# daviddmc/NeSVoR

Measured on AMD Instinct MI355X. Metric: INR train iters/sec (2^20 samples, L=16 hash, 64-wide MLP), higher is better.
Workload: dtype f32 (MLP products evaluated on 2-way fp16 splits of the power-of-two-scaled fp32 operands, fp32 accumulation: error against fp64 at or below the fp32 MFMA chain's; the all-fp32-MFMA rate of the same run is in strict_fp32_mfma)

## Files before the change

### include/nesvor_hip.h

```cpp
#ifndef NESVOR_HIP_H
#define NESVOR_HIP_H

#include <stdint.h>

#ifdef __cplusplus
extern "C" {
#endif

#define NESVOR_MAX_LEVELS 32
#define NESVOR_MAX_MLP_LAYERS 4

int nesvor_hip_abi_version(void);

int nesvor_axisangle2mat_forward(const float* ax, float* mat, int n, void* stream);
int nesvor_axisangle2mat_backward(const float* grad_mat, const float* ax, float* grad_ax, int n, void* stream);
int nesvor_mat2axisangle_forward(const float* mat, float* ax, int n, void* stream);
int nesvor_mat2axisangle_backward(const float* mat, const float* grad_ax, float* grad_mat, int n, void* stream);
int nesvor_axisangle2mat_forward_f64(const double* ax, double* mat, int n, void* stream);
int nesvor_axisangle2mat_backward_f64(const double* grad_mat, const double* ax, double* grad_ax, int n, void* stream);
int nesvor_mat2axisangle_forward_f64(const double* mat, double* ax, int n, void* stream);
int nesvor_mat2axisangle_backward_f64(const double* mat, const double* grad_ax, double* grad_mat, int n, void* stream);

int nesvor_trans_loss(const float* ax, const float* ax_init, float* loss_per_slice, float* grad_ax, int n, void* stream);

int nesvor_slice_acq_forward(const float* transforms, const float* vol, const uint8_t* vol_mask,
                             const uint8_t* slices_mask, const float* psf, float* slices, float* slices_weight,
                             int D, int H, int W, int d_p, int h_p, int w_p, int n, int h, int w,
                             float res_slice, int interp_psf, void* stream);

int nesvor_slice_acq_adjoint_forward(const float* transforms, const float* psf, const float* slices,
                                     const uint8_t* slices_mask, const uint8_t* vol_mask, float* vol, float* vol_weight,
                                     float* scratch, int D, int H, int W, int d_p, int h_p, int w_p, int n, int h, int w,
                                     float res_slice, int equalize, void* stream);
int nesvor_slice_acq_adjoint_backward(const float* transforms, float* grad_vol, const float* vol_weight,
                                      const uint8_t* vol_mask, const float* psf, const float* slices,
                                      const uint8_t* slices_mask, const float* vol, float* grad_slices,
                                      float* grad_transforms, int D, int H, int W, int d_p, int h_p, int w_p, int n, int h,
                                      int w, float res_slice, int equalize, void* stream);
int nesvor_slice_acq_backward(const float* transforms, const float* vol, const uint8_t* vol_mask, const float* psf,
                              const float* grad_slices, const uint8_t* slices_mask, float* grad_vol,
                              float* grad_transforms, float* scratch, int D, int H, int W, int d_p, int h_p, int w_p,
                              int n, int h, int w, float res_slice, void* stream);
int nesvor_slice_acq_adjoint_forward_interp(const float* transforms, const float* psf, const float* slices,
                                            const uint8_t* slices_mask, const uint8_t* vol_mask, float* vol, float* vol_weight,
                                            int D, int H, int W, int d_p, int h_p, int w_p, int n, int h, int w,
                                            float res_slice, int equalize, void* stream);
int nesvor_slice_acq_backward_interp(const float* transforms, const float* vol, const uint8_t* vol_mask, const float* psf,
                                     const float* grad_slices, const uint8_t* slices_mask, float* grad_vol,
                                     float* grad_transforms, int D, int H, int W, int d_p, int h_p, int w_p, int n, int h, int w,
                                     float res_slice, void* stream);
int nesvor_slice_acq_adjoint_backward_interp(const float* transforms, float* grad_vol, const float* vol_weight,
                                             const uint8_t* vol_mask, const float* psf, const float* slices,
                                             const uint8_t* slices_mask, const float* vol, float* grad_slices,
                                             float* grad_transforms, int D, int H, int W, int d_p, int h_p, int w_p, int n,
                                             int h, int w, float res_slice, int equalize, void* stream);
int nesvor_slice_acq_adjoint_forward_interp_f64(const double* transforms, const double* psf, const double* slices,
                                                const uint8_t* slices_mask, const uint8_t* vol_mask, double* vol,
                                                double* vol_weight, int D, int H, int W, int d_p, int h_p, int w_p, int n, int h,
                                                int w, double res_slice, int equalize, void* stream);
int nesvor_slice_acq_backward_interp_f64(const double* transforms, const double* vol, const uint8_t* vol_mask,
                                         const double* psf, const double* grad_slices, const uint8_t* slices_mask,
                                         double* grad_vol, double* grad_transforms, int D, int H, int W, int d_p, int h_p,
                                         int w_p, int n, int h, int w, double res_slice, void* stream);
int nesvor_slice_acq_adjoint_backward_interp_f64(const double* transforms, double* grad_vol, const double* vol_weight,
                                                 const uint8_t* vol_mask, const double* psf, const double* slices,
                                                 const uint8_t* slices_mask, const double* vol, double* grad_slices,
                                                 double* grad_transforms, int D, int H, int W, int d_p, int h_p, int w_p,
                                                 int n, int h, int w, double res_slice, int equalize, void* stream);
int nesvor_slice_acq_forward_f64(const double* transforms, const double* vol, const uint8_t* vol_mask,
                                 const uint8_t* slices_mask, const double* psf, double* slices, double* slices_weight,
                                 int D, int H, int W, int d_p, int h_p, int w_p, int n, int h, int w,
                                 double res_slice, int interp_psf, void* stream);
int nesvor_slice_acq_adjoint_forward_f64(const double* transforms, const double* psf, const double* slices,
                                         const uint8_t* slices_mask, const uint8_t* vol_mask, double* vol, double* vol_weight,
                                         double* scratch, int D, int H, int W, int d_p, int h_p, int w_p, int n, int h, int w,
                                         double res_slice, int equalize, void* stream);
int nesvor_slice_acq_backward_f64(const double* transforms, const double* vol, const uint8_t* vol_mask, const double* psf,
                                  const double* grad_slices, const uint8_t* slices_mask, double* grad_vol,
                                  double* grad_transforms, double* scratch, int D, int H, int W, int d_p, int h_p, int w_p,
                                  int n, int h, int w, double res_slice, void* stream);
int nesvor_slice_acq_adjoint_backward_f64(const double* transforms, double* grad_vol, const double* vol_weight,
                                          const uint8_t* vol_mask, const double* psf, const double* slices,
                                          const uint8_t* slices_mask, const double* vol, double* grad_slices,
                                          double* grad_transforms, int D, int H, int W, int d_p, int h_p, int w_p, int n, int h,
                                          int w, double res_slice, int equalize, void* stream);

typedef struct {
  int32_t n_levels;
  int32_t n_features;
  float scale[NESVOR_MAX_LEVELS];
  uint32_t res[NESVOR_MAX_LEVELS];
  uint32_t size[NESVOR_MAX_LEVELS];
  uint32_t offset[NESVOR_MAX_LEVELS];
  uint32_t hashed[NESVOR_MAX_LEVELS];
} nesvor_grid_t;

#define NESVOR_LAYOUT_ROW_MAJOR 0
#define NESVOR_LAYOUT_FEATURE_MAJOR 1
#define NESVOR_LAYOUT_CLUSTERED 4
#define NESVOR_LAYOUT_UNCLUSTERED 8
#define NESVOR_LAYOUT_DY_SCRATCH 16
#define NESVOR_LAYOUT_MASK 3

int nesvor_hashgrid_forward(const nesvor_grid_t* grid, const float* u, const float* table, float* pe,
                            int64_t N, int layout, void* stream);
int nesvor_hashgrid_forward_bounded(const nesvor_grid_t* grid, const float* u, const float* table, float* pe,
                                    int64_t N, int layout, float* pe_absmax, void* stream);
int64_t nesvor_hashgrid_forward_workspace_bytes(const nesvor_grid_t* grid, int64_t N, int layout);
int nesvor_hashgrid_forward_unclustered(const nesvor_grid_t* grid, const float* u, const float* table, float* pe, int64_t N,
                                        int layout, float* pe_absmax, void* workspace, int64_t workspace_bytes, void* stream);
int64_t nesvor_hashgrid_backward_workspace_bytes(const nesvor_grid_t* grid, int64_t N, const float* queue_scale);
int64_t nesvor_hashgrid_backward_workspace_bytes_ex(const nesvor_grid_t* grid, int64_t N, const float* queue_scale, int layout);
int64_t nesvor_hashgrid_backward_workspace_zero_bytes(void);
int64_t nesvor_hashgrid_backward_overflow_offset(void* workspace);
int nesvor_hashgrid_backward(const nesvor_grid_t* grid, const float* u, const float* table, const float* dpe,
                             float* grad_table, float* grad_u, int64_t N, int layout, void* workspace, int stages,
                             const float* queue_scale, void* stream);

int nesvor_hashgrid_backward_levels(const nesvor_grid_t* grid, const float* u, const float* table, const float* dpe,
                                    float* grad_table, float* grad_u, int64_t N, int layout, void* workspace, int stages,
                                    int level_begin, int level_end, const float* queue_scale, void* stream);
int nesvor_hashgrid_backward_bounded(const nesvor_grid_t* grid, const float* u, const float* table, const float* dpe,
                                     float* grad_table, float* grad_u, int64_t N, int layout, void* workspace, int stages,
                                     int level_begin, int level_end, const float* queue_scale, const float* dy_bound,
                                     void* stream);
int nesvor_hashgrid_backward_atomic(const nesvor_grid_t* grid, const float* u, const float* table, const float* dpe,
                                    float* grad_table, float* grad_u, int64_t N, int layout, void* stream);

int nesvor_psf_transform_forward(const float* mat, const int64_t* slice_idx, const float* xyz, const float* sigma,
                                 const float* noise, const float* bb, float* x, float* u, int B, int S, void* stream);
int nesvor_psf_transform_backward(const float* mat, const int64_t* slice_idx, const float* xyz, const float* sigma,
                                  const float* noise, const float* bb, const float* dx, const float* du, float* dmat,
                                  int B, int S, void* stream);
int nesvor_psf_transform_forward_rng(const float* mat, const int64_t* slice_idx, const float* xyz, const float* sigma,
                                     uint64_t seed, uint64_t offset, const float* bb, float* x, float* u, int B, int S,
                                     void* stream);
int nesvor_psf_transform_forward_rng_gather(const float* mat, const int64_t* slice_idx, const float* xyz, const float* sigma,
                                            uint64_t seed, uint64_t offset, const float* bb, float* x, float* u, int B, int S,
                                            const float* embedding, float* se, int ks, void* stream);
int nesvor_psf_transform_backward_rng(const float* mat, const int64_t* slice_idx, const float* xyz, const float* sigma,
                                      uint64_t seed, uint64_t offset, const float* bb, const float* dx, const float* du,
                                      float* dmat, int B, int S, void* stream);
int nesvor_psf_transform_backward_rng_slices(const float* mat, const int64_t* slice_idx, const float* xyz, const float* sigma,
                                             uint64_t seed, uint64_t offset, const float* bounding_box, const float* dx,
                                             const float* du, float* dpix, float* dmat_slice, int B, int S, void* stream);
int nesvor_psf_noise(uint64_t seed, uint64_t offset, float* out, int64_t n_samples, void* stream);

typedef struct {
  int32_t width;
  int32_t n_hidden;
  int32_t out_dim;
  int32_t k_a, k_b, b_row0;
  int32_t samples_per_pixel;
  int32_t dxa_group_sums;
  int32_t bf16_operands;
  int32_t compact_save;
  const float* weight[NESVOR_MAX_MLP_LAYERS];
  const float* bias[NESVOR_MAX_MLP_LAYERS];
  const float* prep;
  float* y_absmax;
  const void* weight_images;
} nesvor_mlp_t;
#define NESVOR_MLP_MODE_FP32 0
#define NESVOR_MLP_MODE_BF16 1
#define NESVOR_MLP_MODE_SPLIT 2
#define NESVOR_MLP_MODE_FP16 3
#define NESVOR_MLP_MODE_FP16_SCALED 4
#define NESVOR_ABSMAX_SLOTS 16
#define NESVOR_ABSMAX_STRIDE 64
#define NESVOR_ABSMAX_FLOATS (NESVOR_ABSMAX_SLOTS * NESVOR_ABSMAX_STRIDE)
#define NESVOR_MLP_PREP_XA 0
#define NESVOR_MLP_PREP_XB (1 * NESVOR_ABSMAX_FLOATS)
#define NESVOR_MLP_PREP_DY (2 * NESVOR_ABSMAX_FLOATS)
#define NESVOR_MLP_PREP_LAYER0 (3 * NESVOR_ABSMAX_FLOATS)
#define NESVOR_MLP_PREP_FLOATS (NESVOR_MLP_PREP_LAYER0 + 4 * NESVOR_MAX_MLP_LAYERS)
#define NESVOR_MLP_WHAT_INPUT 1
#define NESVOR_MLP_WHAT_DY 2
#define NESVOR_MLP_WHAT_WEIGHTS 4
int nesvor_mlp_prepare(const nesvor_mlp_t* net, const float* xa, const float* xb, const float* dy, int64_t N, float* prep,
                       int what, void* stream);
int nesvor_mlp_prepare_weights(const nesvor_mlp_t* const* nets, float* const* preps, int n_nets, const float* x, int64_t n_x,
                               float* x_slots, void* stream);

int nesvor_mlp_prepare_weights_images(const nesvor_mlp_t* const* nets, float* const* preps, void* const* images, int n_nets,
                                      const float* x, int64_t n_x, float* x_slots, void* stream);
int64_t nesvor_mlp_weight_images_bytes(const nesvor_mlp_t* net);

int nesvor_mlp_compact_save_ok(const nesvor_mlp_t* net, int64_t N);
int nesvor_mlp_bias_free_ok(const nesvor_mlp_t* net, int64_t N);

int nesvor_mlp_forward(const nesvor_mlp_t* net, const float* xa, const float* xb, float* y,
                       float* const* saved_hidden, int64_t N, void* stream);
int nesvor_mlp_backward_fused_ok(const nesvor_mlp_t* net, int64_t N);
int nesvor_mlp_backward(const nesvor_mlp_t* net, const float* xa, const float* xb, const float* dy,
                        float* const* saved_hidden, float* const* dpre_scratch, float* dxa, float* dxb,
                        float* dw_partial, int n_partial, int64_t N, void* stream);
int nesvor_mlp_backward_bounded(const nesvor_mlp_t* net, const float* xa, const float* xb, const float* dy,
                                float* const* saved_hidden, float* const* dpre_scratch, float* dxa, float* dxb,
                                float* dw_partial, int n_partial, int64_t N, float* dxb_absmax, void* stream);

#define NESVOR_MLP_WIDE_MAX_LAYERS 8
typedef struct {
  int32_t width;
  int32_t n_hidden;
  int32_t out_dim;
  int32_t k_a, k_b, b_row0;
  int32_t samples_per_pixel;
  int32_t reserved;
  const float* weight[NESVOR_MLP_WIDE_MAX_LAYERS];
  const float* bias[NESVOR_MLP_WIDE_MAX_LAYERS];
} nesvor_mlp_wide_t;
int64_t nesvor_mlp_wide_saved_floats(const nesvor_mlp_wide_t* net, int64_t N);
int nesvor_mlp_wide_param_count(const nesvor_mlp_wide_t* net);
int nesvor_mlp_wide_forward(const nesvor_mlp_wide_t* net, const float* xa, const float* xb, float* y, float* const* saved_hidden,
                            int64_t N, void* stream);
int nesvor_mlp_wide_backward(const nesvor_mlp_wide_t* net, const float* xa, const float* xb, const float* dy,
                             float* const* saved_hidden, float* const* dpre_scratch, float* dxa, float* dxb, float* dw_partial,
                             int n_partial, int64_t N, void* stream);
int nesvor_mlp_wide_backward_bounded(const nesvor_mlp_wide_t* net, const float* xa, const float* xb, const float* dy,
                                     float* const* saved_hidden, float* const* dpre_scratch, float* dxa, float* dxb,
                                     float* dw_partial, int n_partial, int64_t N, float* dxb_absmax, void* stream);

typedef struct {
  const float* z0; const float* log_var; const float* log_bias; const float* x; const float* v;
  const int64_t* slice_idx; const float* c; const float* log_var_slice; const float* log_bias_mean;
  const float* gw;
  float* loss_pix; float* dz0; float* dlog_var; float* dlog_bias; float* dx; float* dc_pix; float* dlvs_pix;
  int32_t B, S, reg_type;
  float delta;
  float* dz0_absmax; float* dlog_var_absmax; float* dlog_bias_absmax;
} nesvor_loss_t;

int nesvor_imaging_loss(const nesvor_loss_t* args, void* stream);

int nesvor_step_prologue(const float* logit_coef, float* c, const float* axisangle, float* mat, float* zero_buf,
                         int n_zero, int n, void* stream);
int nesvor_step_prologue_pose(const float* logit_coef, float* c, const float* axisangle, float* mat, float* zero_buf,
                              int n_zero, int n, const float* axisangle_init, float* trans_terms, float* g_trans, void* stream);
int nesvor_step_epilogue(const float* dc, const float* c, float* dlogit, const float* dmat, const float* axisangle,
                         const float* dtrans, float w_trans, float* daxisangle, const float* loss_pix,
                         const float* trans_terms, float* losses, int n, int B, float img_scale, float img_offset,
                         void* stream);
int nesvor_step_epilogue_scaled(const float* dc, const float* c, float* dlogit, const float* dmat, const float* axisangle,
                                const float* dtrans, float w_trans, const float* w_trans_scale, float* daxisangle,
                                const float* loss_pix, const float* trans_terms, float* losses, int n, int B, float img_scale,
                                float img_offset, void* stream);
int nesvor_slice_grads(const int64_t* slice_idx, const float* dc_pix, const float* dlvs_pix, const float* dxa,
                       const float* dpix, float* dc, float* dlvs, float* dse, float* dmat, int B, int S, int ks,
                       void* stream);
int nesvor_slice_grads_by_slice(const int64_t* slice_idx, const float* dc_pix, const float* dlvs_pix, const float* dxa,
                                const float* dpix, float* dc, float* dlvs, float* dse, float* dmat, int B, int S, int ks,
                                int n_slices, void* stream);

int nesvor_adamw_step(float* param, float* grad, float* exp_avg, float* exp_avg_sq, int64_t n,
                      float lr, float beta1, float beta2, float eps, float weight_decay,
                      float bias_correction1, float bias_correction2, float grad_scale, int zero_grad,
                      void* stream);

typedef struct {
  float lr, beta1, beta2, eps, weight_decay, bias_correction1, bias_correction2, grad_scale;
} nesvor_adamw_t;

typedef struct nesvor_loss_scaler_t {
  float scale, growth_factor, backoff_factor;
  int32_t growth_interval, growth_tracker, skipped, t;
  uint32_t found_inf;
} nesvor_loss_scaler_t;

int nesvor_grad_found_inf(const float* grad, int64_t n, nesvor_loss_scaler_t* s, void* stream);
int nesvor_adamw_step_scaled(float* param, float* grad, float* exp_avg, float* exp_avg_sq, int64_t n, float lr, double beta1,
                             double beta2, float eps, float weight_decay, int world_size, int zero_grad,
                             const nesvor_loss_scaler_t* s, void* stream);
int nesvor_loss_scaler_update(nesvor_loss_scaler_t* s, void* stream);
int nesvor_loss_scale_weights(const float* base, float* out, int n, const nesvor_loss_scaler_t* s, void* stream);

int nesvor_hashgrid_backward_adamw(const nesvor_grid_t* grid, const float* u, float* table, const float* dpe,
                                   float* grad_table, float* grad_u, int64_t N, int layout, void* workspace, int stages,
                                   const float* queue_scale, const float* dy_bound, float* exp_avg, float* exp_avg_sq,
// ... 66 lines not shown
```

### nesvor_amd/_lib.py

```python
import ctypes
import os
from ctypes import POINTER, Structure, c_double, c_float, c_int, c_int32, c_int64, c_uint32, c_uint64, c_void_p

import torch

_HERE = os.path.dirname(os.path.abspath(__file__))
LIB_PATH = os.environ.get("NESVOR_HIP_LIB") or os.path.join(_HERE, "lib", "libnesvor_hip.so")
MAX_LEVELS = 32
ABI_VERSION = 38

LAYOUT_ROW_MAJOR = 0
LAYOUT_FEATURE_MAJOR = 1
STEP_DEFER_JOIN = 8
STEP_BIAS_SUM_STOP = 16
STEP_BIAS_SUM_RESUME = 32
LAYOUT_CLUSTERED = 4
LAYOUT_UNCLUSTERED = 8
LAYOUT_DY_SCRATCH = 16


class GridT(Structure):

    _fields_ = [
        ("n_levels", c_int32),
        ("n_features", c_int32),
        ("scale", c_float * MAX_LEVELS),
        ("res", c_uint32 * MAX_LEVELS),
        ("size", c_uint32 * MAX_LEVELS),
        ("offset", c_uint32 * MAX_LEVELS),
        ("hashed", c_uint32 * MAX_LEVELS),
    ]


class MlpT(Structure):

    _fields_ = [
        ("width", c_int32), ("n_hidden", c_int32), ("out_dim", c_int32),
        ("k_a", c_int32), ("k_b", c_int32), ("b_row0", c_int32), ("samples_per_pixel", c_int32),
        ("dxa_group_sums", c_int32), ("bf16_operands", c_int32), ("compact_save", c_int32),
        ("weight", c_void_p * 4), ("bias", c_void_p * 4),
        ("prep", c_void_p), ("y_absmax", c_void_p), ("weight_images", c_void_p),
    ]


class MlpWideT(Structure):

    _fields_ = [
        ("width", c_int32), ("n_hidden", c_int32), ("out_dim", c_int32),
        ("k_a", c_int32), ("k_b", c_int32), ("b_row0", c_int32), ("samples_per_pixel", c_int32), ("reserved", c_int32),
        ("weight", c_void_p * 8), ("bias", c_void_p * 8),
    ]


class LossT(Structure):

    _fields_ = [(n, c_void_p) for n in (
        "z0", "log_var", "log_bias", "x", "v", "slice_idx", "c", "log_var_slice", "log_bias_mean", "gw",
        "loss_pix", "dz0", "dlog_var", "dlog_bias", "dx", "dc_pix", "dlvs_pix")] + [
        ("B", c_int32), ("S", c_int32), ("reg_type", c_int32), ("delta", c_float),
        ("dz0_absmax", c_void_p), ("dlog_var_absmax", c_void_p), ("dlog_bias_absmax", c_void_p)]


class StepT(Structure):

    _fields_ = (
        [("grid", GridT), ("density", MlpT), ("sigma", MlpT), ("bias_net", MlpT)]
        + [(n, c_int32) for n in ("B", "S", "n_slices", "opt_T", "has_lv", "has_c", "has_lvs", "has_b", "n_features_z", "ks", "kb_bias",
                                  "reg_type", "overlap_owner")]
        + [("delta", c_float), ("w_T", c_float)]
        + [(n, c_void_p) for n in ("axisangle", "axisangle_init", "psf_sigma", "bounding_box", "logit_coef", "log_var_slice",
                                   "slice_embedding", "table")]
        + [(n, c_void_p) for n in ("g_axisangle", "g_logit_coef", "g_log_var_slice", "g_slice_embedding", "g_table", "g_density", "g_sigma",
                                   "g_bias_net")]
        + [(n, c_int32) for n in ("n_density_params", "n_sigma_params", "n_bias_params")]
        + [("gw", c_void_p)]
        + [(n, c_void_p) for n in ("flat_param", "flat_grad", "flat_exp_avg", "flat_exp_avg_sq")]
        + [("flat_numel", c_int64)]
        + [(n, c_void_p) for n in ("small", "x", "u", "pe", "z", "log_var", "log_bias", "se", "dz", "dlv", "dlb", "dxl", "loss_pix", "pix",
                                   "dpe", "dpe_b", "du", "dpix", "dxa", "dxa_b", "trans_terms", "g_trans", "lb_mean", "mean_scratch",
                                   "partial")]
        + [("saved_d", c_void_p * 4), ("saved_s", c_void_p * 4), ("saved_b", c_void_p * 4), ("dpre_scratch", c_void_p * 4)]
        + [("hg_workspace", c_void_p), ("queue_scale", c_void_p), ("side_stream", c_void_p)]
    )


class AdamwT(Structure):

    _fields_ = [(n, c_float) for n in ("lr", "beta1", "beta2", "eps", "weight_decay", "bias_correction1", "bias_correction2", "grad_scale")]


class LossScalerT(Structure):

    _fields_ = [("scale", c_float), ("growth_factor", c_float), ("backoff_factor", c_float), ("growth_interval", c_int32),
                ("growth_tracker", c_int32), ("skipped", c_int32), ("t", c_int32), ("found_inf", c_uint32)]


_lib = None

_P = c_void_p
_SIGNATURES = {
    "nesvor_hip_abi_version": ([], c_int),
    "nesvor_axisangle2mat_forward": ([_P, _P, c_int, _P], c_int),
    "nesvor_axisangle2mat_backward": ([_P, _P, _P, c_int, _P], c_int),
    "nesvor_mat2axisangle_forward": ([_P, _P, c_int, _P], c_int),
    "nesvor_mat2axisangle_backward": ([_P, _P, _P, c_int, _P], c_int),
    "nesvor_axisangle2mat_forward_f64": ([_P, _P, c_int, _P], c_int),
    "nesvor_axisangle2mat_backward_f64": ([_P, _P, _P, c_int, _P], c_int),
    "nesvor_mat2axisangle_forward_f64": ([_P, _P, c_int, _P], c_int),
    "nesvor_mat2axisangle_backward_f64": ([_P, _P, _P, c_int, _P], c_int),
    "nesvor_trans_loss": ([_P, _P, _P, _P, c_int, _P], c_int),
    "nesvor_slice_acq_forward": (
        [_P, _P, _P, _P, _P, _P, _P] + [c_int] * 9 + [c_float, c_int, _P],
        c_int,
    ),
    "nesvor_slice_acq_adjoint_forward": ([_P] * 8 + [c_int] * 9 + [c_float, c_int, _P], c_int),
    "nesvor_slice_acq_backward": ([_P] * 9 + [c_int] * 9 + [c_float, _P], c_int),
    "nesvor_slice_acq_adjoint_backward": ([_P] * 10 + [c_int] * 9 + [c_float, c_int, _P], c_int),
    "nesvor_slice_acq_forward_f64": ([_P, _P, _P, _P, _P, _P, _P] + [c_int] * 9 + [c_double, c_int, _P], c_int),
    "nesvor_slice_acq_adjoint_forward_f64": ([_P] * 8 + [c_int] * 9 + [c_double, c_int, _P], c_int),
    "nesvor_slice_acq_backward_f64": ([_P] * 9 + [c_int] * 9 + [c_double, _P], c_int),
    "nesvor_slice_acq_adjoint_backward_f64": ([_P] * 10 + [c_int] * 9 + [c_double, c_int, _P], c_int),
    "nesvor_slice_acq_adjoint_forward_interp": ([_P] * 7 + [c_int] * 9 + [c_float, c_int, _P], c_int),
    "nesvor_slice_acq_backward_interp": ([_P] * 8 + [c_int] * 9 + [c_float, _P], c_int),
    "nesvor_slice_acq_adjoint_backward_interp": ([_P] * 10 + [c_int] * 9 + [c_float, c_int, _P], c_int),
    "nesvor_slice_acq_adjoint_forward_interp_f64": ([_P] * 7 + [c_int] * 9 + [c_double, c_int, _P], c_int),
    "nesvor_slice_acq_backward_interp_f64": ([_P] * 8 + [c_int] * 9 + [c_double, _P], c_int),
    "nesvor_slice_acq_adjoint_backward_interp_f64": ([_P] * 10 + [c_int] * 9 + [c_double, c_int, _P], c_int),
    "nesvor_hashgrid_forward": ([POINTER(GridT), _P, _P, _P, c_int64, c_int, _P], c_int),
    "nesvor_hashgrid_forward_bounded": ([POINTER(GridT), _P, _P, _P, c_int64, c_int, _P, _P], c_int),
    "nesvor_hashgrid_forward_workspace_bytes": ([POINTER(GridT), c_int64, c_int], c_int64),
    "nesvor_hashgrid_forward_unclustered": ([POINTER(GridT), _P, _P, _P, c_int64, c_int, _P, _P, c_int64, _P], c_int),
    "nesvor_hashgrid_backward_workspace_bytes": ([POINTER(GridT), c_int64, _P], c_int64),
    "nesvor_hashgrid_backward_workspace_bytes_ex": ([POINTER(GridT), c_int64, _P, c_int], c_int64),
    "nesvor_hashgrid_backward_workspace_zero_bytes": ([], c_int64),
    "nesvor_hashgrid_backward_overflow_offset": ([_P], c_int64),
    "nesvor_hashgrid_backward": ([POINTER(GridT), _P, _P, _P, _P, _P, c_int64, c_int, _P, c_int, _P, _P], c_int),
    "nesvor_hashgrid_backward_levels": ([POINTER(GridT), _P, _P, _P, _P, _P, c_int64, c_int, _P, c_int, c_int, c_int, _P, _P], c_int),
    "nesvor_hashgrid_backward_bounded": ([POINTER(GridT), _P, _P, _P, _P, _P, c_int64, c_int, _P, c_int, c_int, c_int, _P, _P, _P], c_int),
    "nesvor_hashgrid_backward_atomic": ([POINTER(GridT), _P, _P, _P, _P, _P, c_int64, c_int, _P], c_int),
    "nesvor_psf_transform_forward": ([_P] * 8 + [c_int, c_int, _P], c_int),
    "nesvor_psf_transform_backward": ([_P] * 9 + [c_int, c_int, _P], c_int),
    "nesvor_psf_transform_forward_rng_gather": ([_P] * 4 + [c_uint64, c_uint64] + [_P] * 3 + [c_int, c_int, _P, _P, c_int, _P], c_int),
    "nesvor_psf_transform_forward_rng": ([_P] * 4 + [c_uint64, c_uint64] + [_P] * 3 + [c_int, c_int, _P], c_int),
    "nesvor_psf_transform_backward_rng": ([_P] * 4 + [c_uint64, c_uint64] + [_P] * 4 + [c_int, c_int, _P], c_int),
    "nesvor_psf_transform_backward_rng_slices": ([_P] * 4 + [c_uint64, c_uint64] + [_P] * 5 + [c_int, c_int, _P], c_int),
    "nesvor_psf_noise": ([c_uint64, c_uint64, _P, c_int64, _P], c_int),
    "nesvor_mlp_compact_save_ok": ([POINTER(MlpT), c_int64], c_int),
    "nesvor_mlp_bias_free_ok": ([POINTER(MlpT), c_int64], c_int),
    "nesvor_mlp_backward_fused_ok": ([POINTER(MlpT), c_int64], c_int),
    "nesvor_mlp_prepare": ([POINTER(MlpT), _P, _P, _P, c_int64, _P, c_int, _P], c_int),
    "nesvor_mlp_prepare_weights": ([_P, _P, c_int, _P, c_int64, _P, _P], c_int),
    "nesvor_mlp_prepare_weights_images": ([_P, _P, _P, c_int, _P, c_int64, _P, _P], c_int),
    "nesvor_mlp_weight_images_bytes": ([POINTER(MlpT)], c_int64),
    "nesvor_mlp_forward": ([POINTER(MlpT), _P, _P, _P, POINTER(c_void_p), c_int64, _P], c_int),
    "nesvor_mlp_backward": (
        [POINTER(MlpT), _P, _P, _P, POINTER(c_void_p), POINTER(c_void_p), _P, _P, _P, c_int, c_int64, _P],
        c_int,
    ),
    "nesvor_mlp_backward_bounded": (
        [POINTER(MlpT), _P, _P, _P, POINTER(c_void_p), POINTER(c_void_p), _P, _P, _P, c_int, c_int64, _P, _P],
        c_int,
    ),
    "nesvor_mlp_wide_saved_floats": ([POINTER(MlpWideT), c_int64], c_int64),
    "nesvor_mlp_wide_param_count": ([POINTER(MlpWideT)], c_int),
    "nesvor_mlp_wide_forward": ([POINTER(MlpWideT), _P, _P, _P, POINTER(c_void_p), c_int64, _P], c_int),
    "nesvor_mlp_wide_backward": (
        [POINTER(MlpWideT), _P, _P, _P, POINTER(c_void_p), POINTER(c_void_p), _P, _P, _P, c_int, c_int64, _P],
        c_int,
    ),
    "nesvor_mlp_wide_backward_bounded": (
        [POINTER(MlpWideT), _P, _P, _P, POINTER(c_void_p), POINTER(c_void_p), _P, _P, _P, c_int, c_int64, _P, _P],
        c_int,
    ),
    "nesvor_imaging_loss": ([POINTER(LossT), _P], c_int),
    "nesvor_slice_grads_by_slice": ([_P] * 9 + [c_int, c_int, c_int, c_int, _P], c_int),
    "nesvor_slice_grads": ([_P] * 9 + [c_int, c_int, c_int, _P], c_int),
    "nesvor_step_prologue": ([_P] * 5 + [c_int, c_int, _P], c_int),
    "nesvor_step_prologue_pose": ([_P] * 5 + [c_int, c_int, _P, _P, _P, _P], c_int),
    "nesvor_step_epilogue": ([_P] * 6 + [c_float, _P, _P, _P, _P, c_int, c_int, c_float, c_float, _P], c_int),
    "nesvor_step_epilogue_scaled": ([_P] * 6 + [c_float, _P, _P, _P, _P, _P, c_int, c_int, c_float, c_float, _P], c_int),
    "nesvor_hashgrid_backward_adamw": ([POINTER(GridT), _P, _P, _P, _P, _P, c_int64, c_int, _P, c_int, _P, _P, _P, _P, POINTER(AdamwT), _P], c_int),
    "nesvor_adamw_step": (
        [_P, _P, _P, _P, c_int64] + [c_float] * 8 + [c_int, _P],
        c_int,
    ),
    "nesvor_grad_found_inf": ([_P, c_int64, _P, _P], c_int),
    "nesvor_adamw_step_scaled": ([_P, _P, _P, _P, c_int64, c_float, c_double, c_double, c_float, c_float, c_int, c_int, _P, _P], c_int),
    "nesvor_loss_scaler_update": ([_P, _P], c_int),
    "nesvor_loss_scale_weights": ([_P, _P, c_int, _P, _P], c_int),
    "nesvor_sum_rows_multi": ([_P, _P, _P, _P, c_int, c_int, _P], c_int),
    "nesvor_sum_rows": ([_P, _P, c_int, c_int, c_int, _P], c_int),
    "nesvor_step_create": ([POINTER(StepT)], c_void_p),
    "nesvor_step_update": ([_P, POINTER(StepT)], c_int),
    "nesvor_step_destroy": ([_P], None),
    "nesvor_step_join": ([_P, _P], c_int),
    "nesvor_step_set_bias_mean_ranks": ([_P, c_int], c_int),
    "nesvor_step_set_bias_mean_event": ([_P, _P], c_int),
    "nesvor_step_timing": ([_P, c_int], c_int),
    "nesvor_step_timing_read": ([_P, _P], c_int),
    "nesvor_step_run": ([_P, _P, _P, _P, c_uint64, c_uint64, _P, c_int, c_int, POINTER(AdamwT), _P], c_int),
    "nesvor_vvr_similarity": ([_P, c_int, c_int, c_int, _P, _P, _P, _P, c_int64, c_int, _P, _P, _P], c_int),
}


def exported_symbols():
    return list(_SIGNATURES)


def load():
    global _lib
    if _lib is not None:
        return _lib
    if not os.path.exists(LIB_PATH):
        raise RuntimeError(
            f"{LIB_PATH} not found: the HIP backend has not been built. "
            "Run `python -m nesvor_amd.csrc.build` (or __graft_entry__.build()). "
            "There is no CPU fallback for the native ops."
        )
    lib = ctypes.CDLL(LIB_PATH)
    for name, (argtypes, restype) in _SIGNATURES.items():
        fn = getattr(lib, name)
        fn.argtypes = argtypes
        fn.restype = restype
    v = lib.nesvor_hip_abi_version()
    if v != ABI_VERSION:
        raise RuntimeError(f"libnesvor_hip ABI {v} != expected {ABI_VERSION}; rebuild")
    _lib = lib
    return lib


def stream_ptr(device=None):
    return c_void_p(torch.cuda.current_stream(device).cuda_stream)


def ptr(t):
    if t is None:
        return c_void_p(0)
    return c_void_p(t.data_ptr())


def check(err, what):
    if err != 0:
        raise RuntimeError(f"{what}: HIP error {err}")


def require_device(*tensors, dtype=None, name="tensor"):
    for t in tensors:
        if t is None:
            continue
        if not t.is_cuda:
            raise RuntimeError(f"{name} must be a device (HIP) tensor — the native ops have no CPU path")
        if not t.is_contiguous():
            raise RuntimeError(f"{name} must be contiguous")
        if dtype is not None and t.dtype != dtype:
            raise RuntimeError(f"{name} must be {dtype}, got {t.dtype}")


class KernelTimer:

    def __init__(self):
        self.enabled = False
        self.records = {}

    def reset(self, enabled):
        self.enabled = enabled
        self.records = {}

    class _Span:
        def __init__(self, timer, name):
            self.timer, self.name = timer, name

        def __enter__(self):
            if self.timer.enabled:
                self.s = torch.cuda.Event(enable_timing=True)
                self.e = torch.cuda.Event(enable_timing=True)
                self.s.record()
            return self

        def __exit__(self, *exc):
            if self.timer.enabled:
                self.e.record()
                self.timer.records.setdefault(self.name, []).append((self.s, self.e))
            return False

    def span(self, name):
        return KernelTimer._Span(self, name)

    def summary(self):
        return {k: (len(v), sum(s.elapsed_time(e) for s, e in v) / len(v)) for k, v in self.records.items()}


kernel_timer = KernelTimer()
# ... 1 lines not shown
```

### nesvor_amd/csrc/hashgrid.hip

```cpp
#include <hip/hip_runtime.h>
#include <mutex>
#include <type_traits>
#include <unordered_map>
#include "common.h"
#include "adam.h"
#include "../../include/nesvor_hip.h"

#ifndef NESVOR_ABLATE
#define NESVOR_ABLATE 0
#endif
#define NESVOR_ABL(bit) ((NESVOR_ABLATE & (bit)) != 0)
#ifndef NESVOR_SORT_SPAN
#define NESVOR_SORT_SPAN 256
#endif

namespace {

constexpr uint32_t kPrimeY = 2654435761u;
constexpr uint32_t kPrimeZ = 805459861u;

struct LevelParams {
  float scale;
  uint32_t res, size, offset, hashed;
};

__device__ __forceinline__ LevelParams load_level(const nesvor_grid_t& g, int level) {
  LevelParams p;
  p.scale = g.scale[level];
  p.res = g.res[level];
  p.size = g.size[level];
  p.offset = g.offset[level];
  p.hashed = g.hashed[level];
  return p;
}

__device__ __forceinline__ uint32_t corner_index(const LevelParams& p, uint32_t x, uint32_t y, uint32_t z) {
  if (p.hashed) {
    const uint32_t h = x ^ (y * kPrimeY) ^ (z * kPrimeZ);
    return ((p.size & (p.size - 1)) == 0) ? (h & (p.size - 1)) : (h % p.size);
  }
  uint32_t idx = x + __umul24(y, p.res) + __umul24(z, p.res * p.res);
  if (idx >= p.size) idx %= p.size;
  return idx;
}

__device__ __forceinline__ uint32_t scan32_u32(uint32_t v, int lane) {
#define NESVOR_SCAN_STEP_(SHR)                                                                        \
  v += (uint32_t)__builtin_amdgcn_update_dpp(0, (int)v, 0x110 | (SHR), 0xf, 0xf, true);
  NESVOR_SCAN_STEP_(1) NESVOR_SCAN_STEP_(2) NESVOR_SCAN_STEP_(4) NESVOR_SCAN_STEP_(8)
#undef NESVOR_SCAN_STEP_
  const uint32_t row0 = (uint32_t)__builtin_amdgcn_readlane((int)v, 15);
  return v + ((lane >= 16 && lane < 32) ? row0 : 0u);
}

struct RoundSchedule {
  uint32_t slot_off, bkt_off, grp_end, rnd_slots, rnd_bkts;
  int box_end;
};
__device__ __forceinline__ RoundSchedule round_schedule(uint32_t vol, uint32_t nch, int first, int last, int lane, uint32_t max_slots,
                                                        uint32_t max_bkts, int max_group) {
  const unsigned long long no_box = __ballot(vol == 0u) | ~((1ull << last) - 1ull);
  const int e = __builtin_ctzll(no_box & ~((1ull << first) - 1ull));
  const bool in = lane >= first && lane < e;
  const uint32_t v_in = in ? vol : 0u, n_in = in ? nch : 0u;
  const uint32_t C = scan32_u32(v_in, lane), N = scan32_u32(n_in, lane);
  RoundSchedule r;
  r.slot_off = 0u; r.bkt_off = 0u; r.grp_end = 0u; r.rnd_slots = 0u; r.rnd_bkts = 0u; r.box_end = e;
  int g0 = first;
  while (g0 < e) {
    const uint32_t cb = (uint32_t)__builtin_amdgcn_readlane((int)(C - v_in), g0), nb = (uint32_t)__builtin_amdgcn_readlane((int)(N - n_in), g0);
    const bool ok = lane >= g0 && lane < e && C - cb <= max_slots && N - nb <= max_bkts && lane - g0 < max_group;
    int bnd = __builtin_ctzll((__ballot(!ok) & ~((1ull << g0) - 1ull)) | (1ull << 63));
    bnd = bnd > g0 ? bnd : g0 + 1;
    const bool mine = lane >= g0 && lane < bnd;
    r.slot_off = mine ? (C - v_in) - cb : r.slot_off;
    r.bkt_off = mine ? (N - n_in) - nb : r.bkt_off;
    r.grp_end = mine ? (uint32_t)bnd : r.grp_end;
    const uint32_t cs = (uint32_t)__builtin_amdgcn_readlane((int)C, bnd - 1) - cb, ns = (uint32_t)__builtin_amdgcn_readlane((int)N, bnd - 1) - nb;
    r.rnd_slots = lane == g0 ? cs : r.rnd_slots;
    r.rnd_bkts = lane == g0 ? ns : r.rnd_bkts;
    g0 = bnd;
  }
  return r;
}

struct CellPos {
  uint32_t gx, gy, gz;
  float wx, wy, wz;
};

__device__ __forceinline__ CellPos locate(const LevelParams& p, float ux, float uy, float uz) {
  CellPos c;
  const float px = fmaf(p.scale, ux, 0.5f), py = fmaf(p.scale, uy, 0.5f), pz = fmaf(p.scale, uz, 0.5f);
  const float fx = floorf(px), fy = floorf(py), fz = floorf(pz);
  c.gx = (uint32_t)(int)fx; c.gy = (uint32_t)(int)fy; c.gz = (uint32_t)(int)fz;
  c.wx = px - fx; c.wy = py - fy; c.wz = pz - fz;
  return c;
}

template <int F>
__device__ __forceinline__ void load_feat(const float* __restrict__ p, float (&v)[F]) {
  if constexpr (F == 1) {
    v[0] = p[0];
  } else if constexpr (F == 2) {
    const float2 t = *reinterpret_cast<const float2*>(p);
    v[0] = t.x; v[1] = t.y;
  } else {
#pragma unroll
    for (int k = 0; k < F; k += 4) {
      const float4 t = *reinterpret_cast<const float4*>(p + k);
      v[k] = t.x; v[k + 1] = t.y; v[k + 2] = t.z; v[k + 3] = t.w;
    }
  }
}

template <int F>
__device__ __forceinline__ void load_feat_pair(const float* __restrict__ tab, uint32_t i0, uint32_t i1, float (&v0)[F], float (&v1)[F]) {
  if constexpr (F <= 2) {
    const bool adj = (i1 == i0 + 1u) || (i0 == i1 + 1u);
    const uint32_t p = adj ? min(i0, i1) : (i0 & ~1u);
    float t[2 * F];
    if constexpr (F == 1) {
      struct __attribute__((packed, aligned(4))) P2 { float a, b; };
      const P2 w = *reinterpret_cast<const P2*>(tab + (size_t)p);
      t[0] = w.a; t[1] = w.b;
    } else {
      struct __attribute__((packed, aligned(8))) P4 { float a, b, c, d; };
      const P4 w = *reinterpret_cast<const P4*>(tab + (size_t)p * 2);
      t[0] = w.a; t[1] = w.b; t[2] = w.c; t[3] = w.d;
    }
    const bool second0 = i0 != p;
#pragma unroll
    for (int f = 0; f < F; ++f) { v0[f] = second0 ? t[F + f] : t[f]; v1[f] = second0 ? t[f] : t[F + f]; }
    if (!adj) load_feat<F>(tab + (size_t)i1 * F, v1);
  } else {
    load_feat<F>(tab + (size_t)i0 * F, v0);
    load_feat<F>(tab + (size_t)i1 * F, v1);
  }
}

template <int F, int LAYOUT>
__global__ __launch_bounds__(256) void hashgrid_fwd(const nesvor_grid_t g, const float* __restrict__ u,
                                                    const float* __restrict__ table, float* __restrict__ pe,
                                                    int64_t N, int box_cache, float* __restrict__ pe_absmax) {
  constexpr int kFwdSlots = F <= 2 ? 1024 : (F == 4 ? 512 : 256);
  __shared__ uint32_t wbox[4][6];
  __shared__ __attribute__((aligned(16))) float cache[kFwdSlots * F];
  const int level = blockIdx.y, tid = threadIdx.x, lane = tid & 63;
  const int64_t i = (int64_t)blockIdx.x * 256 + tid;
  const bool valid = i < N;
  const int64_t ii = valid ? i : N - 1;
  const LevelParams p = load_level(g, level);
  const float ux = u[3 * ii], uy = u[3 * ii + 1], uz = u[3 * ii + 2];
  const CellPos c = locate(p, ux, uy, uz);
  const float* tab = table + (size_t)p.offset * F;
  float v[8][F];
  bool cached = false;
  if (box_cache) {
    const uint32_t bx = c.gx + 1u, by = c.gy + 1u, bz = c.gz + 1u;
    const uint32_t lo0 = wave_min_u32_dpp(bx), lo1 = wave_min_u32_dpp(by), lo2 = wave_min_u32_dpp(bz);
    const uint32_t hi0 = wave_max_u32_dpp(bx), hi1 = wave_max_u32_dpp(by), hi2 = wave_max_u32_dpp(bz);
    if (lane == 0) {
      uint32_t* w = wbox[tid >> 6];
      w[0] = lo0; w[1] = lo1; w[2] = lo2; w[3] = hi0; w[4] = hi1; w[5] = hi2;
    }
    __syncthreads();
    uint32_t lo[3], hi[3];
#pragma unroll
    for (int d = 0; d < 3; ++d) {
      lo[d] = min(min(wbox[0][d], wbox[1][d]), min(wbox[2][d], wbox[3][d]));
      hi[d] = max(max(wbox[0][3 + d], wbox[1][3 + d]), max(wbox[2][3 + d], wbox[3][3 + d]));
      lo[d] = (uint32_t)__builtin_amdgcn_readfirstlane((int)lo[d]);
      hi[d] = (uint32_t)__builtin_amdgcn_readfirstlane((int)hi[d]);
    }
    const uint32_t ex = hi[0] - lo[0], ey = hi[1] - lo[1], ez = hi[2] - lo[2];
    const uint32_t nx = ex + 2u, ny = ey + 2u, nz = ez + 2u, nxy = nx * ny;
    cached = ex < (uint32_t)kFwdSlots && ey < (uint32_t)kFwdSlots && ez < (uint32_t)kFwdSlots &&
             (uint64_t)nxy * nz <= (uint64_t)kFwdSlots;
    if (cached) {
      const uint32_t vol = nxy * nz;
      const float inv_nxy = 1.f / (float)nxy, inv_nx = 1.f / (float)nx;
      for (uint32_t s = tid; s < vol; s += 256) {
        const uint32_t z = (uint32_t)(((float)s + 0.5f) * inv_nxy);
        const uint32_t r = s - __umul24(z, nxy);
        const uint32_t y = (uint32_t)(((float)r + 0.5f) * inv_nx);
        const uint32_t idx = corner_index(p, lo[0] - 1u + (r - __umul24(y, nx)), lo[1] - 1u + y, lo[2] - 1u + z);
        float t[F];
        load_feat<F>(tab + (size_t)idx * F, t);
#pragma unroll
        for (int f = 0; f < F; ++f) cache[s * F + f] = t[f];
      }
      __syncthreads();
      const uint32_t s0 = __umul24(__umul24(bz - lo[2], ny) + (by - lo[1]), nx) + (bx - lo[0]);
#pragma unroll
      for (int k = 0; k < 8; ++k) {
        const uint32_t s = s0 + (k & 1) + ((k >> 1) & 1) * nx + (k >> 2) * nxy;
#pragma unroll
        for (int f = 0; f < F; ++f) v[k][f] = cache[s * F + f];
      }
    }
  }
  if (!cached) {
#pragma unroll
    for (int k = 0; k < 8; k += 2) {
      const uint32_t i0 = corner_index(p, c.gx, c.gy + ((k >> 1) & 1), c.gz + (k >> 2));
      const uint32_t i1 = corner_index(p, c.gx + 1u, c.gy + ((k >> 1) & 1), c.gz + (k >> 2));
      load_feat_pair<F>(tab, i0, i1, v[k], v[k + 1]);
    }
  }
  float acc[F];
#pragma unroll
  for (int f = 0; f < F; ++f) acc[f] = 0.f;
  if (valid) {
#pragma unroll
    for (int k = 0; k < 8; ++k) {
      const float w = ((k & 1) ? c.wx : 1.f - c.wx) * (((k >> 1) & 1) ? c.wy : 1.f - c.wy) * ((k >> 2) ? c.wz : 1.f - c.wz);
#pragma unroll
      for (int f = 0; f < F; ++f) acc[f] = fmaf(w, v[k][f], acc[f]);
    }
    const int E = g.n_levels * F;
    if constexpr (LAYOUT == NESVOR_LAYOUT_ROW_MAJOR) {
      float* o = pe + (size_t)i * E + level * F;
#pragma unroll
      for (int f = 0; f < F; ++f) o[f] = acc[f];
    } else {
#pragma unroll
      for (int f = 0; f < F; ++f) pe[(size_t)(level * F + f) * N + i] = acc[f];
    }
  }
  if (pe_absmax != nullptr) {
    float m = 0.f;
#pragma unroll
    for (int f = 0; f < F; ++f) m = fmaxf(m, fabsf(acc[f]));
    publish_absmax_wg(pe_absmax, m);
  }
}

#ifndef NESVOR_FWD_PK
#define NESVOR_FWD_PK 1
#endif
#ifndef NESVOR_FWD_SSTORE
#define NESVOR_FWD_SSTORE 1
#endif
template <int F, int LAYOUT>
__global__ __launch_bounds__(256) void hashgrid_fwd_cloud(const nesvor_grid_t g, const float* __restrict__ u,
                                                          const float* __restrict__ table, float* __restrict__ pe, int64_t N,
                                                          float* __restrict__ pe_absmax,
                                                          const uint32_t* __restrict__ perm = nullptr, float* __restrict__ rows = nullptr,
                                                          int level_begin = 0, int level_stop = NESVOR_MAX_LEVELS) {
#ifndef NESVOR_FWD_CLOUD_SLOTS
#define NESVOR_FWD_CLOUD_SLOTS 512
#endif
  constexpr int kSlots = F <= 2 ? NESVOR_FWD_CLOUD_SLOTS : (F == 4 ? 512 : 256);
  constexpr int kMaxGroup = 8;
  constexpr int NRB = kSlots / 256;
  __shared__ __attribute__((aligned(16))) float tcache[2][kSlots * F];
  __shared__ float ubox[4][6];
  __shared__ uint32_t lbox[NESVOR_MAX_LEVELS + 1][8];
  __shared__ uint32_t lpar[NESVOR_MAX_LEVELS + 1][4];
  __shared__ uint32_t slot_off[NESVOR_MAX_LEVELS + 1], grp_end[NESVOR_MAX_LEVELS + 1], rnd_slots[NESVOR_MAX_LEVELS + 1];
  __shared__ int32_t box_end_s;
  const int tid = threadIdx.x, lane = tid & 63;
  const int64_t slot_i = (int64_t)blockIdx.x * 256 + tid;
  const bool valid = slot_i < N;
  const int64_t si = valid ? slot_i : N - 1;
  const int64_t i = perm != nullptr ? (int64_t)perm[si] : slot_i;
  const int64_t ii = perm != nullptr ? i : si;
  const int L = g.n_levels, E = L * F;
  const int lb = level_begin, le = min(level_stop, L);
  const float ux = u[3 * ii], uy = u[3 * ii + 1], uz = u[3 * ii + 2];
  {
    float lo[3] = {ux, uy, uz}, hi[3] = {ux, uy, uz};
#pragma unroll
    for (int d = 0; d < 3; ++d) { lo[d] = -wave_max_f32_dpp(-lo[d]); hi[d] = wave_max_f32_dpp(hi[d]); }
    if (lane == 0) {
#pragma unroll
      for (int d = 0; d < 3; ++d) { ubox[tid >> 6][d] = lo[d]; ubox[tid >> 6][3 + d] = hi[d]; }
    }
  }
  __syncthreads();
  if (tid < 64) {
    float ulo[3], uhi[3];
#pragma unroll
    for (int d = 0; d < 3; ++d) {
      ulo[d] = fminf(fminf(ubox[0][d], ubox[1][d]), fminf(ubox[2][d], ubox[3][d]));
      uhi[d] = fmaxf(fmaxf(ubox[0][3 + d], ubox[1][3 + d]), fmaxf(ubox[2][3 + d], ubox[3][3 + d]));
    }
    uint32_t b[8] = {0u, 0u, 0u, 0u, 0u, 0u, 0u, 0u};
    if (tid < L) {
      const LevelParams p = load_level(g, tid);
      const CellPos blo = locate(p, ulo[0], ulo[1], ulo[2]), bhi = locate(p, uhi[0], uhi[1], uhi[2]);
      const uint32_t ex = bhi.gx - blo.gx, ey = bhi.gy - blo.gy, ez = bhi.gz - blo.gz;
      const bool fits = ex < (uint32_t)kSlots && ey < (uint32_t)kSlots && ez < (uint32_t)kSlots &&
                        (uint64_t)(ex + 2u) * (ey + 2u) * (ez + 2u) <= (uint64_t)kSlots;
      const uint32_t nx = ex + 2u, nxy = nx * (ey + 2u), vol = fits ? nxy * (ez + 2u) : 0u;
      b[0] = blo.gx; b[1] = blo.gy; b[2] = blo.gz; b[3] = ex; b[4] = ey; b[5] = ez; b[6] = vol;
      b[7] = fits ? vol - 2u - nx - nxy : 0u;
      lpar[tid][0] = p.res; lpar[tid][1] = p.size; lpar[tid][2] = p.offset; lpar[tid][3] = p.hashed;
    }
    if (tid <= L) {
#pragma unroll
      for (int q = 0; q < 8; ++q) lbox[tid][q] = b[q];
    }
    const RoundSchedule rs = round_schedule(b[6], 0u, lb, le, tid, (uint32_t)kSlots, 0xFFFFFFFFu, kMaxGroup);
    if (tid == 0) box_end_s = rs.box_end;
    if (tid < NESVOR_MAX_LEVELS) { slot_off[tid] = rs.slot_off; grp_end[tid] = rs.grp_end; rnd_slots[tid] = rs.rnd_slots; }
  }
  __syncthreads();
  const int box_end = __builtin_amdgcn_readfirstlane(box_end_s);
  auto sgpr = [](uint32_t v) { return (uint32_t)__builtin_amdgcn_readfirstlane((int)v); };
  const bool off32 = NESVOR_FWD_SSTORE && N < ((int64_t)1 << 30);
  const uint32_t i4 = (uint32_t)i * 4u;
  float pe_mx = 0.f;
  auto store_pe = [&](int level, const float (&acc)[F]) __attribute__((always_inline)) {
    if (!valid) return;
#pragma unroll
    for (int f = 0; f < F; ++f) pe_mx = fmaxf(pe_mx, fabsf(acc[f]));
    if (rows != nullptr) {
      float* o = rows + (size_t)slot_i * E + level * F;
#pragma unroll
      for (int f = 0; f < F; ++f) o[f] = acc[f];
      return;
    }
    if constexpr (LAYOUT == NESVOR_LAYOUT_ROW_MAJOR) {
      float* o = pe + (size_t)i * E + level * F;
#pragma unroll
      for (int f = 0; f < F; ++f) o[f] = acc[f];
    } else {
      if (off32) {
#pragma unroll
        for (int f = 0; f < F; ++f) gstore_b32_sbase(pe + (size_t)(level * F + f) * N, i4, acc[f]);
      } else {
#pragma unroll
        for (int f = 0; f < F; ++f) pe[(size_t)(level * F + f) * N + i] = acc[f];
      }
    }
  };
  auto blend = [&](const CellPos& c, const float (&v)[8][F], float (&acc)[F]) __attribute__((always_inline)) {
    if constexpr (F == 2 && NESVOR_FWD_PK) {
      typedef float f32x2 __attribute__((ext_vector_type(2)));
      const f32x2 wx2 = {1.f - c.wx, c.wx};
      const float ay[2] = {1.f - c.wy, c.wy}, az[2] = {1.f - c.wz, c.wz};
      f32x2 a = {0.f, 0.f};
#pragma unroll
      for (int zy = 0; zy < 4; ++zy) {
        const f32x2 w2 = (wx2 * ay[zy & 1]) * az[zy >> 1];
        a = __builtin_elementwise_fma(f32x2{w2.x, w2.x}, f32x2{v[2 * zy][0], v[2 * zy][1]}, a);
        a = __builtin_elementwise_fma(f32x2{w2.y, w2.y}, f32x2{v[2 * zy + 1][0], v[2 * zy + 1][1]}, a);
      }
      acc[0] = a.x; acc[1] = a.y;
      return;
    }
#pragma unroll
    for (int f = 0; f < F; ++f) acc[f] = 0.f;
#pragma unroll
    for (int k = 0; k < 8; ++k) {
      const float w = ((k & 1) ? c.wx : 1.f - c.wx) * (((k >> 1) & 1) ? c.wy : 1.f - c.wy) * ((k >> 2) ? c.wz : 1.f - c.wz);
#pragma unroll
      for (int f = 0; f < F; ++f) acc[f] = fmaf(w, v[k][f], acc[f]);
    }
  };
  auto fetch_round = [&](int ra, int rb, float (&feat)[NRB][F]) __attribute__((always_inline)) {
    const uint32_t total = sgpr(rnd_slots[ra]);
#pragma unroll
    for (int j = 0; j < NRB; ++j) {
      const uint32_t slot = (uint32_t)j * 256u + (uint32_t)tid;
#pragma unroll
      for (int f = 0; f < F; ++f) feat[j][f] = 0.f;
      if (slot < total) {
        int lv = ra;
        for (int l = ra + 1; l < rb; ++l) lv = slot >= slot_off[l] ? l : lv;
        const uint32_t local = slot - slot_off[lv];
        const uint32_t nx = lbox[lv][3] + 2u, nxy = nx * (lbox[lv][4] + 2u);
        const uint32_t z = (uint32_t)(((float)local + 0.5f) * (1.f / (float)nxy));
        const uint32_t r = local - __umul24(z, nxy);
        const uint32_t y = (uint32_t)(((float)r + 0.5f) * (1.f / (float)nx));
        LevelParams pl;
        pl.scale = 0.f; pl.res = lpar[lv][0]; pl.size = lpar[lv][1]; pl.offset = lpar[lv][2]; pl.hashed = lpar[lv][3];
        const uint32_t key = corner_index(pl, lbox[lv][0] + (r - __umul24(y, nx)), lbox[lv][1] + y, lbox[lv][2] + z);
        load_feat<F>(table + ((size_t)pl.offset + key) * F, feat[j]);
      }
    }
  };
  auto stash_round = [&](int ra, int buf, const float (&feat)[NRB][F]) __attribute__((always_inline)) {
    const uint32_t total = sgpr(rnd_slots[ra]);
#pragma unroll
    for (int j = 0; j < NRB; ++j) {
      const uint32_t slot = (uint32_t)j * 256u + (uint32_t)tid;
      if (slot < total) {
#pragma unroll
        for (int f = 0; f < F; ++f) tcache[buf][slot * F + f] = feat[j][f];
      }
    }
  };
  if (box_end > lb) {
    int ra = lb, rb = (int)sgpr(grp_end[lb]), buf = 0;
    {
      float feat[NRB][F];
      fetch_round(ra, rb, feat);
      stash_round(ra, 0, feat);
    }
    __syncthreads();
    for (;;) {
      const int na = rb, nb = na < box_end ? (int)sgpr(grp_end[na]) : na;
      const bool more = na < box_end;
      float nfeat[NRB][F];
      if (more) fetch_round(na, nb, nfeat);
#pragma unroll 1
      for (int lv = ra; lv < rb; ++lv) {
        const LevelParams p = load_level(g, lv);
        const CellPos c = locate(p, ux, uy, uz);
        const uint32_t x0 = sgpr(lbox[lv][0]), y0 = sgpr(lbox[lv][1]), z0 = sgpr(lbox[lv][2]);
        const uint32_t ny = sgpr(lbox[lv][4]) + 2u, nx = sgpr(lbox[lv][3]) + 2u, nxy = nx * ny;
        const uint32_t s0 = min(__umul24(__umul24(c.gz - z0, ny) + (c.gy - y0), nx) + (c.gx - x0), sgpr(lbox[lv][7])) + sgpr(slot_off[lv]);
        float v[8][F], acc[F];
#pragma unroll
        for (int k = 0; k < 8; ++k) {
          const uint32_t sl = s0 + (k & 1) + ((k >> 1) & 1) * nx + (k >> 2) * nxy;
#pragma unroll
          for (int f = 0; f < F; ++f) v[k][f] = tcache[buf][sl * F + f];
        }
        blend(c, v, acc);
        store_pe(lv, acc);
      }
      if (!more) break;
      stash_round(na, buf ^ 1, nfeat);
      __syncthreads();
      buf ^= 1; ra = na; rb = nb;
    }
  }
#pragma unroll 1
  for (int lv = box_end; lv < le; lv += 2) {
    const bool two = lv + 1 < le;
    const LevelParams p0 = load_level(g, lv), p1 = load_level(g, two ? lv + 1 : lv);
    const CellPos c0 = locate(p0, ux, uy, uz), c1 = locate(p1, ux, uy, uz);
    const float* tab0 = table + (size_t)p0.offset * F;
    const float* tab1 = table + (size_t)p1.offset * F;
    float v0[8][F], v1[8][F], acc[F];
    {
#pragma unroll
    for (int k = 0; k < 8; ++k) load_feat<F>(tab0 + (size_t)corner_index(p0, c0.gx + (k & 1), c0.gy + ((k >> 1) & 1), c0.gz + (k >> 2)) * F, v0[k]);
    if (two) {
#pragma unroll
      for (int k = 0; k < 8; ++k) load_feat<F>(tab1 + (size_t)corner_index(p1, c1.gx + (k & 1), c1.gy + ((k >> 1) & 1), c1.gz + (k >> 2)) * F, v1[k]);
    }
    }
    blend(c0, v0, acc);
    store_pe(lv, acc);
    if (two) {
      blend(c1, v1, acc);
      store_pe(lv + 1, acc);
    }
  }
  if (pe_absmax != nullptr) publish_absmax_wg(pe_absmax, pe_mx);
}

template <int F, int LAYOUT, bool INPUT_GRAD, bool MERGE>
__global__ __launch_bounds__(256) void hashgrid_bwd(const nesvor_grid_t g, const float* __restrict__ u,
                                                    const float* __restrict__ table, const float* __restrict__ dpe,
                                                    float* __restrict__ grad_table, float* __restrict__ grad_u,
                                                    int64_t N) {
  const int level = blockIdx.y;
  const int64_t i = (int64_t)blockIdx.x * 256 + threadIdx.x;
  const bool valid = i < N;
  const LevelParams p = load_level(g, level);
  const int64_t ii = valid ? i : N - 1;
  const float ux = u[3 * ii], uy = u[3 * ii + 1], uz = u[3 * ii + 2];
  const CellPos c = locate(p, ux, uy, uz);
  const int E = g.n_levels * F;
  float dy[F];
  if constexpr (LAYOUT == NESVOR_LAYOUT_ROW_MAJOR) {
    const float* o = dpe + (size_t)ii * E + level * F;
#pragma unroll
    for (int f = 0; f < F; ++f) dy[f] = valid ? o[f] : 0.f;
  } else {
#pragma unroll
    for (int f = 0; f < F; ++f) dy[f] = valid ? dpe[(size_t)(level * F + f) * N + ii] : 0.f;
  }
  uint32_t idx[8];
#pragma unroll
  for (int k = 0; k < 8; ++k) idx[k] = corner_index(p, c.gx + (k & 1), c.gy + ((k >> 1) & 1), c.gz + (k >> 2));

  if constexpr (INPUT_GRAD) {
    const float* tab = table + (size_t)p.offset * F;
    float gx = 0.f, gy = 0.f, gz = 0.f;
    float v[8][F];
#pragma unroll
    for (int k = 0; k < 8; ++k) load_feat<F>(tab + (size_t)idx[k] * F, v[k]);
#pragma unroll
    for (int k = 0; k < 8; ++k) {
      float fd = 0.f;
#pragma unroll
      for (int f = 0; f < F; ++f) fd = fmaf(v[k][f], dy[f], fd);
      const float wxk = (k & 1) ? c.wx : 1.f - c.wx, wyk = ((k >> 1) & 1) ? c.wy : 1.f - c.wy, wzk = (k >> 2) ? c.wz : 1.f - c.wz;
      gx += ((k & 1) ? fd : -fd) * wyk * wzk;
      gy += (((k >> 1) & 1) ? fd : -fd) * wxk * wzk;
      gz += ((k >> 2) ? fd : -fd) * wxk * wyk;
    }
    if (valid) {
      atomicAdd(grad_u + 3 * i + 0, p.scale * gx);
      atomicAdd(grad_u + 3 * i + 1, p.scale * gy);
      atomicAdd(grad_u + 3 * i + 2, p.scale * gz);
    }
  }

  float* gt = grad_table + (size_t)p.offset * F;
  float val[8][F];
#pragma unroll
  for (int k = 0; k < 8; ++k) {
    const float w = ((k & 1) ? c.wx : 1.f - c.wx) * (((k >> 1) & 1) ? c.wy : 1.f - c.wy) * ((k >> 2) ? c.wz : 1.f - c.wz);
#pragma unroll
    for (int f = 0; f < F; ++f) val[k][f] = w * dy[f];
  }

  bool pending = valid;
  if constexpr (MERGE) {
    const int lane = threadIdx.x & 63;
    for (int round = 0; round < 4; ++round) {
      const unsigned long long rem = __ballot(pending);
      if (rem == 0) break;
      const int leader = __ffsll((long long)rem) - 1;
      const uint32_t lx = __shfl(c.gx, leader, 64), ly = __shfl(c.gy, leader, 64), lz = __shfl(c.gz, leader, 64);
      const bool mine = pending && c.gx == lx && c.gy == ly && c.gz == lz;
      const unsigned long long grp = __ballot(mine);
      if (__popcll(grp) < 8) break;
#pragma unroll
      for (int k = 0; k < 8; ++k)
#pragma unroll
        for (int f = 0; f < F; ++f) {
          const float s = wave_sum(mine ? val[k][f] : 0.f);
          if (lane == leader) atomicAdd(gt + (size_t)idx[k] * F + f, s);
        }
      pending = pending && !mine;
    }
  }
  if (pending) {
#pragma unroll
    for (int k = 0; k < 8; ++k)
#pragma unroll
      for (int f = 0; f < F; ++f) atomicAdd(gt + (size_t)idx[k] * F + f, val[k][f]);
  }
}

constexpr int kMaxChunks = 256;
constexpr int kSubQueues = 8;
constexpr uint32_t kTailStride = 4096;
constexpr uint32_t kOverflowBase = kTailStride - NESVOR_MAX_LEVELS;
constexpr int kOwnerLdsFloats = 8192;

struct BwdPlan {
  uint32_t shift[NESVOR_MAX_LEVELS];
  uint32_t n_buckets;
  uint32_t n_chunks[NESVOR_MAX_LEVELS];
  uint32_t bucket_base[NESVOR_MAX_LEVELS];
  uint32_t cap[NESVOR_MAX_LEVELS];
  uint32_t slice[NESVOR_MAX_LEVELS];
  uint64_t rec_off[NESVOR_MAX_LEVELS];
  uint32_t n_sub;
  uint32_t box_slots;
  int32_t level_begin, level_end;
  int32_t accumulate_u;
};

template <int K, int J>
__device__ __forceinline__ void bitonic_merge(uint32_t& sv, int tid, uint32_t* sortbuf) {
  uint32_t other;
  if constexpr (J < 64) {
    other = lane_xor_u32<J>(sv, tid & 63);
  } else {
    __syncthreads();
    sortbuf[tid] = sv;
    __syncthreads();
    other = sortbuf[tid ^ J];
  }
  const bool keep_min = ((tid & K) == 0) == ((tid & J) == 0);
  sv = keep_min ? min(sv, other) : max(sv, other);
  if constexpr (J > 1) bitonic_merge<K, J / 2>(sv, tid, sortbuf);
}
template <int K>
__device__ __forceinline__ void bitonic_sort(uint32_t& sv, int tid, uint32_t* sortbuf) {
  if constexpr (K > 2) bitonic_sort<K / 2>(sv, tid, sortbuf);
  bitonic_merge<K, K / 2>(sv, tid, sortbuf);
}

__device__ __forceinline__ uint32_t spread3(uint32_t x) {
  x &= 0xffu;
  x = (x ^ (x << 8)) & 0x0300f00fu;
  x = (x ^ (x << 4)) & 0x030c30c3u;
  x = (x ^ (x << 2)) & 0x09249249u;
  return x;
}

__device__ __forceinline__ unsigned long long to_fixed(float x) {
  const float t = rintf(x * 0x1p-32f);
  const int32_t lo = __float2int_rn(fmaf(-t, 0x1p32f, x));
  return ((unsigned long long)(uint32_t)((int32_t)t + (lo >> 31)) << 32) | (unsigned long long)(uint32_t)lo;
}
#ifndef NESVOR_HG_F64FIX
#define NESVOR_HG_F64FIX 0
#endif
__device__ __forceinline__ unsigned long long to_fixed51(float x, double scale) {
  return (unsigned long long)__double_as_longlong(fma((double)x, scale, 0x1.8p52));
}
__device__ __forceinline__ float from_fixed51(unsigned long long q) {
  const uint32_t lo = (uint32_t)q;
  const int32_t hi = ((int32_t)(uint32_t)(q >> 32) << 13) >> 13;
  return fmaf((float)(hi + (int32_t)(lo >> 31)), 0x1p32f, (float)(int32_t)lo);
}
__device__ __forceinline__ float from_fixed(unsigned long long q) {
  const uint32_t lo = (uint32_t)q;
  return fmaf((float)((int32_t)(q >> 32) + (int32_t)(lo >> 31)), 0x1p32f, (float)(int32_t)lo);
}


#ifndef NESVOR_FIXED32
#define NESVOR_FIXED32 0
#endif

#ifndef NESVOR_HG_SLOTS
#define NESVOR_HG_SLOTS 1024
#endif
#ifndef NESVOR_HG_MINBLOCKS
#define NESVOR_HG_MINBLOCKS 4
#endif
#ifndef NESVOR_HG_SPATIAL
#define NESVOR_HG_SPATIAL 1
#endif
#ifndef NESVOR_HG_TIMELINE
#define NESVOR_HG_TIMELINE 0
#endif
#if NESVOR_HG_TIMELINE
constexpr int kTlWgs = 64, kTlMarks = 96;
__device__ unsigned long long g_hg_timeline[kTlWgs][kTlMarks];
#define HG_TICK(site)                                                                                              \
  do {                                                                                                             \
    if (blockIdx.x < (unsigned)kTlWgs && threadIdx.x == 0 && tl_n < kTlMarks)                                      \
      g_hg_timeline[blockIdx.x][tl_n++] = ((unsigned long long)(site) << 56) | (__builtin_amdgcn_s_memtime() & 0x00FFFFFFFFFFFFFFull); \
  } while (0)
#else
#define HG_TICK(site) do { } while (0)
#endif
template <int F, int LAYOUT, bool INPUT_GRAD, bool MERGE, bool BOUND = false>
__global__ __launch_bounds__(256, F <= 2 ? NESVOR_HG_MINBLOCKS : (F == 4 ? 3 : 2)) void hashgrid_bwd_aggregate(const nesvor_grid_t g, const BwdPlan plan,
                                                              const float* __restrict__ u,
                                                              const float* __restrict__ table,
                                                              const float* __restrict__ dpe,
                                                              float* __restrict__ grad_table,
                                                              float* __restrict__ grad_u, uint32_t* __restrict__ tails,
                                                              uint32_t* __restrict__ tails_next,
                                                              uint32_t* __restrict__ records, int64_t N,
                                                              const float* __restrict__ dy_bound,
                                                              uint8_t* __restrict__ order,
                                                              int order_mode,
                                                              const uint32_t* __restrict__ perm,
                                                              int dy_by_slot) {
  for (uint32_t t = blockIdx.x * 256u + threadIdx.x; t < (uint32_t)kSubQueues * kTailStride; t += gridDim.x * 256u) tails_next[t] = 0u;
  constexpr bool kPack = (F == 2) && (NESVOR_FIXED32 != 0);
  constexpr bool kPerLevel = kPack && (NESVOR_FIXED32 >= 2);
  constexpr int kWords = kPack ? 1 : F;
  __shared__ uint32_t bcount[kMaxChunks];
  __shared__ __attribute__((aligned(16))) uint32_t bb_raw[4 * kMaxChunks];
  uint4* const bbase4 = reinterpret_cast<uint4*>(bb_raw);
  uint2(*const bbase)[kMaxChunks] = reinterpret_cast<uint2(*)[kMaxChunks]>(bb_raw);
  __shared__ uint32_t sortbuf[256];
  constexpr int kSlots = F <= 2 ? NESVOR_HG_SLOTS : (F == 4 ? 512 : 256);
  constexpr uint32_t kEmpty = 0xFFFFFFFFu;
  constexpr uint32_t kKeyMask = (1u << 27) - 1u;
  constexpr int kMaxGroup = 8;
  __shared__ __attribute__((aligned(16))) uint32_t tkeys[kSlots];
  __shared__ __attribute__((aligned(16))) unsigned long long tvals[kSlots * kWords];
  __shared__ __attribute__((aligned(16))) float tcache[INPUT_GRAD && MERGE ? kSlots * F : 1];
  __shared__ float gmax[4];
  __shared__ uint32_t lmax_bits[NESVOR_MAX_LEVELS + 1];
  __shared__ float lscale[NESVOR_MAX_LEVELS + 1][2];
  __shared__ uint32_t merge_stat[2];
  __shared__ uint32_t slots_log2;
  __shared__ uint32_t merge_off;
  __shared__ uint32_t prev_cnt;
  __shared__ float ubox[4][6];
  __shared__ uint32_t lbox[NESVOR_MAX_LEVELS + 1][8];
  __shared__ uint32_t lwin[NESVOR_MAX_LEVELS + 1];
  __shared__ uint32_t slot_off[NESVOR_MAX_LEVELS + 1], bkt_off[NESVOR_MAX_LEVELS + 1], grp_end[NESVOR_MAX_LEVELS + 1];
  __shared__ uint32_t rnd_slots[NESVOR_MAX_LEVELS + 1], rnd_bkts[NESVOR_MAX_LEVELS + 1];
  __shared__ uint32_t lpar[NESVOR_MAX_LEVELS + 1][8];
  __shared__ int32_t box_end_s;
  const int tid = threadIdx.x, lane = tid & 63;
  const int64_t base = (int64_t)blockIdx.x * 256;
  const int E = g.n_levels * F;
#if NESVOR_HG_TIMELINE
  int tl_n = 0;
  if (blockIdx.x < (unsigned)kTlWgs && tid == 0) for (int k = 0; k < kTlMarks; ++k) g_hg_timeline[blockIdx.x][k] = 0ull;
#endif
  HG_TICK(0);
  const int level_end = plan.level_end;
  const uint32_t sub = (uint32_t)__builtin_amdgcn_s_getreg((3 << 11) | (0 << 6) | 20) & (plan.n_sub - 1u);
  if (tid < kMaxChunks) bcount[tid] = 0;
  for (int t = tid; t < kSlots; t += 256) tkeys[t] = kEmpty;
  for (int t = tid; t < kSlots * kWords; t += 256) tvals[t] = 0ull;
  if (tid < 2) merge_stat[tid] = 0;
  if (tid == 0) { merge_off = MERGE ? 0u : 1u; slots_log2 = __builtin_ctz(kSlots); prev_cnt = 0u; }
  if constexpr (kPerLevel) {
    if (tid <= NESVOR_MAX_LEVELS) lmax_bits[tid] = 0u;
  }

  uint32_t sv;
  {
    const int64_t s0_ = base + tid;
    uint32_t code = 0x00ffffffu;
    if (s0_ < N) {
      const int64_t i0 = perm != nullptr ? (int64_t)perm[s0_] : s0_;
      const LevelParams pf = load_level(g, g.n_levels - 1);
      const CellPos c = locate(pf, u[3 * i0], u[3 * i0 + 1], u[3 * i0 + 2]);
      code = spread3(c.gx) | (spread3(c.gy) << 1) | (spread3(c.gz) << 2);
    }
    sv = (code << 8) | (uint32_t)tid;
    if (order_mode == 2) sv = (uint32_t)order[base + tid];
    else
#pragma unroll 1
    for (int rep = 0; rep < (NESVOR_ABL(1) ? 2 : 1); ++rep) {
      if (rep) sv ^= 0x80000000u;
      bitonic_sort<NESVOR_SORT_SPAN>(sv, tid, sortbuf);
      if (rep) sv ^= 0x80000000u;
    }
  }
  HG_TICK(1);
  if (order_mode == 1) order[base + tid] = (uint8_t)(sv & 255u);
  const int64_t slot_i = base + (sv & 255u);
  const bool valid = slot_i < N;
  const int64_t i = (valid && perm != nullptr) ? (int64_t)perm[slot_i] : slot_i;
  const int64_t ii = valid ? i : N - 1;
  const int64_t id = dy_by_slot ? (valid ? slot_i : N - 1) : ii;
  const float ux = u[3 * ii], uy = u[3 * ii + 1], uz = u[3 * ii + 2];
  float gux = 0.f, guy = 0.f, guz = 0.f;

  auto load_dy = [&](int level, float (&dy)[F]) __attribute__((always_inline)) {
    if constexpr (LAYOUT == NESVOR_LAYOUT_ROW_MAJOR) {
      const float* o = dpe + (size_t)id * E + level * F;
#pragma unroll
      for (int f = 0; f < F; ++f) dy[f] = valid ? o[f] : 0.f;
    } else {
#pragma unroll
      for (int f = 0; f < F; ++f) dy[f] = valid ? dpe[(size_t)(level * F + f) * N + id] : 0.f;
    }
  };

  if constexpr (MERGE) {
    float lo[3] = {ux, uy, uz}, hi[3] = {ux, uy, uz};
#pragma unroll
    for (int d = 0; d < 3; ++d) {
      lo[d] = -wave_max_f32_dpp(-lo[d]);
      hi[d] = wave_max_f32_dpp(hi[d]);
    }
    float m = 0.f;
    if constexpr (kPerLevel) __syncthreads();
    if constexpr (BOUND) {
      m = *dy_bound;
      if constexpr (kPerLevel) {
        if (tid < NESVOR_MAX_LEVELS) lmax_bits[tid] = __float_as_uint(m);
      }
    } else
    for (int l0 = plan.level_begin; l0 < level_end; l0 += 8) {
      float d[8][F];
#pragma unroll
      for (int q = 0; q < 8; ++q) {
        if (l0 + q < level_end) load_dy(l0 + q, d[q]);
        else {
#pragma unroll
          for (int f = 0; f < F; ++f) d[q][f] = 0.f;
        }
      }
#pragma unroll
      for (int q = 0; q < 8; ++q) {
        float ml = 0.f;
#pragma unroll
        for (int f = 0; f < F; ++f) ml = fmaxf(ml, fabsf(d[q][f]));
        m = fmaxf(m, ml);
        if constexpr (kPerLevel) {
          ml = wave_max_f32_dpp(ml);
          if (lane == 0 && l0 + q < level_end) atomicMax(&lmax_bits[l0 + q], __float_as_uint(ml));
        }
      }
    }
    m = wave_max_f32_dpp(m);
    if (lane == 0) {
#pragma unroll
      for (int d = 0; d < 3; ++d) { ubox[tid >> 6][d] = lo[d]; ubox[tid >> 6][3 + d] = hi[d]; }
      gmax[tid >> 6] = m;
    }
  }
  __syncthreads();
  HG_TICK(2);
  float ulo[3] = {0.f, 0.f, 0.f}, uhi[3] = {0.f, 0.f, 0.f};
  float fscale = 1.f, finv = 1.f;
  if constexpr (MERGE) {
#pragma unroll
    for (int d = 0; d < 3; ++d) {
      ulo[d] = fminf(fminf(ubox[0][d], ubox[1][d]), fminf(ubox[2][d], ubox[3][d]));
      uhi[d] = fmaxf(fmaxf(ubox[0][3 + d], ubox[1][3 + d]), fmaxf(ubox[2][3 + d], ubox[3][3 + d]));
      ulo[d] = __builtin_bit_cast(float, __builtin_amdgcn_readfirstlane(__builtin_bit_cast(int, ulo[d])));
      uhi[d] = __builtin_bit_cast(float, __builtin_amdgcn_readfirstlane(__builtin_bit_cast(int, uhi[d])));
    }
    {
      float mx = 256.f * fmaxf(fmaxf(gmax[0], gmax[1]), fmaxf(gmax[2], gmax[3]));
      mx = __builtin_bit_cast(float, __builtin_amdgcn_readfirstlane(__builtin_bit_cast(int, mx)));
      int sexp = (kPack ? 29 : (NESVOR_HG_F64FIX ? 48 : 60)) - ((int)((__float_as_uint(mx) >> 23) & 0xFFu) - 127);
      sexp = sexp > 100 ? 100 : (sexp < -100 ? -100 : sexp);
      fscale = __uint_as_float((uint32_t)(sexp + 127) << 23);
      finv = __uint_as_float((uint32_t)(127 - sexp) << 23);
    }
    HG_TICK(6);
    if (tid < 64) {
      uint32_t b[8] = {0u, 0u, 0u, 0u, 0u, 0u, 0u, 0u};
      uint32_t nch = 0u;
      const LevelParams p = load_level(g, tid < g.n_levels ? tid : 0);
      const int tl_ = tid < g.n_levels ? tid : 0;
      const uint32_t pl_nch = plan.n_chunks[tl_], pl_cap = plan.cap[tl_], pl_base = plan.bucket_base[tl_], pl_rec = (uint32_t)plan.rec_off[tl_],
                     pl_shift = plan.shift[tl_];
      if (tid < g.n_levels) {
        const CellPos blo = locate(p, ulo[0], ulo[1], ulo[2]), bhi = locate(p, uhi[0], uhi[1], uhi[2]);
        const uint32_t ex = bhi.gx - blo.gx, ey = bhi.gy - blo.gy, ez = bhi.gz - blo.gz;
        const bool fits = plan.box_slots != 0u && ex < (uint32_t)kSlots && ey < (uint32_t)kSlots && ez < (uint32_t)kSlots &&
                          (uint64_t)(ex + 2u) * (ey + 2u) * (ez + 2u) <= (uint64_t)kSlots;
        const uint32_t nx = ex + 2u, nxy = nx * (ey + 2u), vol = fits ? nxy * (ez + 2u) : 0u;
        b[0] = blo.gx; b[1] = blo.gy; b[2] = blo.gz; b[3] = ex; b[4] = ey; b[5] = ez; b[6] = vol;
        b[7] = fits ? vol - 2u - nx - nxy : 0u;
        {
          const uint32_t vx = min(ex, 1023u) + 2u, vy = min(ey, 1023u) + 2u, vz = min(ez, 1023u) + 2u;
          uint32_t ba = 0, bb = 0, bc = 0;
          for (int n = 0; n < __builtin_ctz(kSlots); ++n) {
            const uint32_t rx = (vx << 12) >> ba, ry = (vy << 12) >> bb, rz = (vz << 12) >> bc;
            if (rz >= rx && rz >= ry) ++bc;
            else if (ry >= rx) ++bb;
            else ++ba;
          }
          lwin[tid] = ba | (bb << 8) | (bc << 16);
        }
        nch = pl_nch;
        lpar[tid][0] = p.res; lpar[tid][1] = p.size; lpar[tid][2] = p.offset; lpar[tid][3] = p.hashed;
        lpar[tid][4] = pl_cap; lpar[tid][5] = pl_base; lpar[tid][6] = pl_rec;
        lpar[tid][7] = pl_shift;
        if constexpr (kPerLevel) {
          const float mxl = 256.f * __uint_as_float(lmax_bits[tid]);
          int se = 29 - ((int)((__float_as_uint(mxl) >> 23) & 0xFFu) - 127);
          se = se > 100 ? 100 : (se < -100 ? -100 : se);
          lscale[tid][0] = __uint_as_float((uint32_t)(se + 127) << 23);
          lscale[tid][1] = __uint_as_float((uint32_t)(127 - se) << 23);
        }
      }
      HG_TICK(7);
      if (tid <= g.n_levels) {
#pragma unroll
        for (int q = 0; q < 8; ++q) lbox[tid][q] = b[q];
      }
      const RoundSchedule rs = round_schedule(b[6], nch, plan.level_begin, level_end, tid, (uint32_t)kSlots, (uint32_t)kMaxChunks, kMaxGroup);
      if (tid == 0) box_end_s = rs.box_end;
      if (tid < NESVOR_MAX_LEVELS) {
        slot_off[tid] = rs.slot_off; bkt_off[tid] = rs.bkt_off; grp_end[tid] = rs.grp_end;
        rnd_slots[tid] = rs.rnd_slots; rnd_bkts[tid] = rs.rnd_bkts;
      }
      HG_TICK(8);
    }
    __syncthreads();
    HG_TICK(3);
  }
  const int box_end = MERGE ? __builtin_amdgcn_readfirstlane(box_end_s) : plan.level_begin;
  auto sgpr = [](uint32_t v) { return (uint32_t)__builtin_amdgcn_readfirstlane((int)v); };

  auto prepare = [&](auto box_c, int level, const float (&dy)[F], uint32_t (&idx)[8], uint32_t& s0, uint32_t& nx, uint32_t& nxy,
                     float (&val)[8][F], bool& tail) __attribute__((always_inline)) {
    constexpr bool BOX = decltype(box_c)::value;
    level = __builtin_amdgcn_readfirstlane(level);
    const LevelParams p = load_level(g, level);
    const CellPos c = locate(p, ux, uy, uz);
    if constexpr (BOX) {
      const uint32_t x0 = sgpr(lbox[level][0]), y0 = sgpr(lbox[level][1]), z0 = sgpr(lbox[level][2]);
      const uint32_t ny = sgpr(lbox[level][4]) + 2u;
      nx = sgpr(lbox[level][3]) + 2u; nxy = nx * ny;
      s0 = min(__umul24(__umul24(c.gz - z0, ny) + (c.gy - y0), nx) + (c.gx - x0), sgpr(lbox[level][7])) + sgpr(slot_off[level]);
    } else {
#pragma unroll
      for (int k = 0; k < 8; ++k) idx[k] = corner_index(p, c.gx + (k & 1), c.gy + ((k >> 1) & 1), c.gz + (k >> 2));
      s0 = (c.gx & 1023u) | ((c.gy & 1023u) << 10) | ((c.gz & 1023u) << 20);
    }
    if constexpr (INPUT_GRAD) {
      float v[8][F];
      if constexpr (BOX) {
#pragma unroll
        for (int k = 0; k < 8; ++k) {
          const uint32_t s = s0 + (k & 1) + ((k >> 1) & 1) * nx + (k >> 2) * nxy;
#pragma unroll
          for (int f = 0; f < F; ++f) v[k][f] = tcache[s * F + f];
        }
      } else {
        const float* tab = table + (size_t)p.offset * F;
#pragma unroll
        for (int k = 0; k < 8; ++k) load_feat<F>(tab + (size_t)idx[k] * F, v[k]);
      }
      float q[8];
#pragma unroll
      for (int k = 0; k < 8; ++k) {
        q[k] = v[k][0] * dy[0];
#pragma unroll
        for (int f = 1; f < F; ++f) q[k] = fmaf(v[k][f], dy[f], q[k]);
      }
      float dxl[4], lx[4];
#pragma unroll
      for (int e = 0; e < 4; ++e) { dxl[e] = q[2 * e + 1] - q[2 * e]; lx[e] = fmaf(c.wx, dxl[e], q[2 * e]); }
      const float sx0 = fmaf(c.wy, dxl[1] - dxl[0], dxl[0]), sx1 = fmaf(c.wy, dxl[3] - dxl[2], dxl[2]);
      const float sx = fmaf(c.wz, sx1 - sx0, sx0);
      const float dy0 = lx[1] - lx[0], dy1 = lx[3] - lx[2];
      const float sy = fmaf(c.wz, dy1 - dy0, dy0);
      const float sz = fmaf(c.wy, dy1, lx[2]) - fmaf(c.wy, dy0, lx[0]);
      gux = fmaf(p.scale, sx, gux); guy = fmaf(p.scale, sy, guy); guz = fmaf(p.scale, sz, guz);
    }
    {
      const float ax[2] = {1.f - c.wx, c.wx}, ay[2] = {1.f - c.wy, c.wy}, az[2] = {1.f - c.wz, c.wz};
#pragma unroll
      for (int k = 0; k < 8; ++k) {
        const float w = ax[k & 1] * ay[(k >> 1) & 1] * az[k >> 2];
#pragma unroll
        for (int f = 0; f < F; ++f) val[k][f] = w * dy[f];
      }
    }
    const int rl = lane & 15;
    const uint32_t px_ = (uint32_t)__builtin_amdgcn_update_dpp(0, (int)c.gx, 0x111, 0xf, 0xf, true);
    const uint32_t py_ = (uint32_t)__builtin_amdgcn_update_dpp(0, (int)c.gy, 0x111, 0xf, 0xf, true);
    const uint32_t pz_ = (uint32_t)__builtin_amdgcn_update_dpp(0, (int)c.gz, 0x111, 0xf, 0xf, true);
    const bool vprev = __builtin_amdgcn_update_dpp(0, (int)valid, 0x111, 0xf, 0xf, true) != 0;
    const bool head = rl == 0 || !valid || !vprev || c.gx != px_ || c.gy != py_ || c.gz != pz_;
    const bool next_head = __builtin_amdgcn_update_dpp(1, (int)head, 0x101, 0xf, 0xf, false) != 0;
    tail = valid && (rl == 15 || next_head);
    int flag = head ? 1 : 0;
#define NESVOR_SCAN_STEP(SHR, CTRL)                                                                        \
    {                                                                                                      \
      const float m = flag ? 0.f : 1.f;                                                                    \
      _Pragma("unroll") for (int k = 0; k < 8; ++k) _Pragma("unroll") for (int f = 0; f < F; ++f)          \
        asm volatile("v_fmac_f32_dpp %0, %0, %1 row_shr:" #SHR " row_mask:0xf bank_mask:0xf bound_ctrl:1"  \
                     : "+v"(val[k][f]) : "v"(m));                                                          \
      flag |= __builtin_amdgcn_update_dpp(0, flag, CTRL, 0xf, 0xf, true);                                  \
    }
    if constexpr (!NESVOR_ABL(2)) {
#define NESVOR_FENCE8(f) asm volatile("s_nop 1" : "+v"(val[0][f]), "+v"(val[1][f]), "+v"(val[2][f]), "+v"(val[3][f]), "+v"(val[4][f]), "+v"(val[5][f]), "+v"(val[6][f]), "+v"(val[7][f]))
      NESVOR_FENCE8(0);
      if constexpr (F >= 2) NESVOR_FENCE8(1);
      if constexpr (F >= 4) { NESVOR_FENCE8(2); NESVOR_FENCE8(3); }
      if constexpr (F >= 8) { NESVOR_FENCE8(4); NESVOR_FENCE8(5); NESVOR_FENCE8(6); NESVOR_FENCE8(7); }
#undef NESVOR_FENCE8
      NESVOR_SCAN_STEP(1, 0x111)
      if (__ballot(flag == 0)) {
        NESVOR_SCAN_STEP(2, 0x112)
        if (__ballot(flag == 0)) {
          NESVOR_SCAN_STEP(4, 0x114)
          if (__ballot(flag == 0)) NESVOR_SCAN_STEP(8, 0x118)
        }
      }
    }
#undef NESVOR_SCAN_STEP
  };

  auto scale_of = [&](uint32_t lv) __attribute__((always_inline)) { return kPerLevel ? lscale[lv][0] : fscale; };
  auto inv_of = [&](uint32_t lv) __attribute__((always_inline)) { return kPerLevel ? lscale[lv][1] : finv; };
  auto slot_add = [&](uint32_t slot, const float (&v)[F], float fscale) __attribute__((always_inline)) {
    if constexpr (kPack) {
      const int32_t q0 = __float2int_rn(v[0] * fscale), q1 = __float2int_rn(v[1] * fscale);
      atomicAdd(&tvals[slot], ((unsigned long long)(uint32_t)(q1 + (q0 >> 31)) << 32) | (unsigned long long)(uint32_t)q0);
    } else {
#pragma unroll
      for (int f = 0; f < F; ++f) {
        if constexpr (NESVOR_HG_F64FIX != 0) atomicAdd(&tvals[f * kSlots + slot], to_fixed51(v[f], (double)fscale));
        else atomicAdd(&tvals[f * kSlots + slot], to_fixed(v[f] * fscale));
      }
    }
  };
  auto slot_take = [&](uint32_t slot, float (&v)[F], float finv) __attribute__((always_inline)) -> bool {
    bool any = false;
    if constexpr (kPack) {
      const unsigned long long w = tvals[slot];
      any = w != 0ull;
      if (any) {
        const int32_t lo = (int32_t)(uint32_t)w;
        const int32_t hi = (int32_t)(uint32_t)(w >> 32) - (lo >> 31);
        v[0] = (float)lo * finv; v[1] = (float)hi * finv;
        tvals[slot] = 0ull;
      }
    } else {
      unsigned long long w[F];
#pragma unroll
      for (int f = 0; f < F; ++f) { w[f] = tvals[f * kSlots + slot]; any = any || w[f] != 0ull; }
      if (any) {
#pragma unroll
        for (int f = 0; f < F; ++f) {
          v[f] = (NESVOR_HG_F64FIX != 0 ? from_fixed51(w[f]) : from_fixed(w[f])) * finv;
          tvals[f * kSlots + slot] = 0ull;
        }
      }
    }
    return any;
  };

  float dy_a[F], dy_b[F];
// ... 751 lines not shown
  s.where[i] = ((unsigned long long)c << 32) | k;
}
__global__ __launch_bounds__(1024) void sort_scan_kernel(SortPlan p, SortBufs s) {
  constexpr int kTile = 32768, kPer = kTile / 1024;
  extern __shared__ uint32_t cnt[];
  __shared__ uint32_t wsum[16];
  __shared__ uint32_t carry_s;
  const int tid = threadIdx.x;
  if (tid == 0) carry_s = 0;
  __syncthreads();
  const uint32_t total = p.n_cells + 1;
  for (uint32_t t0 = 0; t0 < total; t0 += kTile) {
    {
      uint32_t v[kPer];
#pragma unroll
      for (int k = 0; k < kPer; ++k) {
        const uint32_t c = t0 + (uint32_t)(k * 1024 + tid);
        v[k] = c < total ? s.count[c] : 0u;
      }
#pragma unroll
      for (int k = 0; k < kPer; ++k) {
        const uint32_t c = t0 + (uint32_t)(k * 1024 + tid);
        const int j = k * 1024 + tid;
        cnt[j + (j >> 5)] = c < p.n_cells ? min(v[k], p.cap) : v[k];
      }
    }
    __syncthreads();
    uint32_t sum = 0;
#pragma unroll
    for (int k = 0; k < kPer; ++k) sum += cnt[tid * kPer + k + tid];
    uint32_t incl = sum;
#pragma unroll
    for (int d = 1; d < 64; d <<= 1) {
      const uint32_t o = (uint32_t)__shfl_up((int)incl, d);
      if ((tid & 63) >= d) incl += o;
    }
    if ((tid & 63) == 63) wsum[tid >> 6] = incl;
    __syncthreads();
    uint32_t before = carry_s + incl - sum;
    for (int w = 0; w < (tid >> 6); ++w) before += wsum[w];
#pragma unroll
    for (int k = 0; k < kPer; ++k) {
      const int j = tid * kPer + k;
      const uint32_t v = cnt[j + tid];
      cnt[j + tid] = before;
      before += v;
    }
    __syncthreads();
    if (tid == 1023) carry_s = before;
    for (int k = 0; k < kPer; ++k) {
      const uint32_t c = t0 + (uint32_t)(k * 1024 + tid);
      const int j = k * 1024 + tid;
      if (c < total) s.first[c] = cnt[j + (j >> 5)];
    }
    __syncthreads();
  }
  if (tid == 0) s.first[total] = carry_s;
}
__global__ __launch_bounds__(256) void sort_compact_kernel(SortPlan p, SortBufs s) {
  const uint64_t t = (uint64_t)blockIdx.x * 256 + threadIdx.x;
  const uint64_t n_strip = (uint64_t)p.n_cells * p.cap;
  if (t < n_strip) {
    const uint32_t c = (uint32_t)(t / p.cap), k = (uint32_t)(t - (uint64_t)c * p.cap);
    if (k < min(s.count[c], p.cap)) s.perm[s.first[c] + k] = s.strips[t];
  } else {
    const uint64_t k = t - n_strip;
    if (k < (uint64_t)s.count[p.n_cells]) s.perm[s.first[p.n_cells] + (uint32_t)k] = s.spill[k];
  }
}
constexpr int kGatherPts = 256;
__global__ __launch_bounds__(256) void gather_dy_rows_kernel(const float* __restrict__ dpe, SortBufs s, float* __restrict__ rows, int64_t N, int E) {
  extern __shared__ float tile[];
  __shared__ uint32_t rank[kGatherPts];
  const int tid = threadIdx.x;
  const int64_t i0 = (int64_t)blockIdx.x * kGatherPts;
  const bool ok = i0 + tid < N;
  if (ok) {
    const unsigned long long w = s.where[i0 + tid];
    rank[tid] = s.first[(uint32_t)(w >> 32)] + (uint32_t)w;
  }
  for (int e0 = 0; e0 < E; e0 += 8) {
    float v[8];
#pragma unroll
    for (int q = 0; q < 8; ++q) v[q] = (ok && e0 + q < E) ? dpe[(size_t)(e0 + q) * N + i0 + tid] : 0.f;
#pragma unroll
    for (int q = 0; q < 8; ++q)
      if (e0 + q < E) tile[tid * (E + 1) + e0 + q] = v[q];
  }
  __syncthreads();
  if ((E & 3) == 0) {
    const int E4 = E >> 2;
    for (int idx = tid; idx < kGatherPts * E4; idx += 256) {
      const int q = idx / E4, e = (idx - q * E4) * 4;
      const float* t = tile + q * (E + 1) + e;
      if (i0 + q < N) *reinterpret_cast<float4*>(rows + (size_t)rank[q] * E + e) = make_float4(t[0], t[1], t[2], t[3]);
    }
  } else {
    for (int idx = tid; idx < kGatherPts * E; idx += 256) {
      const int q = idx / E, e = idx - q * E;
      if (i0 + q < N) rows[(size_t)rank[q] * E + e] = tile[q * (E + 1) + e];
    }
  }
}
__global__ __launch_bounds__(256) void scatter_pe_rows_kernel(const float* __restrict__ rows, SortBufs s, float* __restrict__ pe, int64_t N, int E) {
  extern __shared__ float tile[];
  __shared__ uint32_t rank[kGatherPts];
  const int tid = threadIdx.x;
  const int64_t i0 = (int64_t)blockIdx.x * kGatherPts;
  const bool ok = i0 + tid < N;
  if (ok) {
    const unsigned long long w = s.where[i0 + tid];
    rank[tid] = s.first[(uint32_t)(w >> 32)] + (uint32_t)w;
  }
  __syncthreads();
  if ((E & 3) == 0) {
    const int E4 = E >> 2;
    for (int idx = tid; idx < kGatherPts * E4; idx += 256) {
      const int q = idx / E4, e = (idx - q * E4) * 4;
      if (i0 + q < N) {
        const float4 v = *reinterpret_cast<const float4*>(rows + (size_t)rank[q] * E + e);
        float* t = tile + q * (E + 1) + e;
        t[0] = v.x; t[1] = v.y; t[2] = v.z; t[3] = v.w;
      }
    }
  } else {
    for (int idx = tid; idx < kGatherPts * E; idx += 256) {
      const int q = idx / E, e = idx - q * E;
      if (i0 + q < N) tile[q * (E + 1) + e] = rows[(size_t)rank[q] * E + e];
    }
  }
  __syncthreads();
  if (ok) {
    for (int e = 0; e < E; ++e) pe[(size_t)e * N + i0 + tid] = tile[tid * (E + 1) + e];
  }
}
inline int sort_points(const float* u, int64_t N, uint32_t* base, hipStream_t st) {
  const SortPlan p = sort_plan(N);
  const SortBufs s = sort_bufs(base, N, p);
  hipError_t e = hipMemsetAsync(s.count, 0, sizeof(uint32_t) * (p.n_cells + 1), st);
  if (e != hipSuccess) return (int)e;
  hipLaunchKernelGGL(sort_place_kernel, dim3((unsigned)((N + 255) / 256)), dim3(256), 0, st, u, N, p, s);
  static std::once_flag raised;
  constexpr size_t kScanLds = sizeof(uint32_t) * (32768 + 32768 / 32);
  std::call_once(raised, []() { (void)hipFuncSetAttribute(reinterpret_cast<const void*>(sort_scan_kernel), hipFuncAttributeMaxDynamicSharedMemorySize, (int)kScanLds); });
  hipLaunchKernelGGL(sort_scan_kernel, dim3(1), dim3(1024), kScanLds, st, p, s);
  const uint64_t n_threads = (uint64_t)p.n_cells * p.cap + (uint64_t)((N + 255) / 256) * 256;
  hipLaunchKernelGGL(sort_compact_kernel, dim3((unsigned)((n_threads + 255) / 256)), dim3(256), 0, st, p, s);
  return (int)hipGetLastError();
}

template <int F, int LAYOUT>
int launch_bwd_owner(const nesvor_grid_t* g, const float* u, const float* table, const float* dpe, float* gt,
                     float* gu, int64_t N, void* workspace, int stages, int level_begin, int level_end, const float* queue_scale,
                     const float* dy_bound, const OwnerAdam* adam, hipStream_t st, int hints = 0) {
  const bool unclustered = (hints & NESVOR_LAYOUT_UNCLUSTERED) != 0;
  if constexpr (LAYOUT == NESVOR_LAYOUT_FEATURE_MAJOR) {
    if (unclustered && (hints & NESVOR_LAYOUT_DY_SCRATCH) && (stages & 1))
      return launch_bwd_owner<F, NESVOR_LAYOUT_ROW_MAJOR>(g, u, table, dpe, gt, gu, N, workspace, stages, level_begin, level_end, queue_scale,
                                                          dy_bound, adam, st, hints | 0x10000);
  }
  BwdPlan plan;
  uint64_t n_rec;
  if (!make_plan(g, N, &plan, &n_rec, queue_scale)) return (int)hipErrorInvalidValue;
  plan.level_begin = level_begin; plan.level_end = level_end;
  plan.accumulate_u = (stages & 8) ? 1 : 0;
  const int par = tails_parity(workspace, (stages & 1) && !(stages & 4));
  uint32_t* tails = reinterpret_cast<uint32_t*>(reinterpret_cast<char*>(workspace) + (par ? kTailBytes : 0));
  uint32_t* tails_next = reinterpret_cast<uint32_t*>(reinterpret_cast<char*>(workspace) + (par ? 0 : kTailBytes));
  uint32_t* records = reinterpret_cast<uint32_t*>(reinterpret_cast<char*>(workspace) + kHeadBytes);
  uint8_t* order = reinterpret_cast<uint8_t*>(records) + n_rec * (1 + F) * sizeof(uint32_t);
  const int order_mode = (stages & 4) ? 2 : 1;
  uint32_t* const perm_buf = reinterpret_cast<uint32_t*>((reinterpret_cast<uintptr_t>(order) + (uintptr_t)((N + 255) / 256) * 256 + 255) & ~(uintptr_t)255);
  const uint32_t* const perm = unclustered ? perm_buf : nullptr;
  dim3 grid((unsigned)((N + 255) / 256)), block(256);
  hipError_t e;
  int dy_by_slot = 0;
  if (!(stages & 1)) goto owner_stage;
  if (unclustered && order_mode == 1) {
    const int se = sort_points(u, N, perm_buf, st);
    if (se) return se;
  }
  if (hints & 0x10000) {
    const int E = g->n_levels * F;
    float* rows = reinterpret_cast<float*>(reinterpret_cast<char*>(perm_buf) + ((sort_bytes(N) + 255) & ~(uint64_t)255));
    if (order_mode == 1) {
      const size_t lds = sizeof(float) * kGatherPts * (E + 1);
      if (lds > 48 * 1024) {
        static std::mutex mu;
        static size_t raised = 0;
        std::lock_guard<std::mutex> lock(mu);
        if (lds > raised) {
          e = hipFuncSetAttribute(reinterpret_cast<const void*>(gather_dy_rows_kernel), hipFuncAttributeMaxDynamicSharedMemorySize, (int)lds);
          if (e != hipSuccess) return (int)e;
          raised = lds;
        }
      }
      hipLaunchKernelGGL(gather_dy_rows_kernel, dim3((unsigned)((N + kGatherPts - 1) / kGatherPts)), dim3(256), lds, st, dpe,
                         sort_bufs(perm_buf, N, sort_plan(N)), rows, N, E);
    }
    dpe = rows;
    dy_by_slot = 1;
  }
  {
    static const bool merge = []() { const char* e = getenv("NESVOR_HASHGRID_MERGE"); return e == nullptr || atoi(e) != 0; }();
#define NESVOR_LAUNCH_AGG(IG, MG, BD)                                                                                     \
    hipLaunchKernelGGL((hashgrid_bwd_aggregate<F, LAYOUT, IG, MG, BD>), grid, block, 0, st, *g, plan, u, table, dpe, gt, gu, \
                       tails, tails_next, records, N, dy_bound, order, order_mode, perm, dy_by_slot)
    const bool bounded = dy_bound != nullptr && merge;
    if (gu != nullptr) { if (bounded) NESVOR_LAUNCH_AGG(true, true, true); else if (merge) NESVOR_LAUNCH_AGG(true, true, false); else NESVOR_LAUNCH_AGG(true, false, false); }
    else { if (bounded) NESVOR_LAUNCH_AGG(false, true, true); else if (merge) NESVOR_LAUNCH_AGG(false, true, false); else NESVOR_LAUNCH_AGG(false, false, false); }
#undef NESVOR_LAUNCH_AGG
  }
  e = hipGetLastError();
  if (e != hipSuccess) return (int)e;
owner_stage:
  if (stages & 2) {
    static const int coalesced = []() { const char* e = getenv("NESVOR_OWNER_COALESCED"); return e == nullptr ? 1 : atoi(e); }();
    OwnerAdam oa{};
    static const uint32_t want = []() { const char* e = getenv("NESVOR_OWNER_STRIDE"); return e ? (uint32_t)atoi(e) : 1u; }();
    const uint32_t wg_base = NESVOR_OWNER_FINE_FIRST ? 0u : owner_grid(g, plan, 0, plan.level_begin);
    const uint32_t og = NESVOR_OWNER_FINE_FIRST ? owner_grid(g, plan) : owner_grid(g, plan, plan.level_begin, plan.level_end);
    if (og == 0u) return (int)hipGetLastError();
    uint32_t id_stride = want < 1u ? 1u : want;
    auto gcd = [](uint32_t a, uint32_t b) { while (b) { const uint32_t t = a % b; a = b; b = t; } return a; };
    while (id_stride > 1u && gcd(id_stride, og) != 1u) ++id_stride;
    if (adam != nullptr) {
      oa = *adam;
      oa.done = reinterpret_cast<uint32_t*>(reinterpret_cast<char*>(workspace) + 2 * kTailBytes);
      hipLaunchKernelGGL((hashgrid_bwd_owner<F, true, true>), dim3(og), dim3(kOwnerThreads), 0, st, *g, plan, tails, records, gt, oa, id_stride, wg_base);
    } else if (coalesced)
      hipLaunchKernelGGL((hashgrid_bwd_owner<F, true>), dim3(og), dim3(kOwnerThreads), 0, st, *g, plan, tails, records, gt, oa, id_stride, wg_base);
    else
      hipLaunchKernelGGL((hashgrid_bwd_owner<F, false>), dim3(og), dim3(kOwnerThreads), 0, st, *g, plan, tails, records, gt, oa, id_stride, wg_base);
  }
  return (int)hipGetLastError();
}

inline uint64_t fwd_ws_bytes(const nesvor_grid_t* g, int64_t N, int layout) {
  const uint64_t n_pad = (uint64_t)((N + 255) / 256) * 256;
  uint64_t b = 256 + ((sort_bytes(N) + 255) & ~(uint64_t)255);
  if ((layout & NESVOR_LAYOUT_MASK) == NESVOR_LAYOUT_FEATURE_MAJOR) b += n_pad * (uint64_t)(g->n_levels * g->n_features) * sizeof(float);
  return b;
}
template <int F, int LAYOUT>
int launch_fwd_unclustered(const nesvor_grid_t* g, const float* u, const float* table, float* pe, int64_t N, float* pe_absmax,
                           void* workspace, hipStream_t st) {
  uint32_t* const perm_buf = reinterpret_cast<uint32_t*>((reinterpret_cast<uintptr_t>(workspace) + 255) & ~(uintptr_t)255);
  const int se = sort_points(u, N, perm_buf, st);
  if (se) return se;
  float* rows = nullptr;
  const int E = g->n_levels * F;
  if constexpr (LAYOUT == NESVOR_LAYOUT_FEATURE_MAJOR)
    rows = reinterpret_cast<float*>(reinterpret_cast<char*>(perm_buf) + ((sort_bytes(N) + 255) & ~(uint64_t)255));
  hipLaunchKernelGGL((hashgrid_fwd_cloud<F, LAYOUT>), dim3((unsigned)((N + 255) / 256)), dim3(256), 0, st, *g, u, table, pe, N, pe_absmax,
                     (const uint32_t*)perm_buf, rows);
  if constexpr (LAYOUT == NESVOR_LAYOUT_FEATURE_MAJOR) {
    const size_t lds = sizeof(float) * kGatherPts * (E + 1);
    if (lds > 48 * 1024) {
      static std::mutex mu;
      static size_t raised = 0;
      std::lock_guard<std::mutex> lock(mu);
      if (lds > raised) {
        const hipError_t e = hipFuncSetAttribute(reinterpret_cast<const void*>(scatter_pe_rows_kernel), hipFuncAttributeMaxDynamicSharedMemorySize, (int)lds);
        if (e != hipSuccess) return (int)e;
        raised = lds;
      }
    }
    hipLaunchKernelGGL(scatter_pe_rows_kernel, dim3((unsigned)((N + kGatherPts - 1) / kGatherPts)), dim3(256), lds, st, rows,
                       sort_bufs(perm_buf, N, sort_plan(N)), pe, N, E);
  }
  return (int)hipGetLastError();
}

template <int F, int LAYOUT>
int launch_fwd(const nesvor_grid_t* g, const float* u, const float* table, float* pe, int64_t N, int clustered, float* pe_absmax, hipStream_t st) {
  static const int forced = []() {
    const char* e = getenv("NESVOR_HASHGRID_FWD");
    if (e == nullptr) return -1;
    return e[0] == 'c' ? 0 : (e[0] == 'g' ? 2 : 1);
  }();
  const int mode = forced >= 0 ? forced : (clustered ? 0 : 1);
  if (mode == 0) {
    hipLaunchKernelGGL((hashgrid_fwd_cloud<F, LAYOUT>), dim3((unsigned)((N + 255) / 256)), dim3(256), 0, st, *g, u, table, pe, N, pe_absmax);
    return (int)hipGetLastError();
  }
  dim3 grid((unsigned)((N + 255) / 256), g->n_levels), block(256);
  hipLaunchKernelGGL((hashgrid_fwd<F, LAYOUT>), grid, block, 0, st, *g, u, table, pe, N, mode == 1 ? 1 : 0, pe_absmax);
  return (int)hipGetLastError();
}

template <int F, int LAYOUT>
int launch_bwd(const nesvor_grid_t* g, const float* u, const float* table, const float* dpe, float* gt, float* gu,
               int64_t N, hipStream_t st) {
  dim3 grid((unsigned)((N + 255) / 256), g->n_levels), block(256);
  if (gu != nullptr) {
    hipError_t e = hipMemsetAsync(gu, 0, sizeof(float) * 3 * N, st);
    if (e != hipSuccess) return (int)e;
    hipLaunchKernelGGL((hashgrid_bwd<F, LAYOUT, true, true>), grid, block, 0, st, *g, u, table, dpe, gt, gu, N);
  } else {
    hipLaunchKernelGGL((hashgrid_bwd<F, LAYOUT, false, true>), grid, block, 0, st, *g, u, table, dpe, gt, gu, N);
  }
  return (int)hipGetLastError();
}

}

#define DISPATCH_F_LAYOUT(FN, ...)                                                              \
  do {                                                                                          \
    const int F_ = grid->n_features;                                                            \
    if (layout == NESVOR_LAYOUT_ROW_MAJOR) {                                                    \
      if (F_ == 1) return FN<1, NESVOR_LAYOUT_ROW_MAJOR>(__VA_ARGS__);                          \
      if (F_ == 2) return FN<2, NESVOR_LAYOUT_ROW_MAJOR>(__VA_ARGS__);                          \
      if (F_ == 4) return FN<4, NESVOR_LAYOUT_ROW_MAJOR>(__VA_ARGS__);                          \
      if (F_ == 8) return FN<8, NESVOR_LAYOUT_ROW_MAJOR>(__VA_ARGS__);                          \
    } else if (layout == NESVOR_LAYOUT_FEATURE_MAJOR) {                                         \
      if (F_ == 1) return FN<1, NESVOR_LAYOUT_FEATURE_MAJOR>(__VA_ARGS__);                      \
      if (F_ == 2) return FN<2, NESVOR_LAYOUT_FEATURE_MAJOR>(__VA_ARGS__);                      \
      if (F_ == 4) return FN<4, NESVOR_LAYOUT_FEATURE_MAJOR>(__VA_ARGS__);                      \
      if (F_ == 8) return FN<8, NESVOR_LAYOUT_FEATURE_MAJOR>(__VA_ARGS__);                      \
    }                                                                                           \
    return (int)hipErrorInvalidValue;                                                           \
  } while (0)

extern "C" int nesvor_hashgrid_forward_bounded(const nesvor_grid_t* grid, const float* u, const float* table, float* pe,
                                               int64_t N, int layout, float* pe_absmax, void* stream) {
  if (N <= 0) return 0;
  if (grid->n_levels <= 0 || grid->n_levels > NESVOR_MAX_LEVELS) return (int)hipErrorInvalidValue;
  const int clustered = (layout & NESVOR_LAYOUT_CLUSTERED) ? 1 : 0;
  layout &= NESVOR_LAYOUT_MASK;
  DISPATCH_F_LAYOUT(launch_fwd, grid, u, table, pe, N, clustered, pe_absmax, (hipStream_t)stream);
}

extern "C" int nesvor_hashgrid_forward(const nesvor_grid_t* grid, const float* u, const float* table, float* pe,
                                       int64_t N, int layout, void* stream) {
  return nesvor_hashgrid_forward_bounded(grid, u, table, pe, N, layout, nullptr, stream);
}

extern "C" int64_t nesvor_hashgrid_forward_workspace_bytes(const nesvor_grid_t* grid, int64_t N, int layout) {
  if (grid == nullptr || N <= 0) return 0;
  if (!(layout & NESVOR_LAYOUT_UNCLUSTERED)) return 0;
  return (int64_t)fwd_ws_bytes(grid, N, layout);
}

extern "C" int nesvor_hashgrid_forward_unclustered(const nesvor_grid_t* grid, const float* u, const float* table, float* pe,
                                                   int64_t N, int layout, float* pe_absmax, void* workspace, int64_t workspace_bytes,
                                                   void* stream) {
  if (N <= 0) return 0;
  if (grid->n_levels <= 0 || grid->n_levels > NESVOR_MAX_LEVELS) return (int)hipErrorInvalidValue;
  if (N >= ((int64_t)1 << 32)) return (int)hipErrorInvalidValue;
  if (workspace == nullptr || workspace_bytes < (int64_t)fwd_ws_bytes(grid, N, layout)) return (int)hipErrorInvalidValue;
  layout &= NESVOR_LAYOUT_MASK;
  DISPATCH_F_LAYOUT(launch_fwd_unclustered, grid, u, table, pe, N, pe_absmax, workspace, (hipStream_t)stream);
}

extern "C" int nesvor_hashgrid_backward_atomic(const nesvor_grid_t* grid, const float* u, const float* table,
                                               const float* dpe, float* grad_table, float* grad_u, int64_t N,
                                               int layout, void* stream) {
  if (N <= 0) return 0;
  if (grid->n_levels <= 0 || grid->n_levels > NESVOR_MAX_LEVELS) return (int)hipErrorInvalidValue;
  layout &= NESVOR_LAYOUT_MASK;
  DISPATCH_F_LAYOUT(launch_bwd, grid, u, table, dpe, grad_table, grad_u, N, (hipStream_t)stream);
}

extern "C" int64_t nesvor_hashgrid_backward_workspace_bytes_ex(const nesvor_grid_t* grid, int64_t N, const float* queue_scale, int layout) {
  int64_t base = nesvor_hashgrid_backward_workspace_bytes(grid, N, queue_scale);
  if (base <= 0) return base;
  if (!(layout & NESVOR_LAYOUT_UNCLUSTERED)) base -= (int64_t)((sort_bytes(N) + 255) & ~(uint64_t)255);
  if ((layout & NESVOR_LAYOUT_MASK) == NESVOR_LAYOUT_FEATURE_MAJOR && (layout & NESVOR_LAYOUT_UNCLUSTERED) && (layout & NESVOR_LAYOUT_DY_SCRATCH))
    return base + 256 + (int64_t)((N + 255) / 256) * 256 * grid->n_levels * grid->n_features * (int64_t)sizeof(float);
  return base;
}

extern "C" int64_t nesvor_hashgrid_backward_workspace_bytes(const nesvor_grid_t* grid, int64_t N, const float* queue_scale) {
  if (N <= 0) return 0;
  BwdPlan plan;
  uint64_t n_rec;
  if (grid->n_levels <= 0 || grid->n_levels > NESVOR_MAX_LEVELS) return -1;
  if (!make_plan(grid, N, &plan, &n_rec, queue_scale)) return -1;
  if (plan.n_buckets > kOverflowBase) return -1;
  return (int64_t)(kHeadBytes + n_rec * (1 + grid->n_features) * sizeof(uint32_t) + (uint64_t)((N + 255) / 256) * 256 + 256 + ((sort_bytes(N) + 255) & ~(uint64_t)255));
}

extern "C" int64_t nesvor_hashgrid_backward_workspace_zero_bytes(void) { return (int64_t)kHeadBytes; }

#if NESVOR_HG_TIMELINE
extern "C" int nesvor_debug_hg_timeline(unsigned long long* dst_host) {
  return (int)hipMemcpyFromSymbol(dst_host, HIP_SYMBOL(g_hg_timeline), sizeof(unsigned long long) * kTlWgs * kTlMarks);
}
#endif

extern "C" int64_t nesvor_hashgrid_backward_overflow_offset(void* workspace) {
  return (int64_t)(tails_parity(workspace, false) ? kTailBytes : 0) + (int64_t)kOverflowBase * (int64_t)sizeof(uint32_t);
}

extern "C" int nesvor_hashgrid_backward(const nesvor_grid_t* grid, const float* u, const float* table,
                                        const float* dpe, float* grad_table, float* grad_u, int64_t N, int layout,
                                        void* workspace, int stages, const float* queue_scale, void* stream) {
  if (N <= 0) return 0;
  if (grid->n_levels <= 0 || grid->n_levels > NESVOR_MAX_LEVELS) return (int)hipErrorInvalidValue;
  if (workspace == nullptr || (stages & 3) == 0) return (int)hipErrorInvalidValue;
  const int hints = layout & (NESVOR_LAYOUT_UNCLUSTERED | NESVOR_LAYOUT_DY_SCRATCH);
  layout &= NESVOR_LAYOUT_MASK;
  DISPATCH_F_LAYOUT(launch_bwd_owner, grid, u, table, dpe, grad_table, grad_u, N, workspace, stages & 3, 0, grid->n_levels,
                    queue_scale, nullptr, nullptr, (hipStream_t)stream, hints);
}

extern "C" int nesvor_hashgrid_backward_levels(const nesvor_grid_t* grid, const float* u, const float* table,
                                               const float* dpe, float* grad_table, float* grad_u, int64_t N, int layout,
                                               void* workspace, int stages, int level_begin, int level_end,
                                               const float* queue_scale, void* stream) {
  if (N <= 0) return 0;
  if (grid->n_levels <= 0 || grid->n_levels > NESVOR_MAX_LEVELS) return (int)hipErrorInvalidValue;
  if (workspace == nullptr || (stages & 3) == 0) return (int)hipErrorInvalidValue;
  if (level_begin < 0 || level_end > grid->n_levels || level_begin >= level_end) return (int)hipErrorInvalidValue;
  const int hints = layout & (NESVOR_LAYOUT_UNCLUSTERED | NESVOR_LAYOUT_DY_SCRATCH);
  layout &= NESVOR_LAYOUT_MASK;
  DISPATCH_F_LAYOUT(launch_bwd_owner, grid, u, table, dpe, grad_table, grad_u, N, workspace, stages, level_begin, level_end,
                    queue_scale, nullptr, nullptr, (hipStream_t)stream, hints);
}

extern "C" int nesvor_hashgrid_backward_bounded(const nesvor_grid_t* grid, const float* u, const float* table,
                                                const float* dpe, float* grad_table, float* grad_u, int64_t N, int layout,
                                                void* workspace, int stages, int level_begin, int level_end,
                                                const float* queue_scale, const float* dy_bound, void* stream) {
  if (N <= 0) return 0;
  if (grid->n_levels <= 0 || grid->n_levels > NESVOR_MAX_LEVELS) return (int)hipErrorInvalidValue;
  if (workspace == nullptr || (stages & 3) == 0) return (int)hipErrorInvalidValue;
  if (level_begin < 0 || level_end > grid->n_levels || level_begin >= level_end) return (int)hipErrorInvalidValue;
  const int hints = layout & (NESVOR_LAYOUT_UNCLUSTERED | NESVOR_LAYOUT_DY_SCRATCH);
  layout &= NESVOR_LAYOUT_MASK;
  DISPATCH_F_LAYOUT(launch_bwd_owner, grid, u, table, dpe, grad_table, grad_u, N, workspace, stages, level_begin, level_end,
                    queue_scale, dy_bound, nullptr, (hipStream_t)stream, hints);
}

extern "C" int nesvor_hashgrid_backward_adamw(const nesvor_grid_t* grid, const float* u, float* table, const float* dpe,
                                              float* grad_table, float* grad_u, int64_t N, int layout, void* workspace,
                                              int stages, const float* queue_scale, const float* dy_bound, float* exp_avg,
                                              float* exp_avg_sq, const nesvor_adamw_t* adam, void* stream) {
  if (grid->n_levels <= 0 || grid->n_levels > NESVOR_MAX_LEVELS) return (int)hipErrorInvalidValue;
  if (N <= 0 || workspace == nullptr || (stages & ~3) != 0 || (stages & 3) == 0) return (int)hipErrorInvalidValue;
  if (table == nullptr || grad_table == nullptr || exp_avg == nullptr || exp_avg_sq == nullptr || adam == nullptr) return (int)hipErrorInvalidValue;
  OwnerAdam oa;
  oa.param = table; oa.exp_avg = exp_avg; oa.exp_avg_sq = exp_avg_sq; oa.done = nullptr;
  oa.a = make_adam_args(adam->lr, adam->beta1, adam->beta2, adam->eps, adam->weight_decay, adam->bias_correction1,
                        adam->bias_correction2, adam->grad_scale);
  const int hints = layout & (NESVOR_LAYOUT_UNCLUSTERED | NESVOR_LAYOUT_DY_SCRATCH);
  layout &= NESVOR_LAYOUT_MASK;
  DISPATCH_F_LAYOUT(launch_bwd_owner, grid, u, table, dpe, grad_table, grad_u, N, workspace, stages, 0, grid->n_levels, queue_scale,
                    dy_bound, &oa, (hipStream_t)stream, hints);
}
```

### nesvor_amd/csrc/step.hip

```cpp
#include <hip/hip_runtime.h>
#include <cstdlib>
#include <cstring>
#include <new>
#include "../../include/nesvor_hip.h"

namespace {

struct StepCtx {
  nesvor_step_t d;
  hipEvent_t ev_agg, ev_owner, ev_sg0, ev_sg1;
  void* wimg = nullptr;
  size_t wimg_stride = 0;
  bool pending_join = false;
  int bias_mean_ranks = 1;
  hipEvent_t bias_mean_event = nullptr;
  unsigned* mean_ticket = nullptr;
  bool timing = false, timed_run = false;
  hipEvent_t t0[NESVOR_STEP_TIMED_SPANS], t1[NESVOR_STEP_TIMED_SPANS];
  bool span_used[NESVOR_STEP_TIMED_SPANS];
};
struct Span {
  StepCtx* c; int k; hipStream_t st;
  Span(StepCtx* c_, int k_, hipStream_t st_) : c(c_->timing ? c_ : nullptr), k(k_), st(st_) {
    if (c != nullptr) { (void)hipEventRecord(c->t0[k], st); c->span_used[k] = true; }
  }
  ~Span() { if (c != nullptr) (void)hipEventRecord(c->t1[k], st); }
};

__global__ __launch_bounds__(256) void mean_partial_kernel(const float* __restrict__ x, int64_t n, float* __restrict__ partial) {
  __shared__ float red[256];
  float s = 0.f;
  for (int64_t i = (int64_t)blockIdx.x * 256 + threadIdx.x; i < n; i += (int64_t)gridDim.x * 256) s += x[i];
  red[threadIdx.x] = s;
  __syncthreads();
  for (int w = 128; w > 0; w >>= 1) {
    if ((int)threadIdx.x < w) red[threadIdx.x] += red[threadIdx.x + w];
    __syncthreads();
  }
  if (threadIdx.x == 0) partial[blockIdx.x] = red[0];
}
__global__ __launch_bounds__(256) void mean_final_kernel(const float* __restrict__ partial, int n_partial, float scale, float* __restrict__ out) {
  __shared__ float red[256];
  red[threadIdx.x] = (int)threadIdx.x < n_partial ? partial[threadIdx.x] : 0.f;
  __syncthreads();
  for (int w = 128; w > 0; w >>= 1) {
    if ((int)threadIdx.x < w) red[threadIdx.x] += red[threadIdx.x + w];
    __syncthreads();
  }
  if (threadIdx.x == 0) out[0] = red[0] * scale;
}

__global__ __launch_bounds__(256) void mean_share_kernel(const float* __restrict__ x, int64_t n, int64_t n4, float scale, float* partial,
                                                         unsigned* ticket, float* __restrict__ out) {
  __shared__ float red[256];
  __shared__ unsigned arrived;
  const int t = (int)threadIdx.x;
  const int64_t stride = (int64_t)gridDim.x * 256;
  float s = 0.f;
  const float4* x4 = reinterpret_cast<const float4*>(x);
  for (int64_t i = (int64_t)blockIdx.x * 256 + t; i < n4; i += stride) {
    const float4 q = x4[i];
    s += (q.x + q.y) + (q.z + q.w);
  }
  for (int64_t i = 4 * n4 + (int64_t)blockIdx.x * 256 + t; i < n; i += stride) s += x[i];
  red[t] = s;
  __syncthreads();
  for (int w = 128; w > 0; w >>= 1) {
    if (t < w) red[t] += red[t + w];
    __syncthreads();
  }
  if (t == 0) {
    __hip_atomic_store(&partial[blockIdx.x], red[0], __ATOMIC_RELAXED, __HIP_MEMORY_SCOPE_AGENT);
    arrived = __hip_atomic_fetch_add(ticket, 1u, __ATOMIC_ACQ_REL, __HIP_MEMORY_SCOPE_AGENT);
  }
  __syncthreads();
  if (arrived != gridDim.x - 1) return;
  __atomic_thread_fence(__ATOMIC_ACQUIRE);
  red[t] = t < (int)gridDim.x ? __hip_atomic_load(&partial[t], __ATOMIC_RELAXED, __HIP_MEMORY_SCOPE_AGENT) : 0.f;
  __syncthreads();
  for (int w = 128; w > 0; w >>= 1) {
    if (t < w) red[t] += red[t + w];
    __syncthreads();
  }
  if (t == 0) {
    out[0] = red[0] * scale;
    __hip_atomic_store(ticket, 0u, __ATOMIC_RELAXED, __HIP_MEMORY_SCOPE_AGENT);
  }
}

__global__ __launch_bounds__(256) void add_inplace_kernel(float* __restrict__ dst, const float* __restrict__ src, int64_t n) {
  const int64_t i = ((int64_t)blockIdx.x * 256 + threadIdx.x) * 4;
  if (i + 3 < n) {
    float4 a = *reinterpret_cast<float4*>(dst + i);
    const float4 b = *reinterpret_cast<const float4*>(src + i);
    a.x += b.x; a.y += b.y; a.z += b.z; a.w += b.w;
    *reinterpret_cast<float4*>(dst + i) = a;
  } else {
    for (int64_t k = i; k < n; ++k) dst[k] += src[k];
  }
}

__global__ void square_kernel(const float* __restrict__ m, float* __restrict__ out) { out[0] = m[0] * m[0]; }

#define NESVOR_TRY(expr)            \
  do {                              \
    const int e_ = (int)(expr);     \
    if (e_ != 0) return e_;         \
  } while (0)

int mlp_backward_into(const nesvor_mlp_t& net, int group_sums, const float* xa, const float* xb, const float* dy,
                      float* const* saved, float* dxa, float* dxb, float* partial, int64_t N, hipStream_t st, float* const* dpre_scratch, float* dxb_absmax = nullptr) {
  nesvor_mlp_t d = net;
  d.dxa_group_sums = group_sums;
  float* no_scratch[NESVOR_MAX_MLP_LAYERS] = {nullptr, nullptr, nullptr, nullptr};
  if (!nesvor_mlp_backward_fused_ok(&d, N)) {
    for (int l = 0; l < d.n_hidden; ++l) {
      if (dpre_scratch == nullptr || dpre_scratch[l] == nullptr) return (int)hipErrorInvalidValue;
      no_scratch[l] = dpre_scratch[l];
    }
  }
  return nesvor_mlp_backward_bounded(&d, xa, xb, dy, saved, no_scratch, dxa, dxb, partial, NESVOR_STEP_MLP_PARTIALS, N, dxb_absmax, st);
}

bool bias_free_refused(const nesvor_mlp_t& n) {
  bool any_null = false;
  for (int l = 0; l <= n.n_hidden && l < NESVOR_MAX_MLP_LAYERS; ++l) any_null = any_null || n.bias[l] == nullptr;
  return any_null && n.bf16_operands != NESVOR_MLP_MODE_FP16_SCALED;
}
bool bias_free_refused(const nesvor_step_t& d) {
  return bias_free_refused(d.density) || (d.has_lv && bias_free_refused(d.sigma)) || (d.has_b && bias_free_refused(d.bias_net));
}

}

extern "C" void* nesvor_step_create(const nesvor_step_t* desc) {
  if (desc == nullptr) return nullptr;
  if (bias_free_refused(*desc)) return nullptr;
  StepCtx* c = new (std::nothrow) StepCtx;
  if (c == nullptr) return nullptr;
  c->d = *desc;
  hipEvent_t* evs[4] = {&c->ev_agg, &c->ev_owner, &c->ev_sg0, &c->ev_sg1};
  for (hipEvent_t* e : evs) {
    if (hipEventCreateWithFlags(e, hipEventDisableTiming) != hipSuccess) { delete c; return nullptr; }
  }
  for (int k = 0; k < NESVOR_STEP_TIMED_SPANS; ++k) { c->t0[k] = nullptr; c->t1[k] = nullptr; c->span_used[k] = false; }
  {
    int64_t need = nesvor_mlp_weight_images_bytes(&desc->density);
    if (desc->has_lv && nesvor_mlp_weight_images_bytes(&desc->sigma) > need) need = nesvor_mlp_weight_images_bytes(&desc->sigma);
    if (desc->has_b && nesvor_mlp_weight_images_bytes(&desc->bias_net) > need) need = nesvor_mlp_weight_images_bytes(&desc->bias_net);
    c->wimg_stride = ((size_t)need + 255) / 256 * 256;
    if (need > 0 && hipMalloc(&c->wimg, 3 * c->wimg_stride) != hipSuccess) { c->wimg = nullptr; (void)hipGetLastError(); }
  }
  if (desc->has_b) {
    if (hipMalloc(reinterpret_cast<void**>(&c->mean_ticket), sizeof(unsigned)) != hipSuccess) { c->mean_ticket = nullptr; (void)hipGetLastError(); }
    else if (hipMemset(c->mean_ticket, 0, sizeof(unsigned)) != hipSuccess) { (void)hipFree(c->mean_ticket); c->mean_ticket = nullptr; (void)hipGetLastError(); }
  }
  return c;
}

extern "C" int nesvor_step_timing(void* handle, int on) {
  if (handle == nullptr) return (int)hipErrorInvalidValue;
  StepCtx* c = static_cast<StepCtx*>(handle);
  if (on && c->t0[0] == nullptr) {
    for (int k = 0; k < NESVOR_STEP_TIMED_SPANS; ++k)
      if (hipEventCreate(&c->t0[k]) != hipSuccess || hipEventCreate(&c->t1[k]) != hipSuccess) return (int)hipGetLastError();
  }
  c->timing = on != 0;
  c->timed_run = false;
  return 0;
}
extern "C" int nesvor_step_timing_read(void* handle, float* ms) {
  if (handle == nullptr || ms == nullptr) return (int)hipErrorInvalidValue;
  StepCtx* c = static_cast<StepCtx*>(handle);
  for (int k = 0; k < NESVOR_STEP_TIMED_SPANS; ++k) ms[k] = -1.f;
  if (!c->timed_run) return 0;
  for (int k = 0; k < NESVOR_STEP_TIMED_SPANS; ++k) {
    if (!c->span_used[k]) continue;
    if (hipEventSynchronize(c->t1[k]) != hipSuccess || hipEventElapsedTime(&ms[k], c->t0[k], c->t1[k]) != hipSuccess) return (int)hipGetLastError();
  }
  return 0;
}

extern "C" int nesvor_step_update(void* handle, const nesvor_step_t* desc) {
  if (handle == nullptr || desc == nullptr) return (int)hipErrorInvalidValue;
  if (bias_free_refused(*desc)) return (int)hipErrorInvalidValue;
  static_cast<StepCtx*>(handle)->d = *desc;
  return 0;
}

extern "C" int nesvor_step_set_bias_mean_ranks(void* handle, int ranks) {
  if (handle == nullptr) return (int)hipErrorInvalidValue;
  static_cast<StepCtx*>(handle)->bias_mean_ranks = ranks > 0 ? ranks : 1;
  return 0;
}
extern "C" int nesvor_step_set_bias_mean_event(void* handle, void* event) {
  if (handle == nullptr) return (int)hipErrorInvalidValue;
  static_cast<StepCtx*>(handle)->bias_mean_event = (hipEvent_t)event;
  return 0;
}

extern "C" void nesvor_step_destroy(void* handle) {
  if (handle == nullptr) return;
  StepCtx* c = static_cast<StepCtx*>(handle);
  (void)hipEventDestroy(c->ev_agg); (void)hipEventDestroy(c->ev_owner); (void)hipEventDestroy(c->ev_sg0); (void)hipEventDestroy(c->ev_sg1);
  if (c->wimg != nullptr) (void)hipFree(c->wimg);
  if (c->mean_ticket != nullptr) (void)hipFree(c->mean_ticket);
  for (int k = 0; k < NESVOR_STEP_TIMED_SPANS; ++k) {
    if (c->t0[k] != nullptr) (void)hipEventDestroy(c->t0[k]);
    if (c->t1[k] != nullptr) (void)hipEventDestroy(c->t1[k]);
  }
  delete c;
}

extern "C" int nesvor_step_run(void* handle, const float* xyz, const float* v, const int64_t* slice_idx, uint64_t seed,
                               uint64_t offset, float* losses, int phase, int split_level, const nesvor_adamw_t* adam,
                               void* stream) {
  if (handle == nullptr || xyz == nullptr || v == nullptr || slice_idx == nullptr || losses == nullptr) return (int)hipErrorInvalidValue;
  StepCtx* ctx = static_cast<StepCtx*>(handle);
  const nesvor_step_t& d = ctx->d;
  hipStream_t main = (hipStream_t)stream, side = (hipStream_t)d.side_stream;
  const int B = d.B, S = d.S, n = d.n_slices, L = d.grid.n_levels;
  const int64_t N = (int64_t)B * S;
  const bool defer_join = (phase & NESVOR_STEP_DEFER_JOIN) != 0;
  const bool bias_stop = (phase & NESVOR_STEP_BIAS_SUM_STOP) != 0, bias_resume = (phase & NESVOR_STEP_BIAS_SUM_RESUME) != 0;
  phase &= ~(NESVOR_STEP_DEFER_JOIN | NESVOR_STEP_BIAS_SUM_STOP | NESVOR_STEP_BIAS_SUM_RESUME);
  if (phase < 0 || phase > 2 || (phase != 0) != (split_level > 0 && split_level < L)) return (int)hipErrorInvalidValue;
  if ((bias_stop || bias_resume) && (!d.has_b || phase == 2 || (bias_stop && bias_resume) || ctx->mean_ticket == nullptr))
    return (int)hipErrorInvalidValue;
  float* c = d.has_c ? d.small : nullptr;
  float* mat = d.small + n;
  float* acc = d.small + 13 * n;
  float* dc = acc;
  float* dmat = acc + n;
  float* dpe_bound = d.has_b ? nullptr : d.small + 26 * n;
  float* prep_d = d.small + 26 * n + 1;
  float* prep_s = prep_d + NESVOR_MLP_PREP_FLOATS;
  float* prep_b = prep_s + NESVOR_MLP_PREP_FLOATS;
  nesvor_mlp_t net_d = d.density, net_s = d.sigma, net_b = d.bias_net;
  net_d.prep = prep_d; net_s.prep = prep_s; net_b.prep = prep_b;
  net_d.y_absmax = d.has_lv ? prep_s + NESVOR_MLP_PREP_XB : nullptr;
  void* wimg_d = ctx->wimg;
  void* wimg_s = ctx->wimg != nullptr ? static_cast<char*>(ctx->wimg) + ctx->wimg_stride : nullptr;
  void* wimg_b = ctx->wimg != nullptr ? static_cast<char*>(ctx->wimg) + 2 * ctx->wimg_stride : nullptr;
  net_d.weight_images = nesvor_mlp_weight_images_bytes(&net_d) > 0 ? wimg_d : nullptr;
  net_s.weight_images = (d.has_lv && nesvor_mlp_weight_images_bytes(&net_s) > 0) ? wimg_s : nullptr;
  net_b.weight_images = (d.has_b && nesvor_mlp_weight_images_bytes(&net_b) > 0) ? wimg_b : nullptr;
  auto scaled = [](const nesvor_mlp_t& n_) { return n_.bf16_operands == NESVOR_MLP_MODE_SPLIT || n_.bf16_operands == NESVOR_MLP_MODE_FP16_SCALED; };
  const bool split_d = scaled(net_d), split_s = d.has_lv && scaled(net_s), split_b = d.has_b && scaled(net_b);
  const int layout = NESVOR_LAYOUT_FEATURE_MAJOR;
  const bool overlap_owner = (d.overlap_owner & 1) != 0;
  const int64_t table_off = d.table - d.flat_param;
  const bool fuse_adamw = adam != nullptr && phase == 0 && (d.overlap_owner & 2) != 0 && d.table != nullptr && d.flat_param != nullptr &&
                          d.g_table == d.flat_grad + table_off && table_off >= 0 && table_off < d.flat_numel;

  const int group_sums_s = (d.has_lv && nesvor_mlp_backward_fused_ok(&net_s, N)) ? 1 : 0;
  const int group_sums_b = (d.has_b && nesvor_mlp_backward_fused_ok(&net_b, N)) ? 1 : 0;
  const int rows_pp_s = group_sums_s ? S / 16 : S, rows_pp_b = group_sums_b ? S / 16 : S;
  const bool first_is_sigma = d.has_lv && d.ks;
  const float* dxa_first = first_is_sigma ? d.dxa : ((d.has_b && d.ks) ? d.dxa_b : nullptr);
  const int rows_pp_first = first_is_sigma ? rows_pp_s : rows_pp_b;
  auto slice_grads = [&](const float* dc_pix, const float* dlvs_pix, const float* dxa, int rows_per_pixel, const float* dpix, float* dc_,
                         float* dlvs_, float* dse_, float* dmat_, hipStream_t st_) -> int {
    static const bool by_slice = []() { const char* e = getenv("NESVOR_SLICE_GRADS"); return e != nullptr && strcmp(e, "by_slice") == 0; }();
    if (by_slice) {
      const int e = nesvor_slice_grads_by_slice(slice_idx, dc_pix, dlvs_pix, dxa, dpix, dc_, dlvs_, dse_, dmat_, B, rows_per_pixel, d.ks, n, st_);
      if (e != (int)hipErrorInvalidValue) return e;
    }
    return nesvor_slice_grads(slice_idx, dc_pix, dlvs_pix, dxa, dpix, dc_, dlvs_, dse_, dmat_, B, rows_per_pixel, d.ks, st_);
  };
  const bool early_sg = overlap_owner && !d.has_b;
  if (ctx->timing && !bias_resume) { for (int k = 0; k < NESVOR_STEP_TIMED_SPANS; ++k) ctx->span_used[k] = false; ctx->timed_run = true; }
  auto bias_forward = [&](bool share) -> int {
    if (split_b) NESVOR_TRY(nesvor_mlp_prepare(&net_b, d.se, d.pe, nullptr, N, prep_b, NESVOR_MLP_WHAT_INPUT, main));
    NESVOR_TRY(nesvor_mlp_forward(&net_b, d.se, d.pe, d.log_bias, d.saved_b, N, main));
    if (share) {
      const int64_t n4 = (reinterpret_cast<uintptr_t>(d.log_bias) % 16 == 0) ? N / 4 : 0;
      const int64_t blocks = (N + 1023) / 1024;
      hipLaunchKernelGGL(mean_share_kernel, dim3((unsigned)(blocks < 1 ? 1 : (blocks > 256 ? 256 : blocks))), dim3(256), 0, main, d.log_bias, N, n4,
                         1.f / ((float)N * (float)ctx->bias_mean_ranks), d.mean_scratch, ctx->mean_ticket, d.lb_mean);
    } else {
      hipLaunchKernelGGL(mean_partial_kernel, dim3(256), dim3(256), 0, main, d.log_bias, N, d.mean_scratch);
      hipLaunchKernelGGL(mean_final_kernel, dim3(1), dim3(256), 0, main, d.mean_scratch, 256, 1.f / (float)N, d.lb_mean);
    }
    return 0;
  };
  if (phase != 2) {
   if (!bias_resume) {
    NESVOR_TRY(nesvor_step_prologue_pose(d.has_c ? d.logit_coef : nullptr, c, d.axisangle, mat, acc, 13 * n + 1 + 3 * NESVOR_MLP_PREP_FLOATS, n,
                                         d.opt_T ? d.axisangle_init : nullptr, d.opt_T ? d.trans_terms : nullptr,
                                         d.opt_T ? d.g_trans : nullptr, main));
    const bool any_split = split_d || split_s || split_b;
    if (any_split) {
      const nesvor_mlp_t* nets[3]; float* preps[3]; void* imgs[3]; int nn = 0;
      if (split_d) { nets[nn] = &net_d; imgs[nn] = const_cast<void*>(net_d.weight_images); preps[nn++] = prep_d; }
      if (split_s) { nets[nn] = &net_s; imgs[nn] = const_cast<void*>(net_s.weight_images); preps[nn++] = prep_s; }
      if (split_b) { nets[nn] = &net_b; imgs[nn] = const_cast<void*>(net_b.weight_images); preps[nn++] = prep_b; }
      const bool se_bound = split_s && d.ks > 0;
      NESVOR_TRY(nesvor_mlp_prepare_weights_images(nets, preps, imgs, nn, se_bound ? d.slice_embedding : nullptr, (int64_t)n * d.ks,
                                                   se_bound ? prep_s + NESVOR_MLP_PREP_XA : nullptr, main));
    }
    {
      Span t(ctx, NESVOR_STEP_SPAN_PSF_FWD, main);
      NESVOR_TRY(nesvor_psf_transform_forward_rng_gather(mat, slice_idx, xyz, d.psf_sigma, seed, offset, d.bounding_box, d.x, d.u, B, S,
                                                         d.ks > 0 ? d.slice_embedding : nullptr, d.ks > 0 ? d.se : nullptr, d.ks, main));
    }
    if (ctx->pending_join) {
      if (hipStreamWaitEvent(main, ctx->ev_owner, 0) != hipSuccess) return (int)hipGetLastError();
      ctx->pending_join = false;
    }
    {
      Span t(ctx, NESVOR_STEP_SPAN_HASHGRID_FWD, main);
      NESVOR_TRY(nesvor_hashgrid_forward_bounded(&d.grid, d.u, d.table, d.pe, N, layout | (S >= 128 ? NESVOR_LAYOUT_CLUSTERED : 0),
                                                 split_d ? prep_d + NESVOR_MLP_PREP_XB : nullptr, main));
    }
   }
    if (bias_stop) {
      NESVOR_TRY(bias_forward(true));
      return (int)hipGetLastError();
    }
    {
      Span t(ctx, NESVOR_STEP_SPAN_MLP_FWD_DENSITY, main);
      NESVOR_TRY(nesvor_mlp_forward(&net_d, nullptr, d.pe, d.z, d.saved_d, N, main));
    }
    if (d.has_b && !bias_resume) NESVOR_TRY(bias_forward(false));
    if (d.has_lv) {
      Span t(ctx, NESVOR_STEP_SPAN_MLP_FWD_SIGMA, main);
      NESVOR_TRY(nesvor_mlp_forward(&net_s, d.se, d.z, d.log_var, d.saved_s, N, main));
    }
    if (bias_resume) {
      hipEvent_t exchanged = ctx->bias_mean_event;
      ctx->bias_mean_event = nullptr;
      if (exchanged != nullptr && hipStreamWaitEvent(main, exchanged, 0) != hipSuccess) return (int)hipGetLastError();
    }
    const int z_rows = 1 + d.n_features_z, written = 1 + (d.has_lv ? d.n_features_z : 0);
    if (written < z_rows) {
      if (hipMemsetAsync(d.dz + (size_t)written * N, 0, sizeof(float) * (size_t)(z_rows - written) * N, main) != hipSuccess) return (int)hipGetLastError();
    }
    nesvor_loss_t la;
    std::memset(&la, 0, sizeof(la));
    la.z0 = d.z; la.log_var = d.has_lv ? d.log_var : nullptr; la.log_bias = d.has_b ? d.log_bias : nullptr;
    la.x = d.x; la.v = v; la.slice_idx = slice_idx; la.c = c; la.log_var_slice = d.has_lvs ? d.log_var_slice : nullptr;
    la.log_bias_mean = d.has_b ? d.lb_mean : nullptr;
    la.gw = d.gw; la.loss_pix = d.loss_pix; la.dz0 = d.dz; la.dlog_var = d.has_lv ? d.dlv : nullptr;
    la.dlog_bias = d.has_b ? d.dlb : nullptr; la.dx = d.opt_T ? d.dxl : nullptr;
    la.dc_pix = d.has_c ? d.pix : nullptr; la.dlvs_pix = d.has_lvs ? d.pix + B : nullptr;
    la.B = B; la.S = S; la.reg_type = d.reg_type; la.delta = d.delta;
    la.dz0_absmax = prep_d + NESVOR_MLP_PREP_DY; la.dlog_var_absmax = prep_s + NESVOR_MLP_PREP_DY; la.dlog_bias_absmax = prep_b + NESVOR_MLP_PREP_DY;
    {
      Span t(ctx, NESVOR_STEP_SPAN_LOSS, main);
      NESVOR_TRY(nesvor_imaging_loss(&la, main));
    }
    int widest = d.n_density_params;
    if (d.has_lv && d.n_sigma_params > widest) widest = d.n_sigma_params;
    if (d.has_b && d.n_bias_params > widest) widest = d.n_bias_params;
    float* part_d = d.partial;
    float* part_s = d.partial + (size_t)NESVOR_STEP_MLP_PARTIALS * widest;
    float* part_b = d.partial + 2 * (size_t)NESVOR_STEP_MLP_PARTIALS * widest;
    if (d.has_lv) {
      Span t(ctx, NESVOR_STEP_SPAN_MLP_BWD_SIGMA, main);
      NESVOR_TRY(mlp_backward_into(net_s, group_sums_s, d.se, d.z, d.dlv, d.saved_s, d.ks ? d.dxa : nullptr, d.dz + N, part_s, N, main,
                                   d.dpre_scratch, prep_d + NESVOR_MLP_PREP_DY));
    }
    if (early_sg) {
      if (hipEventRecord(ctx->ev_sg0, main) != hipSuccess || hipStreamWaitEvent(side, ctx->ev_sg0, 0) != hipSuccess) return (int)hipGetLastError();
      NESVOR_TRY(slice_grads(d.has_c ? d.pix : nullptr, d.has_lvs ? d.pix + B : nullptr, (d.has_lv && d.ks) ? d.dxa : nullptr, rows_pp_s, nullptr, dc,
                             d.has_lvs ? d.g_log_var_slice : nullptr, d.ks ? d.g_slice_embedding : nullptr, nullptr, side));
      if (hipEventRecord(ctx->ev_sg1, side) != hipSuccess) return (int)hipGetLastError();
    }
    {
      Span t(ctx, NESVOR_STEP_SPAN_MLP_BWD_DENSITY, main);
      NESVOR_TRY(mlp_backward_into(net_d, 0, nullptr, d.pe, d.dz, d.saved_d, nullptr, d.dpe, part_d, N, main, d.dpre_scratch, dpe_bound));
    }
    if (d.has_b) {
      NESVOR_TRY(mlp_backward_into(net_b, group_sums_b, d.se, d.pe, d.dlb, d.saved_b, d.ks ? d.dxa_b : nullptr, d.dpe_b, part_b, N, main,
                                   d.dpre_scratch));
      const int64_t nb = (int64_t)d.kb_bias * N;
      hipLaunchKernelGGL(add_inplace_kernel, dim3((unsigned)((nb / 4 + 255) / 256 + 1)), dim3(256), 0, main, d.dpe, d.dpe_b, nb);
    }
    {
      const float* in[3]; float* out[3]; int cols[3], n_jobs = 0;
      in[n_jobs] = part_d; out[n_jobs] = d.g_density; cols[n_jobs++] = d.n_density_params;
      if (d.has_lv) { in[n_jobs] = part_s; out[n_jobs] = d.g_sigma; cols[n_jobs++] = d.n_sigma_params; }
      if (d.has_b) { in[n_jobs] = part_b; out[n_jobs] = d.g_bias_net; cols[n_jobs++] = d.n_bias_params; }
      NESVOR_TRY(nesvor_sum_rows_multi(in, out, cols, cols, n_jobs, NESVOR_STEP_MLP_PARTIALS, main));
    }
  }
  float* du = d.opt_T ? d.du : nullptr;
  if (phase == 0) {
    {
      Span t(ctx, NESVOR_STEP_SPAN_HASHGRID_BWD_AGGREGATE, main);
      NESVOR_TRY(nesvor_hashgrid_backward_bounded(&d.grid, d.u, d.table, d.dpe, d.g_table, du, N, layout, d.hg_workspace, 1, 0, L,
                                                  d.queue_scale, dpe_bound, main));
    }
    hipStream_t owner_stream = main;
    if (overlap_owner) {
      if (hipEventRecord(ctx->ev_agg, main) != hipSuccess || hipStreamWaitEvent(side, ctx->ev_agg, 0) != hipSuccess) return (int)hipGetLastError();
      owner_stream = side;
    }
    {
      Span t(ctx, NESVOR_STEP_SPAN_HASHGRID_BWD_OWNER, owner_stream);
      if (fuse_adamw)
        NESVOR_TRY(nesvor_hashgrid_backward_adamw(&d.grid, d.u, d.flat_param + table_off, d.dpe, d.g_table, du, N, layout, d.hg_workspace, 2,
                                                  d.queue_scale, dpe_bound, d.flat_exp_avg + table_off, d.flat_exp_avg_sq + table_off, adam,
                                                  owner_stream));
      else
        NESVOR_TRY(nesvor_hashgrid_backward_levels(&d.grid, d.u, d.table, d.dpe, d.g_table, du, N, layout, d.hg_workspace, 2, 0, L,
                                                   d.queue_scale, owner_stream));
    }
    if (overlap_owner && hipEventRecord(ctx->ev_owner, side) != hipSuccess) return (int)hipGetLastError();
  } else if (phase == 1) {
    return nesvor_hashgrid_backward_bounded(&d.grid, d.u, d.table, d.dpe, d.g_table, du, N, layout, d.hg_workspace, 3, split_level, L,
                                            d.queue_scale, dpe_bound, main);
  } else {
    NESVOR_TRY(nesvor_hashgrid_backward_bounded(&d.grid, d.u, d.table, d.dpe, d.g_table, du, N, layout, d.hg_workspace, 1 | 4 | 8, 0,
                                                split_level, d.queue_scale, dpe_bound, main));
    hipStream_t owner_stream = main;
    if (overlap_owner) {
      if (hipEventRecord(ctx->ev_agg, main) != hipSuccess || hipStreamWaitEvent(side, ctx->ev_agg, 0) != hipSuccess) return (int)hipGetLastError();
      owner_stream = side;
    }
    NESVOR_TRY(nesvor_hashgrid_backward_bounded(&d.grid, d.u, d.table, d.dpe, d.g_table, du, N, layout, d.hg_workspace, 2 | 4 | 8, 0,
                                                split_level, d.queue_scale, dpe_bound, owner_stream));
    if (overlap_owner && hipEventRecord(ctx->ev_owner, side) != hipSuccess) return (int)hipGetLastError();
  }
  if (d.opt_T) {
    Span t(ctx, NESVOR_STEP_SPAN_PSF_BWD, main);
    if (early_sg)
      NESVOR_TRY(nesvor_psf_transform_backward_rng_slices(mat, slice_idx, xyz, d.psf_sigma, seed, offset, d.bounding_box, d.dxl, du, nullptr, dmat, B, S, main));
    else
      NESVOR_TRY(nesvor_psf_transform_backward_rng(mat, slice_idx, xyz, d.psf_sigma, seed, offset, d.bounding_box, d.dxl, du, d.dpix, B, S, main));
  }
  if (early_sg) {
    if (hipStreamWaitEvent(main, ctx->ev_sg1, 0) != hipSuccess) return (int)hipGetLastError();
  } else {
    NESVOR_TRY(slice_grads(d.has_c ? d.pix : nullptr, d.has_lvs ? d.pix + B : nullptr, dxa_first, rows_pp_first, d.opt_T ? d.dpix : nullptr, dc,
                           d.has_lvs ? d.g_log_var_slice : nullptr, d.ks ? d.g_slice_embedding : nullptr, dmat, main));
    if (d.has_lv && d.has_b && d.ks)
      NESVOR_TRY(slice_grads(nullptr, nullptr, d.dxa_b, rows_pp_b, nullptr, nullptr, nullptr, d.g_slice_embedding, nullptr, main));
  }
  const float img_scale = (d.reg_type == 0 ? d.delta : 1.f) / (float)N, img_off = d.reg_type == 0 ? -d.delta : 0.f;
  NESVOR_TRY(nesvor_step_epilogue(d.has_c ? dc : nullptr, c, d.has_c ? d.g_logit_coef : nullptr, d.opt_T ? dmat : nullptr, d.axisangle,
                                  d.opt_T ? d.g_trans : nullptr, d.w_T, d.opt_T ? d.g_axisangle : nullptr, d.loss_pix,
                                  d.opt_T ? d.trans_terms : nullptr, losses, n, B, img_scale, img_off, main));
  if (d.has_b) hipLaunchKernelGGL(square_kernel, dim3(1), dim3(1), 0, main, d.lb_mean, losses + 5);
  if (adam != nullptr) {
    if (fuse_adamw) {
      NESVOR_TRY(nesvor_adamw_step(d.flat_param, d.flat_grad, d.flat_exp_avg, d.flat_exp_avg_sq, table_off, adam->lr, adam->beta1, adam->beta2,
                                   adam->eps, adam->weight_decay, adam->bias_correction1, adam->bias_correction2, adam->grad_scale, 1, main));
      const int64_t table_end = (table_off + (int64_t)(d.grid.offset[L - 1] + d.grid.size[L - 1]) * d.grid.n_features + 3) / 4 * 4;
      if (table_end < d.flat_numel)
        NESVOR_TRY(nesvor_adamw_step(d.flat_param + table_end, d.flat_grad + table_end, d.flat_exp_avg + table_end, d.flat_exp_avg_sq + table_end,
                                     d.flat_numel - table_end, adam->lr, adam->beta1, adam->beta2, adam->eps, adam->weight_decay,
                                     adam->bias_correction1, adam->bias_correction2, adam->grad_scale, 1, main));
      if (overlap_owner) {
        if (defer_join) ctx->pending_join = true;
        else if (hipStreamWaitEvent(main, ctx->ev_owner, 0) != hipSuccess) return (int)hipGetLastError();
      }
    } else {
      if (phase != 1 && overlap_owner && hipStreamWaitEvent(main, ctx->ev_owner, 0) != hipSuccess) return (int)hipGetLastError();
      NESVOR_TRY(nesvor_adamw_step(d.flat_param, d.flat_grad, d.flat_exp_avg, d.flat_exp_avg_sq, d.flat_numel, adam->lr, adam->beta1, adam->beta2,
                                   adam->eps, adam->weight_decay, adam->bias_correction1, adam->bias_correction2, adam->grad_scale, 1, main));
    }
  }
  return (int)hipGetLastError();
}

extern "C" int nesvor_step_join(void* handle, void* stream) {
  if (handle == nullptr) return (int)hipErrorInvalidValue;
  StepCtx* ctx = static_cast<StepCtx*>(handle);
  if (ctx->pending_join) {
    if (hipStreamWaitEvent((hipStream_t)stream, ctx->ev_owner, 0) != hipSuccess) return (int)hipGetLastError();
    ctx->pending_join = false;
  }
  return 0;
}
```

### nesvor_amd/encoding.py

```python
import ctypes

import torch
from torch.autograd import Function

from . import _lib
from .grid import HashGridSpec


_FWD_WS = {}
UNCLUSTERED_FWD_MIN_POINTS = 1 << 15
_FWD_MODE = __import__("os").environ.get("NESVOR_HASHGRID_FWD", "")


def hashgrid_forward(spec: HashGridSpec, u: torch.Tensor, table: torch.Tensor, layout=_lib.LAYOUT_ROW_MAJOR, clustered=False):
    _lib.require_device(u, table, dtype=torch.float32, name="hashgrid input/table")
    N = u.shape[0]
    E = spec.n_output_dims
    shape = (N, E) if layout == _lib.LAYOUT_ROW_MAJOR else (E, N)
    pe = torch.empty(shape, dtype=torch.float32, device=u.device)
    lib = _lib.load()
    ordered = ((not clustered and layout == _lib.LAYOUT_ROW_MAJOR and N >= UNCLUSTERED_FWD_MIN_POINTS and _FWD_MODE == "")
               or (_FWD_MODE == "sorted" and N > 0))
    with torch.cuda.device(u.device), _lib.kernel_timer.span("hashgrid_fwd"):
        if ordered:
            lay = layout | _lib.LAYOUT_UNCLUSTERED
            nbytes = lib.nesvor_hashgrid_forward_workspace_bytes(ctypes.byref(spec.c_struct), N, lay)
            ws = _FWD_WS.get(u.device)
            if ws is None or ws.numel() < nbytes:
                ws = _FWD_WS[u.device] = torch.empty(nbytes, dtype=torch.uint8, device=u.device)
            err = lib.nesvor_hashgrid_forward_unclustered(ctypes.byref(spec.c_struct), _lib.ptr(u), _lib.ptr(table), _lib.ptr(pe), N, lay,
                                                          None, _lib.ptr(ws), ws.numel(), _lib.stream_ptr())
        else:
            err = lib.nesvor_hashgrid_forward(
                ctypes.byref(spec.c_struct), _lib.ptr(u), _lib.ptr(table), _lib.ptr(pe), N,
                layout | (_lib.LAYOUT_CLUSTERED if clustered else 0), _lib.stream_ptr()
            )
    _lib.check(err, "hashgrid forward")
    return pe


def points_are_ordered(u: torch.Tensor, box_fraction: float = 1.0 / 16) -> bool:
    n = min(int(u.shape[0]), 4096)
    if n < 2:
        return False
    step = (u[1:n] - u[: n - 1]).abs().amax(-1)
    return bool(step.median() < box_fraction)


_WORKSPACES = {}


class QueueSizer:

    START = 1.0 / 16
    policy = __import__("os").environ.get("NESVOR_HASHGRID_QUEUE", "adaptive")

    def __init__(self, n_levels: int, key=None) -> None:
        start = 1.0 if QueueSizer.policy == "worst" else QueueSizer.START
        self.scale = (ctypes.c_float * _lib.MAX_LEVELS)(*([start] * _lib.MAX_LEVELS))
        if QueueSizer.policy.startswith("load:") and key is not None:
            import json, os

            path = QueueSizer.policy[5:]
            saved = json.load(open(path)).get(_key_name(key)) if os.path.exists(path) else None
            if saved is not None:
                for l, v in enumerate(saved[: _lib.MAX_LEVELS]):
                    self.scale[l] = min(1.0, max(QueueSizer.START, float(v)))
        self.n_levels = n_levels
        self.calls = 0
        self.pending = None
        self.host = None

    def poll(self) -> bool:
        if self.pending is None or not self.pending.query():
            return False
        counts = self.host.tolist()
        self.pending = None
        grown = False
        for l in range(self.n_levels):
            if counts[l] > 0 and self.scale[l] < 1.0:
                self.scale[l] = min(1.0, self.scale[l] * 4)
                grown = True
        return grown

    def snapshot(self, ws: torch.Tensor) -> None:
        self.calls += 1
        if QueueSizer.policy == "worst" or self.pending is not None or not (self.calls <= 64 or self.calls % 4 == 0):
            return
        if all(self.scale[l] >= 1.0 for l in range(self.n_levels)):
            return
        off = _lib.load().nesvor_hashgrid_backward_overflow_offset(_lib.ptr(ws))
        if self.host is None:
            self.host = torch.empty(_lib.MAX_LEVELS, dtype=torch.int32, pin_memory=True)
            self.stream = torch.cuda.Stream(device=ws.device)
        self.stream.wait_stream(torch.cuda.current_stream(ws.device))
        with torch.cuda.stream(self.stream):
            self.host.copy_(ws[off : off + 4 * _lib.MAX_LEVELS].view(torch.int32), non_blocking=True)
            self.pending = torch.cuda.Event()
            self.pending.record()


_SIZERS = {}


def _key_name(key) -> str:
    return "/".join(str(k) for k in key[1:])


def save_queue_scales(path: str) -> None:
    import json

    with open(path, "w") as f:
        json.dump({_key_name(k): [float(v) for v in sz.scale] for k, sz in _SIZERS.items()}, f)


def queue_sizer(spec, N, device, clustered=True) -> QueueSizer:
    key = (device, N, spec.n_levels, spec.n_features, spec.log2_hashmap_size, spec.base_resolution, spec.per_level_scale, bool(clustered))
    sz = _SIZERS.get(key)
    if sz is None:
        sz = _SIZERS[key] = QueueSizer(spec.n_levels, key)
    return sz


def _workspace(spec, N, device, sizer=None, layout=0):
    sizer = sizer or queue_sizer(spec, N, device)
    nbytes = _lib.load().nesvor_hashgrid_backward_workspace_bytes_ex(ctypes.byref(spec.c_struct), N, sizer.scale, layout)
    if nbytes < 0:
        return None
    key = (device, nbytes)
    ws = _WORKSPACES.get(key)
    if ws is None:
        stale = [k for k in _WORKSPACES if k[0] == device]
        if stale:
            torch.cuda.synchronize(device)
        for k in stale:
            del _WORKSPACES[k]
        ws = torch.empty(nbytes, dtype=torch.uint8, device=device)
        ws[: _lib.load().nesvor_hashgrid_backward_workspace_zero_bytes()].zero_()
        _WORKSPACES[key] = ws
    return ws


def hashgrid_backward(spec, u, table, dpe, grad_table=None, need_input_grad=True, layout=_lib.LAYOUT_ROW_MAJOR,
                      method="owner", levels=None, grad_u=None, first=True, owner_stream=None, dy_bound=None, clustered=True):
    _lib.require_device(u, table, dpe, dtype=torch.float32, name="hashgrid backward input")
    if not clustered:
        layout = layout | _lib.LAYOUT_UNCLUSTERED | _lib.LAYOUT_DY_SCRATCH
    N = u.shape[0]
    if grad_table is None:
        grad_table = torch.zeros_like(table)
    if grad_u is None:
        if not first and need_input_grad:
            raise RuntimeError("a later part of a split backward needs the first part's grad_u")
        grad_u = torch.empty_like(u) if need_input_grad else None
    lib = _lib.load()
    sizer = queue_sizer(spec, N, u.device, clustered) if method == "owner" else None
    if sizer is not None and first:
        sizer.poll()
    ws = _workspace(spec, N, u.device, sizer, layout) if method == "owner" else None
    if levels is not None and ws is None:
        raise RuntimeError("level ranges exist for the owner method only")
    with torch.cuda.device(u.device):
        if ws is not None:
            args = (ctypes.byref(spec.c_struct), _lib.ptr(u), _lib.ptr(table), _lib.ptr(dpe), _lib.ptr(grad_table),
                    _lib.ptr(grad_u), N, layout, _lib.ptr(ws))
            l0, l1 = (0, spec.n_levels) if levels is None else levels
            extra = 0 if first else (4 | 8)
            call = lambda stage: lib.nesvor_hashgrid_backward_bounded(*args, stage | extra, l0, l1, sizer.scale, _lib.ptr(dy_bound),
                                                                      _lib.stream_ptr())
            if _lib.kernel_timer.enabled:
                with _lib.kernel_timer.span("hashgrid_bwd_aggregate"):
                    err = call(1)
                if err == 0:
                    with _lib.kernel_timer.span("hashgrid_bwd_owner"):
                        err = call(2)
            elif owner_stream is not None:
                err = call(1)
                if err == 0:
                    owner_stream.wait_stream(torch.cuda.current_stream(u.device))
                    err = lib.nesvor_hashgrid_backward_bounded(*args, 2 | extra, l0, l1, sizer.scale, _lib.ptr(dy_bound),
                                                               ctypes.c_void_p(owner_stream.cuda_stream))
            else:
                err = call(3)
        else:
            err = lib.nesvor_hashgrid_backward_atomic(
                ctypes.byref(spec.c_struct), _lib.ptr(u), _lib.ptr(table), _lib.ptr(dpe), _lib.ptr(grad_table),
                _lib.ptr(grad_u), N, layout, _lib.stream_ptr(),
            )
    _lib.check(err, "hashgrid backward")
    if sizer is not None and ws is not None:
        sizer.snapshot(ws)
    return grad_table, grad_u


def hashgrid_backward_adamw(spec, u, table, dpe, grad_table, exp_avg, exp_avg_sq, adam, need_input_grad=True,
                            layout=_lib.LAYOUT_ROW_MAJOR, dy_bound=None):
    _lib.require_device(u, table, dpe, grad_table, exp_avg, exp_avg_sq, dtype=torch.float32, name="hashgrid backward + AdamW input")
    N = u.shape[0]
    grad_u = torch.empty_like(u) if need_input_grad else None
    lib = _lib.load()
    sizer = queue_sizer(spec, N, u.device)
    sizer.poll()
    ws = _workspace(spec, N, u.device, sizer)
    if ws is None:
        raise RuntimeError("the grid does not fit the owner method's plan")
    with torch.cuda.device(u.device):
        err = lib.nesvor_hashgrid_backward_adamw(ctypes.byref(spec.c_struct), _lib.ptr(u), _lib.ptr(table), _lib.ptr(dpe), _lib.ptr(grad_table),
                                                 _lib.ptr(grad_u), N, layout, _lib.ptr(ws), 3, sizer.scale, _lib.ptr(dy_bound),
                                                 _lib.ptr(exp_avg), _lib.ptr(exp_avg_sq), ctypes.byref(adam), _lib.stream_ptr())
    _lib.check(err, "hashgrid backward + AdamW")
    sizer.snapshot(ws)
    return grad_u


def hashgrid_encode(u, table, spec, layout=_lib.LAYOUT_ROW_MAJOR, grad_accum=None):
    cfg = (spec.n_levels, spec.n_features, spec.log2_hashmap_size, spec.base_resolution, spec.per_level_scale, layout)
    if grad_accum is None:
        return torch.ops.nesvor.hashgrid_encode(u.contiguous(), table, *cfg)
    return _AccumulatingEncode.apply(u.contiguous(), table, cfg, grad_accum)


class _AccumulatingEncode(Function):

    @staticmethod
    def forward(ctx, u, table, cfg, grad_accum):
        ctx.save_for_backward(u, table)
        ctx.cfg, ctx.grad_accum = cfg, grad_accum
        with torch.no_grad():
            return torch.ops.nesvor.hashgrid_encode(u, table, *cfg)

    @staticmethod
    def backward(ctx, dpe):
        u, table = ctx.saved_tensors
        gu = torch.ops.nesvor.hashgrid_encode_backward_(u, table, dpe.contiguous(), ctx.grad_accum, *ctx.cfg, ctx.needs_input_grad[0])
        return (gu if ctx.needs_input_grad[0] else None), None, None, None
```

Measured before the change: 1063.

## Hand the forward pass's point sort and cloud plan to the hashgrid backward

The hashgrid forward now computes the Morton-key bitonic sort order and per-block lattice box and round schedule records, and writes them to device buffers. The backward aggregate kernel reads these instead of recomputing the sort, the bounding box reductions and the schedule. This removes duplicated sorting and planning work in the backward pass. In exchange the forward does extra work and writes extra memory, and the handover depends on the points being unchanged between forward and backward.

After: 1076 (median of 6 runs). 1.01x the previous value.

```diff
diff --git a/include/nesvor_hip.h b/include/nesvor_hip.h
--- a/include/nesvor_hip.h
+++ b/include/nesvor_hip.h
@@ -124,6 +124,15 @@
                                      float* grad_table, float* grad_u, int64_t N, int layout, void* workspace, int stages,
                                      int level_begin, int level_end, const float* queue_scale, const float* dy_bound,
                                      void* stream);
+int64_t nesvor_hashgrid_cloud_order_bytes(int64_t N);
+int64_t nesvor_hashgrid_cloud_plan_bytes(const nesvor_grid_t* grid, int64_t N);
+int64_t nesvor_hashgrid_backward_order_offset(const nesvor_grid_t* grid, int64_t N, const float* queue_scale);
+int nesvor_hashgrid_forward_plan(const nesvor_grid_t* grid, const float* u, const float* table, float* pe, int64_t N, int layout,
+                                 float* pe_absmax, void* order, void* cloud_plan, const float* queue_scale, void* stream);
+int nesvor_hashgrid_backward_plan(const nesvor_grid_t* grid, const float* u, const float* table, const float* dpe,
+                                  float* grad_table, float* grad_u, int64_t N, int layout, void* workspace, int stages,
+                                  int level_begin, int level_end, const float* queue_scale, const float* dy_bound,
+                                  const void* order, const void* cloud_plan, void* stream);
 int nesvor_hashgrid_backward_atomic(const nesvor_grid_t* grid, const float* u, const float* table, const float* dpe,
                                     float* grad_table, float* grad_u, int64_t N, int layout, void* stream);
 
diff --git a/nesvor_amd/_lib.py b/nesvor_amd/_lib.py
--- a/nesvor_amd/_lib.py
+++ b/nesvor_amd/_lib.py
@@ -138,6 +138,11 @@
     "nesvor_hashgrid_backward_levels": ([POINTER(GridT), _P, _P, _P, _P, _P, c_int64, c_int, _P, c_int, c_int, c_int, _P, _P], c_int),
     "nesvor_hashgrid_backward_bounded": ([POINTER(GridT), _P, _P, _P, _P, _P, c_int64, c_int, _P, c_int, c_int, c_int, _P, _P, _P], c_int),
     "nesvor_hashgrid_backward_atomic": ([POINTER(GridT), _P, _P, _P, _P, _P, c_int64, c_int, _P], c_int),
+    "nesvor_hashgrid_cloud_order_bytes": ([c_int64], c_int64),
+    "nesvor_hashgrid_cloud_plan_bytes": ([POINTER(GridT), c_int64], c_int64),
+    "nesvor_hashgrid_backward_order_offset": ([POINTER(GridT), c_int64, _P], c_int64),
+    "nesvor_hashgrid_forward_plan": ([POINTER(GridT), _P, _P, _P, c_int64, c_int, _P, _P, _P, _P, _P], c_int),
+    "nesvor_hashgrid_backward_plan": ([POINTER(GridT), _P, _P, _P, _P, _P, c_int64, c_int, _P, c_int, c_int, c_int, _P, _P, _P, _P, _P], c_int),
     "nesvor_psf_transform_forward": ([_P] * 8 + [c_int, c_int, _P], c_int),
     "nesvor_psf_transform_backward": ([_P] * 9 + [c_int, c_int, _P], c_int),
     "nesvor_psf_transform_forward_rng_gather": ([_P] * 4 + [c_uint64, c_uint64] + [_P] * 3 + [c_int, c_int, _P, _P, c_int, _P], c_int),
diff --git a/nesvor_amd/csrc/hashgrid.hip b/nesvor_amd/csrc/hashgrid.hip
--- a/nesvor_amd/csrc/hashgrid.hip
+++ b/nesvor_amd/csrc/hashgrid.hip
@@ -98,6 +98,80 @@
   return c;
 }
 
+template <int K, int J>
+__device__ __forceinline__ void bitonic_merge(uint32_t& sv, int tid, uint32_t* sortbuf) {
+  uint32_t other;
+  if constexpr (J < 64) {
+    other = lane_xor_u32<J>(sv, tid & 63);
+  } else {
+    __syncthreads();
+    sortbuf[tid] = sv;
+    __syncthreads();
+    other = sortbuf[tid ^ J];
+  }
+  const bool keep_min = ((tid & K) == 0) == ((tid & J) == 0);
+  sv = keep_min ? min(sv, other) : max(sv, other);
+  if constexpr (J > 1) bitonic_merge<K, J / 2>(sv, tid, sortbuf);
+}
+template <int K>
+__device__ __forceinline__ void bitonic_sort(uint32_t& sv, int tid, uint32_t* sortbuf) {
+  if constexpr (K > 2) bitonic_sort<K / 2>(sv, tid, sortbuf);
+  bitonic_merge<K, K / 2>(sv, tid, sortbuf);
+}
+
+__device__ __forceinline__ uint32_t spread3(uint32_t x) {
+  x &= 0xffu;
+  x = (x ^ (x << 8)) & 0x0300f00fu;
+  x = (x ^ (x << 4)) & 0x030c30c3u;
+  x = (x ^ (x << 2)) & 0x09249249u;
+  return x;
+}
+
+__device__ __forceinline__ uint32_t cloud_sort_key(const nesvor_grid_t& g, bool in_range, float ux, float uy, float uz, int tid) {
+  uint32_t code = 0x00ffffffu;
+  if (in_range) {
+    const LevelParams pf = load_level(g, g.n_levels - 1);
+    const CellPos c = locate(pf, ux, uy, uz);
+    code = spread3(c.gx) | (spread3(c.gy) << 1) | (spread3(c.gz) << 2);
+  }
+  return (code << 8) | (uint32_t)tid;
+}
+
+__device__ __forceinline__ void lattice_box(const LevelParams& p, const float (&ulo)[3], const float (&uhi)[3], bool boxes_on, uint32_t max_slots,
+                                            uint32_t (&b)[8]) {
+  const CellPos blo = locate(p, ulo[0], ulo[1], ulo[2]), bhi = locate(p, uhi[0], uhi[1], uhi[2]);
+  const uint32_t ex = bhi.gx - blo.gx, ey = bhi.gy - blo.gy, ez = bhi.gz - blo.gz;
+  const bool fits = boxes_on && ex < max_slots && ey < max_slots && ez < max_slots &&
+                    (uint64_t)(ex + 2u) * (ey + 2u) * (ez + 2u) <= (uint64_t)max_slots;
+  const uint32_t nx = ex + 2u, nxy = nx * (ey + 2u), vol = fits ? nxy * (ez + 2u) : 0u;
+  b[0] = blo.gx; b[1] = blo.gy; b[2] = blo.gz; b[3] = ex; b[4] = ey; b[5] = ez; b[6] = vol;
+  b[7] = fits ? vol - 2u - nx - nxy : 0u;
+}
+__device__ __forceinline__ uint32_t window_bits(uint32_t ex, uint32_t ey, uint32_t ez, int log2_slots) {
+  const uint32_t vx = min(ex, 1023u) + 2u, vy = min(ey, 1023u) + 2u, vz = min(ez, 1023u) + 2u;
+  uint32_t ba = 0, bb = 0, bc = 0;
+  for (int n = 0; n < log2_slots; ++n) {
+    const uint32_t rx = (vx << 12) >> ba, ry = (vy << 12) >> bb, rz = (vz << 12) >> bc;
+    if (rz >= rx && rz >= ry) ++bc;
+    else if (ry >= rx) ++bb;
+    else ++ba;
+  }
+  return ba | (bb << 8) | (bc << 16);
+}
+
+#ifndef NESVOR_HG_SLOTS
+#define NESVOR_HG_SLOTS 1024
+#endif
+constexpr int kMaxChunks = 256;
+constexpr int kAggMaxGroup = 8;
+template <int F> constexpr int agg_slots() { return F <= 2 ? NESVOR_HG_SLOTS : (F == 4 ? 512 : 256); }
+__host__ __device__ constexpr uint32_t plan_rows(int L) { return (uint32_t)(L + 4) & ~3u; }
+__host__ __device__ constexpr uint32_t plan_words(int L) { return 8u + 14u * plan_rows(L); }
+struct CloudPlanArgs {
+  uint32_t n_chunks[NESVOR_MAX_LEVELS];
+  uint32_t box_slots;
+};
+
 template <int F>
 __device__ __forceinline__ void load_feat(const float* __restrict__ p, float (&v)[F]) {
   if constexpr (F == 1) {
@@ -247,7 +321,10 @@
                                                           const float* __restrict__ table, float* __restrict__ pe, int64_t N,
                                                           float* __restrict__ pe_absmax,
                                                           const uint32_t* __restrict__ perm = nullptr, float* __restrict__ rows = nullptr,
-                                                          int level_begin = 0, int level_stop = NESVOR_MAX_LEVELS) {
+                                                          int level_begin = 0, int level_stop = NESVOR_MAX_LEVELS,
+                                                          uint8_t* __restrict__ order = nullptr,
+                                                          uint32_t* __restrict__ cloud_plan = nullptr,
+                                                          const CloudPlanArgs cpa = CloudPlanArgs{}) {
 #ifndef NESVOR_FWD_CLOUD_SLOTS
 #define NESVOR_FWD_CLOUD_SLOTS 512
 #endif
@@ -260,6 +337,7 @@
   __shared__ uint32_t lpar[NESVOR_MAX_LEVELS + 1][4];
   __shared__ uint32_t slot_off[NESVOR_MAX_LEVELS + 1], grp_end[NESVOR_MAX_LEVELS + 1], rnd_slots[NESVOR_MAX_LEVELS + 1];
   __shared__ int32_t box_end_s;
+  __shared__ uint32_t sortbuf[256];
   const int tid = threadIdx.x, lane = tid & 63;
   const int64_t slot_i = (int64_t)blockIdx.x * 256 + tid;
   const bool valid = slot_i < N;
@@ -269,6 +347,11 @@
   const int L = g.n_levels, E = L * F;
   const int lb = level_begin, le = min(level_stop, L);
   const float ux = u[3 * ii], uy = u[3 * ii + 1], uz = u[3 * ii + 2];
+  if (order != nullptr) {
+    uint32_t sv = cloud_sort_key(g, valid, ux, uy, uz, tid);
+    bitonic_sort<NESVOR_SORT_SPAN>(sv, tid, sortbuf);
+    order[(int64_t)blockIdx.x * 256 + tid] = (uint8_t)(sv & 255u);
+  }
   {
     float lo[3] = {ux, uy, uz}, hi[3] = {ux, uy, uz};
 #pragma unroll
@@ -289,13 +372,7 @@
     uint32_t b[8] = {0u, 0u, 0u, 0u, 0u, 0u, 0u, 0u};
     if (tid < L) {
       const LevelParams p = load_level(g, tid);
-      const CellPos blo = locate(p, ulo[0], ulo[1], ulo[2]), bhi = locate(p, uhi[0], uhi[1], uhi[2]);
-      const uint32_t ex = bhi.gx - blo.gx, ey = bhi.gy - blo.gy, ez = bhi.gz - blo.gz;
-      const bool fits = ex < (uint32_t)kSlots && ey < (uint32_t)kSlots && ez < (uint32_t)kSlots &&
-                        (uint64_t)(ex + 2u) * (ey + 2u) * (ez + 2u) <= (uint64_t)kSlots;
-      const uint32_t nx = ex + 2u, nxy = nx * (ey + 2u), vol = fits ? nxy * (ez + 2u) : 0u;
-      b[0] = blo.gx; b[1] = blo.gy; b[2] = blo.gz; b[3] = ex; b[4] = ey; b[5] = ez; b[6] = vol;
-      b[7] = fits ? vol - 2u - nx - nxy : 0u;
+      lattice_box(p, ulo, uhi, true, (uint32_t)kSlots, b);
       lpar[tid][0] = p.res; lpar[tid][1] = p.size; lpar[tid][2] = p.offset; lpar[tid][3] = p.hashed;
     }
     if (tid <= L) {
@@ -305,6 +382,40 @@
     const RoundSchedule rs = round_schedule(b[6], 0u, lb, le, tid, (uint32_t)kSlots, 0xFFFFFFFFu, kMaxGroup);
     if (tid == 0) box_end_s = rs.box_end;
     if (tid < NESVOR_MAX_LEVELS) { slot_off[tid] = rs.slot_off; grp_end[tid] = rs.grp_end; rnd_slots[tid] = rs.rnd_slots; }
+  } else if (tid < 128 && cloud_plan != nullptr) {
+    if constexpr (F <= 2) {
+      const int lv = tid - 64;
+      float ulo[3], uhi[3];
+#pragma unroll
+      for (int d = 0; d < 3; ++d) {
+        ulo[d] = fminf(fminf(ubox[0][d], ubox[1][d]), fminf(ubox[2][d], ubox[3][d]));
+        uhi[d] = fmaxf(fmaxf(ubox[0][3 + d], ubox[1][3 + d]), fmaxf(ubox[2][3 + d], ubox[3][3 + d]));
+      }
+      constexpr uint32_t kAggSlots = (uint32_t)agg_slots<F>();
+      uint32_t b[8] = {0u, 0u, 0u, 0u, 0u, 0u, 0u, 0u};
+      uint32_t win = 0u, nch = 0u;
+      if (lv < L) {
+        const LevelParams p = load_level(g, lv);
+        lattice_box(p, ulo, uhi, cpa.box_slots != 0u, kAggSlots, b);
+        win = window_bits(b[3], b[4], b[5], __builtin_ctz(kAggSlots));
+        nch = cpa.n_chunks[lv];
+      }
+      const RoundSchedule rs = round_schedule(b[6], nch, 0, L, lv, kAggSlots, (uint32_t)kMaxChunks, kAggMaxGroup);
+      const uint32_t R = plan_rows(L);
+      uint32_t* rec = cloud_plan + (size_t)blockIdx.x * plan_words(L);
+      if (lv == 0) {
+        uint4* h = reinterpret_cast<uint4*>(rec);
+        h[0] = make_uint4(__float_as_uint(ulo[0]), __float_as_uint(ulo[1]), __float_as_uint(ulo[2]), __float_as_uint(uhi[0]));
+        h[1] = make_uint4(__float_as_uint(uhi[1]), __float_as_uint(uhi[2]), (uint32_t)rs.box_end, 0u);
+      }
+      if ((uint32_t)lv < R) {
+        uint4* bx = reinterpret_cast<uint4*>(rec + 8 + 8 * lv);
+        bx[0] = make_uint4(b[0], b[1], b[2], b[3]);
+        bx[1] = make_uint4(b[4], b[5], b[6], b[7]);
+        uint32_t* a = rec + 8 + 8 * R + lv;
+        a[0] = win; a[R] = rs.slot_off; a[2 * R] = rs.bkt_off; a[3 * R] = rs.grp_end; a[4 * R] = rs.rnd_slots; a[5 * R] = rs.rnd_bkts;
+      }
+    }
   }
   __syncthreads();
   const int box_end = __builtin_amdgcn_readfirstlane(box_end_s);
@@ -542,7 +653,6 @@
   }
 }
 
-constexpr int kMaxChunks = 256;
 constexpr int kSubQueues = 8;
 constexpr uint32_t kTailStride = 4096;
 constexpr uint32_t kOverflowBase = kTailStride - NESVOR_MAX_LEVELS;
@@ -562,35 +672,6 @@
   int32_t accumulate_u;
 };
 
-template <int K, int J>
-__device__ __forceinline__ void bitonic_merge(uint32_t& sv, int tid, uint32_t* sortbuf) {
-  uint32_t other;
-  if constexpr (J < 64) {
-    other = lane_xor_u32<J>(sv, tid & 63);
-  } else {
-    __syncthreads();
-    sortbuf[tid] = sv;
-    __syncthreads();
-    other = sortbuf[tid ^ J];
-  }
-  const bool keep_min = ((tid & K) == 0) == ((tid & J) == 0);
-  sv = keep_min ? min(sv, other) : max(sv, other);
-  if constexpr (J > 1) bitonic_merge<K, J / 2>(sv, tid, sortbuf);
-}
-template <int K>
-__device__ __forceinline__ void bitonic_sort(uint32_t& sv, int tid, uint32_t* sortbuf) {
-  if constexpr (K > 2) bitonic_sort<K / 2>(sv, tid, sortbuf);
-  bitonic_merge<K, K / 2>(sv, tid, sortbuf);
-}
-
-__device__ __forceinline__ uint32_t spread3(uint32_t x) {
-  x &= 0xffu;
-  x = (x ^ (x << 8)) & 0x0300f00fu;
-  x = (x ^ (x << 4)) & 0x030c30c3u;
-  x = (x ^ (x << 2)) & 0x09249249u;
-  return x;
-}
-
 __device__ __forceinline__ unsigned long long to_fixed(float x) {
   const float t = rintf(x * 0x1p-32f);
   const int32_t lo = __float2int_rn(fmaf(-t, 0x1p32f, x));
@@ -617,9 +698,6 @@
 #define NESVOR_FIXED32 0
 #endif
 
-#ifndef NESVOR_HG_SLOTS
-#define NESVOR_HG_SLOTS 1024
-#endif
 #ifndef NESVOR_HG_MINBLOCKS
 #define NESVOR_HG_MINBLOCKS 4
 #endif
@@ -640,7 +718,7 @@
 #else
 #define HG_TICK(site) do { } while (0)
 #endif
-template <int F, int LAYOUT, bool INPUT_GRAD, bool MERGE, bool BOUND = false>
+template <int F, int LAYOUT, bool INPUT_GRAD, bool MERGE, bool BOUND = false, bool PLAN = false>
 __global__ __launch_bounds__(256, F <= 2 ? NESVOR_HG_MINBLOCKS : (F == 4 ? 3 : 2)) void hashgrid_bwd_aggregate(const nesvor_grid_t g, const BwdPlan plan,
                                                               const float* __restrict__ u,
                                                               const float* __restrict__ table,
@@ -653,7 +731,9 @@
                                                               uint8_t* __restrict__ order,
                                                               int order_mode,
                                                               const uint32_t* __restrict__ perm,
-                                                              int dy_by_slot) {
+                                                              int dy_by_slot,
+                                                              const uint32_t* __restrict__ cloud_plan = nullptr) {
+  static_assert(!PLAN || (MERGE && F <= 2), "the cloud plan exists for the merging pass at F <= 2");
   for (uint32_t t = blockIdx.x * 256u + threadIdx.x; t < (uint32_t)kSubQueues * kTailStride; t += gridDim.x * 256u) tails_next[t] = 0u;
   constexpr bool kPack = (F == 2) && (NESVOR_FIXED32 != 0);
   constexpr bool kPerLevel = kPack && (NESVOR_FIXED32 >= 2);
@@ -663,10 +743,10 @@
   uint4* const bbase4 = reinterpret_cast<uint4*>(bb_raw);
   uint2(*const bbase)[kMaxChunks] = reinterpret_cast<uint2(*)[kMaxChunks]>(bb_raw);
   __shared__ uint32_t sortbuf[256];
-  constexpr int kSlots = F <= 2 ? NESVOR_HG_SLOTS : (F == 4 ? 512 : 256);
+  constexpr int kSlots = agg_slots<F>();
   constexpr uint32_t kEmpty = 0xFFFFFFFFu;
   constexpr uint32_t kKeyMask = (1u << 27) - 1u;
-  constexpr int kMaxGroup = 8;
+  constexpr int kMaxGroup = kAggMaxGroup;
   __shared__ __attribute__((aligned(16))) uint32_t tkeys[kSlots];
   __shared__ __attribute__((aligned(16))) unsigned long long tvals[kSlots * kWords];
   __shared__ __attribute__((aligned(16))) float tcache[INPUT_GRAD && MERGE ? kSlots * F : 1];
@@ -704,16 +784,15 @@
   }
 
   uint32_t sv;
-  {
+  if constexpr (PLAN) sv = (uint32_t)order[base + tid];
+  else {
     const int64_t s0_ = base + tid;
-    uint32_t code = 0x00ffffffu;
+    float kx = 0.f, ky = 0.f, kz = 0.f;
     if (s0_ < N) {
       const int64_t i0 = perm != nullptr ? (int64_t)perm[s0_] : s0_;
-      const LevelParams pf = load_level(g, g.n_levels - 1);
-      const CellPos c = locate(pf, u[3 * i0], u[3 * i0 + 1], u[3 * i0 + 2]);
-      code = spread3(c.gx) | (spread3(c.gy) << 1) | (spread3(c.gz) << 2);
-    }
-    sv = (code << 8) | (uint32_t)tid;
+      kx = u[3 * i0]; ky = u[3 * i0 + 1]; kz = u[3 * i0 + 2];
+    }
+    sv = cloud_sort_key(g, s0_ < N, kx, ky, kz, tid);
     if (order_mode == 2) sv = (uint32_t)order[base + tid];
     else
 #pragma unroll 1
@@ -746,10 +825,12 @@
 
   if constexpr (MERGE) {
     float lo[3] = {ux, uy, uz}, hi[3] = {ux, uy, uz};
-#pragma unroll
-    for (int d = 0; d < 3; ++d) {
-      lo[d] = -wave_max_f32_dpp(-lo[d]);
-      hi[d] = wave_max_f32_dpp(hi[d]);
+    if constexpr (!PLAN) {
+#pragma unroll
+      for (int d = 0; d < 3; ++d) {
+        lo[d] = -wave_max_f32_dpp(-lo[d]);
+        hi[d] = wave_max_f32_dpp(hi[d]);
+      }
     }
     float m = 0.f;
     if constexpr (kPerLevel) __syncthreads();
@@ -783,8 +864,10 @@
     }
     m = wave_max_f32_dpp(m);
     if (lane == 0) {
-#pragma unroll
-      for (int d = 0; d < 3; ++d) { ubox[tid >> 6][d] = lo[d]; ubox[tid >> 6][3 + d] = hi[d]; }
+      if constexpr (!PLAN) {
+#pragma unroll
+        for (int d = 0; d < 3; ++d) { ubox[tid >> 6][d] = lo[d]; ubox[tid >> 6][3 + d] = hi[d]; }
+      }
       gmax[tid >> 6] = m;
     }
   }
@@ -793,12 +876,14 @@
   float ulo[3] = {0.f, 0.f, 0.f}, uhi[3] = {0.f, 0.f, 0.f};
   float fscale = 1.f, finv = 1.f;
   if constexpr (MERGE) {
-#pragma unroll
-    for (int d = 0; d < 3; ++d) {
-      ulo[d] = fminf(fminf(ubox[0][d], ubox[1][d]), fminf(ubox[2][d], ubox[3][d]));
-      uhi[d] = fmaxf(fmaxf(ubox[0][3 + d], ubox[1][3 + d]), fmaxf(ubox[2][3 + d], ubox[3][3 + d]));
-      ulo[d] = __builtin_bit_cast(float, __builtin_amdgcn_readfirstlane(__builtin_bit_cast(int, ulo[d])));
-      uhi[d] = __builtin_bit_cast(float, __builtin_amdgcn_readfirstlane(__builtin_bit_cast(int, uhi[d])));
+    if constexpr (!PLAN) {
+#pragma unroll
+      for (int d = 0; d < 3; ++d) {
+        ulo[d] = fminf(fminf(ubox[0][d], ubox[1][d]), fminf(ubox[2][d], ubox[3][d]));
+        uhi[d] = fmaxf(fmaxf(ubox[0][3 + d], ubox[1][3 + d]), fmaxf(ubox[2][3 + d], ubox[3][3 + d]));
+        ulo[d] = __builtin_bit_cast(float, __builtin_amdgcn_readfirstlane(__builtin_bit_cast(int, ulo[d])));
+        uhi[d] = __builtin_bit_cast(float, __builtin_amdgcn_readfirstlane(__builtin_bit_cast(int, uhi[d])));
+      }
     }
     {
       float mx = 256.f * fmaxf(fmaxf(gmax[0], gmax[1]), fmaxf(gmax[2], gmax[3]));
@@ -809,43 +894,50 @@
       finv = __uint_as_float((uint32_t)(127 - sexp) << 23);
     }
     HG_TICK(6);
-    if (tid < 64) {
+    auto fill_lpar = [&](int lv, const LevelParams& p) __attribute__((always_inline)) {
+      lpar[lv][0] = p.res; lpar[lv][1] = p.size; lpar[lv][2] = p.offset; lpar[lv][3] = p.hashed;
+      lpar[lv][4] = plan.cap[lv]; lpar[lv][5] = plan.bucket_base[lv]; lpar[lv][6] = (uint32_t)plan.rec_off[lv];
+      lpar[lv][7] = plan.shift[lv];
+      if constexpr (kPerLevel) {
+        const float mxl = 256.f * __uint_as_float(lmax_bits[lv]);
+        int se = 29 - ((int)((__float_as_uint(mxl) >> 23) & 0xFFu) - 127);
+        se = se > 100 ? 100 : (se < -100 ? -100 : se);
+        lscale[lv][0] = __uint_as_float((uint32_t)(se + 127) << 23);
+        lscale[lv][1] = __uint_as_float((uint32_t)(127 - se) << 23);
+      }
+    };
+    if constexpr (PLAN) {
+      const uint32_t R = plan_rows(g.n_levels), nq = plan_words(g.n_levels) / 4u, q = 255u - (uint32_t)tid;
+      if (q < nq) {
+        const uint4 w4 = reinterpret_cast<const uint4*>(cloud_plan)[(size_t)blockIdx.x * nq + q];
+        const uint32_t w[4] = {w4.x, w4.y, w4.z, w4.w};
+        if (q < 2u) {
+          if (q == 1u) box_end_s = (int32_t)w[2];
+        } else if (q < 2u + 2u * R) {
+          uint32_t* dst = &lbox[0][0] + (q - 2u) * 4u;
+          if ((q - 2u) * 4u < (uint32_t)(NESVOR_MAX_LEVELS + 1) * 8u) {
+#pragma unroll
+            for (int k = 0; k < 4; ++k) dst[k] = w[k];
+          }
+        } else {
+          const uint32_t qa = q - 2u - 2u * R, a = qa / (R / 4u), r0 = (qa - a * (R / 4u)) * 4u;
+          uint32_t* dst = a == 0u ? lwin : (a == 1u ? slot_off : (a == 2u ? bkt_off : (a == 3u ? grp_end : (a == 4u ? rnd_slots : rnd_bkts))));
+#pragma unroll
+          for (int k = 0; k < 4; ++k)
+            if (r0 + k <= (uint32_t)NESVOR_MAX_LEVELS) dst[r0 + k] = w[k];
+        }
+      }
+      if (tid < g.n_levels) fill_lpar(tid, load_level(g, tid));
+    } else if (tid < 64) {
       uint32_t b[8] = {0u, 0u, 0u, 0u, 0u, 0u, 0u, 0u};
       uint32_t nch = 0u;
-      const LevelParams p = load_level(g, tid < g.n_levels ? tid : 0);
       const int tl_ = tid < g.n_levels ? tid : 0;
-      const uint32_t pl_nch = plan.n_chunks[tl_], pl_cap = plan.cap[tl_], pl_base = plan.bucket_base[tl_], pl_rec = (uint32_t)plan.rec_off[tl_],
-                     pl_shift = plan.shift[tl_];
+      const LevelParams p = load_level(g, tl_);
       if (tid < g.n_levels) {
-        const CellPos blo = locate(p, ulo[0], ulo[1], ulo[2]), bhi = locate(p, uhi[0], uhi[1], uhi[2]);
-        const uint32_t ex = bhi.gx - blo.gx, ey = bhi.gy - blo.gy, ez = bhi.gz - blo.gz;
-        const bool fits = plan.box_slots != 0u && ex < (uint32_t)kSlots && ey < (uint32_t)kSlots && ez < (uint32_t)kSlots &&
-                          (uint64_t)(ex + 2u) * (ey + 2u) * (ez + 2u) <= (uint64_t)kSlots;
-        const uint32_t nx = ex + 2u, nxy = nx * (ey + 2u), vol = fits ? nxy * (ez + 2u) : 0u;
-        b[0] = blo.gx; b[1] = blo.gy; b[2] = blo.gz; b[3] = ex; b[4] = ey; b[5] = ez; b[6] = vol;
-        b[7] = fits ? vol - 2u - nx - nxy : 0u;
-        {
-          const uint32_t vx = min(ex, 1023u) + 2u, vy = min(ey, 1023u) + 2u, vz = min(ez, 1023u) + 2u;
-          uint32_t ba = 0, bb = 0, bc = 0;
-          for (int n = 0; n < __builtin_ctz(kSlots); ++n) {
-            const uint32_t rx = (vx << 12) >> ba, ry = (vy << 12) >> bb, rz = (vz << 12) >> bc;
-            if (rz >= rx && rz >= ry) ++bc;
-            else if (ry >= rx) ++bb;
-            else ++ba;
-          }
-          lwin[tid] = ba | (bb << 8) | (bc << 16);
-        }
-        nch = pl_nch;
-        lpar[tid][0] = p.res; lpar[tid][1] = p.size; lpar[tid][2] = p.offset; lpar[tid][3] = p.hashed;
-        lpar[tid][4] = pl_cap; lpar[tid][5] = pl_base; lpar[tid][6] = pl_rec;
-        lpar[tid][7] = pl_shift;
-        if constexpr (kPerLevel) {
-          const float mxl = 256.f * __uint_as_float(lmax_bits[tid]);
-          int se = 29 - ((int)((__float_as_uint(mxl) >> 23) & 0xFFu) - 127);
-          se = se > 100 ? 100 : (se < -100 ? -100 : se);
-          lscale[tid][0] = __uint_as_float((uint32_t)(se + 127) << 23);
-          lscale[tid][1] = __uint_as_float((uint32_t)(127 - se) << 23);
-        }
+        lattice_box(p, ulo, uhi, plan.box_slots != 0u, (uint32_t)kSlots, b);
+        lwin[tid] = window_bits(b[3], b[4], b[5], __builtin_ctz(kSlots));
+        nch = plan.n_chunks[tl_];
+        fill_lpar(tid, p);
       }
       HG_TICK(7);
       if (tid <= g.n_levels) {
@@ -1903,12 +1995,15 @@
 template <int F, int LAYOUT>
 int launch_bwd_owner(const nesvor_grid_t* g, const float* u, const float* table, const float* dpe, float* gt,
                      float* gu, int64_t N, void* workspace, int stages, int level_begin, int level_end, const float* queue_scale,
-                     const float* dy_bound, const OwnerAdam* adam, hipStream_t st, int hints = 0) {
+                     const float* dy_bound, const OwnerAdam* adam, hipStream_t st, int hints = 0,
+                     const uint8_t* fwd_order = nullptr, const uint32_t* cloud_plan = nullptr) {
   const bool unclustered = (hints & NESVOR_LAYOUT_UNCLUSTERED) != 0;
+  if ((fwd_order != nullptr || cloud_plan != nullptr) && unclustered) return (int)hipErrorInvalidValue;
+  if (cloud_plan != nullptr && (fwd_order == nullptr || F > 2 || level_begin != 0 || level_end != g->n_levels)) return (int)hipErrorInvalidValue;
   if constexpr (LAYOUT == NESVOR_LAYOUT_FEATURE_MAJOR) {
     if (unclustered && (hints & NESVOR_LAYOUT_DY_SCRATCH) && (stages & 1))
       return launch_bwd_owner<F, NESVOR_LAYOUT_ROW_MAJOR>(g, u, table, dpe, gt, gu, N, workspace, stages, level_begin, level_end, queue_scale,
-                                                          dy_bound, adam, st, hints | 0x10000);
+                                                          dy_bound, adam, st, hints | 0x10000, fwd_order, cloud_plan);
   }
   BwdPlan plan;
   uint64_t n_rec;
@@ -1919,22 +2014,23 @@
   uint32_t* tails = reinterpret_cast<uint32_t*>(reinterpret_cast<char*>(workspace) + (par ? kTailBytes : 0));
   uint32_t* tails_next = reinterpret_cast<uint32_t*>(reinterpret_cast<char*>(workspace) + (par ? 0 : kTailBytes));
   uint32_t* records = reinterpret_cast<uint32_t*>(reinterpret_cast<char*>(workspace) + kHeadBytes);
-  uint8_t* order = reinterpret_cast<uint8_t*>(records) + n_rec * (1 + F) * sizeof(uint32_t);
-  const int order_mode = (stages & 4) ? 2 : 1;
-  uint32_t* const perm_buf = reinterpret_cast<uint32_t*>((reinterpret_cast<uintptr_t>(order) + (uintptr_t)((N + 255) / 256) * 256 + 255) & ~(uintptr_t)255);
+  uint8_t* const own_order = reinterpret_cast<uint8_t*>(records) + n_rec * (1 + F) * sizeof(uint32_t);
+  uint8_t* const order = fwd_order != nullptr ? const_cast<uint8_t*>(fwd_order) : own_order;
+  const int order_mode = (fwd_order != nullptr || (stages & 4)) ? 2 : 1;
+  uint32_t* const perm_buf = reinterpret_cast<uint32_t*>((reinterpret_cast<uintptr_t>(own_order) + (uintptr_t)((N + 255) / 256) * 256 + 255) & ~(uintptr_t)255);
   const uint32_t* const perm = unclustered ? perm_buf : nullptr;
   dim3 grid((unsigned)((N + 255) / 256)), block(256);
   hipError_t e;
   int dy_by_slot = 0;
   if (!(stages & 1)) goto owner_stage;
-  if (unclustered && order_mode == 1) {
+  if (unclustered && !(stages & 4)) {
     const int se = sort_points(u, N, perm_buf, st);
     if (se) return se;
   }
   if (hints & 0x10000) {
     const int E = g->n_levels * F;
     float* rows = reinterpret_cast<float*>(reinterpret_cast<char*>(perm_buf) + ((sort_bytes(N) + 255) & ~(uint64_t)255));
-    if (order_mode == 1) {
+    if (!(stages & 4)) {
       const size_t lds = sizeof(float) * kGatherPts * (E + 1);
       if (lds > 48 * 1024) {
         static std::mutex mu;
@@ -1957,8 +2053,21 @@
 #define NESVOR_LAUNCH_AGG(IG, MG, BD)                                                                                     \
     hipLaunchKernelGGL((hashgrid_bwd_aggregate<F, LAYOUT, IG, MG, BD>), grid, block, 0, st, *g, plan, u, table, dpe, gt, gu, \
                        tails, tails_next, records, N, dy_bound, order, order_mode, perm, dy_by_slot)
+#define NESVOR_LAUNCH_AGG_PLAN(IG, BD)                                                                                      \
+    hipLaunchKernelGGL((hashgrid_bwd_aggregate<F, LAYOUT, IG, true, BD, true>), grid, block, 0, st, *g, plan, u, table, dpe, gt, gu, \
+                       tails, tails_next, records, N, dy_bound, order, order_mode, perm, dy_by_slot, cloud_plan)
     const bool bounded = dy_bound != nullptr && merge;
-    if (gu != nullptr) { if (bounded) NESVOR_LAUNCH_AGG(true, true, true); else if (merge) NESVOR_LAUNCH_AGG(true, true, false); else NESVOR_LAUNCH_AGG(true, false, false); }
+    bool planned = false;
+    if constexpr (F <= 2) {
+      if (cloud_plan != nullptr && merge) {
+        planned = true;
+        if (gu != nullptr) { if (bounded) NESVOR_LAUNCH_AGG_PLAN(true, true); else NESVOR_LAUNCH_AGG_PLAN(true, false); }
+        else { if (bounded) NESVOR_LAUNCH_AGG_PLAN(false, true); else NESVOR_LAUNCH_AGG_PLAN(false, false); }
+      }
+    }
+#undef NESVOR_LAUNCH_AGG_PLAN
+    if (planned) { }
+    else if (gu != nullptr) { if (bounded) NESVOR_LAUNCH_AGG(true, true, true); else if (merge) NESVOR_LAUNCH_AGG(true, true, false); else NESVOR_LAUNCH_AGG(true, false, false); }
     else { if (bounded) NESVOR_LAUNCH_AGG(false, true, true); else if (merge) NESVOR_LAUNCH_AGG(false, true, false); else NESVOR_LAUNCH_AGG(false, false, false); }
 #undef NESVOR_LAUNCH_AGG
   }
@@ -2041,6 +2150,23 @@
 }
 
 template <int F, int LAYOUT>
+int launch_fwd_plan(const nesvor_grid_t* g, const float* u, const float* table, float* pe, int64_t N, float* pe_absmax, uint8_t* order,
+                    uint32_t* cloud_plan, const float* queue_scale, hipStream_t st) {
+  CloudPlanArgs cpa{};
+  if (cloud_plan != nullptr) {
+    if (F > 2) return (int)hipErrorInvalidValue;
+    BwdPlan plan;
+    uint64_t n_rec;
+    if (!make_plan(g, N, &plan, &n_rec, queue_scale)) return (int)hipErrorInvalidValue;
+    for (int l = 0; l < NESVOR_MAX_LEVELS; ++l) cpa.n_chunks[l] = plan.n_chunks[l];
+    cpa.box_slots = plan.box_slots;
+  }
+  hipLaunchKernelGGL((hashgrid_fwd_cloud<F, LAYOUT>), dim3((unsigned)((N + 255) / 256)), dim3(256), 0, st, *g, u, table, pe, N, pe_absmax,
+                     (const uint32_t*)nullptr, (float*)nullptr, 0, NESVOR_MAX_LEVELS, order, cloud_plan, cpa);
+  return (int)hipGetLastError();
+}
+
+template <int F, int LAYOUT>
 int launch_bwd(const nesvor_grid_t* g, const float* u, const float* table, const float* dpe, float* gt, float* gu,
                int64_t N, hipStream_t st) {
   dim3 grid((unsigned)((N + 255) / 256), g->n_levels), block(256);
@@ -2184,6 +2310,47 @@
                     queue_scale, dy_bound, nullptr, (hipStream_t)stream, hints);
 }
 
+extern "C" int64_t nesvor_hashgrid_cloud_order_bytes(int64_t N) { return N <= 0 ? 0 : (N + 255) / 256 * 256; }
+
+extern "C" int64_t nesvor_hashgrid_cloud_plan_bytes(const nesvor_grid_t* grid, int64_t N) {
+  if (grid == nullptr || N <= 0 || grid->n_levels <= 0 || grid->n_levels > NESVOR_MAX_LEVELS || grid->n_features > 2) return 0;
+  return (N + 255) / 256 * (int64_t)plan_words(grid->n_levels) * (int64_t)sizeof(uint32_t);
+}
+
+extern "C" int64_t nesvor_hashgrid_backward_order_offset(const nesvor_grid_t* grid, int64_t N, const float* queue_scale) {
+  BwdPlan plan;
+  uint64_t n_rec;
+  if (grid == nullptr || N <= 0 || grid->n_levels <= 0 || grid->n_levels > NESVOR_MAX_LEVELS) return -1;
+  if (!make_plan(grid, N, &plan, &n_rec, queue_scale)) return -1;
+  return (int64_t)(kHeadBytes + n_rec * (1 + grid->n_features) * sizeof(uint32_t));
+}
+
+extern "C" int nesvor_hashgrid_forward_plan(const nesvor_grid_t* grid, const float* u, const float* table, float* pe, int64_t N, int layout,
+                                            float* pe_absmax, void* order, void* cloud_plan, const float* queue_scale, void* stream) {
+  if (N <= 0) return 0;
+  if (grid->n_levels <= 0 || grid->n_levels > NESVOR_MAX_LEVELS) return (int)hipErrorInvalidValue;
+  if (order == nullptr || (reinterpret_cast<uintptr_t>(cloud_plan) & 15u) != 0) return (int)hipErrorInvalidValue;
+  layout &= NESVOR_LAYOUT_MASK;
+  DISPATCH_F_LAYOUT(launch_fwd_plan, grid, u, table, pe, N, pe_absmax, static_cast<uint8_t*>(order), static_cast<uint32_t*>(cloud_plan),
+                    queue_scale, (hipStream_t)stream);
+}
+
+extern "C" int nesvor_hashgrid_backward_plan(const nesvor_grid_t* grid, const float* u, const float* table, const float* dpe,
+                                             float* grad_table, float* grad_u, int64_t N, int layout, void* workspace, int stages,
+                                             int level_begin, int level_end, const float* queue_scale, const float* dy_bound,
+                                             const void* order, const void* cloud_plan, void* stream) {
+  if (N <= 0) return 0;
+  if (grid->n_levels <= 0 || grid->n_levels > NESVOR_MAX_LEVELS) return (int)hipErrorInvalidValue;
+  if (workspace == nullptr || (stages & 3) == 0) return (int)hipErrorInvalidValue;
+  if (level_begin < 0 || level_end > grid->n_levels || level_begin >= level_end) return (int)hipErrorInvalidValue;
+  if ((reinterpret_cast<uintptr_t>(cloud_plan) & 15u) != 0) return (int)hipErrorInvalidValue;
+  const int hints = layout & (NESVOR_LAYOUT_UNCLUSTERED | NESVOR_LAYOUT_DY_SCRATCH);
+  layout &= NESVOR_LAYOUT_MASK;
+  DISPATCH_F_LAYOUT(launch_bwd_owner, grid, u, table, dpe, grad_table, grad_u, N, workspace, stages, level_begin, level_end,
+                    queue_scale, dy_bound, nullptr, (hipStream_t)stream, hints, static_cast<const uint8_t*>(order),
+                    static_cast<const uint32_t*>(cloud_plan));
+}
+
 extern "C" int nesvor_hashgrid_backward_adamw(const nesvor_grid_t* grid, const float* u, float* table, const float* dpe,
                                               float* grad_table, float* grad_u, int64_t N, int layout, void* workspace,
                                               int stages, const float* queue_scale, const float* dy_bound, float* exp_avg,
diff --git a/nesvor_amd/csrc/step.hip b/nesvor_amd/csrc/step.hip
--- a/nesvor_amd/csrc/step.hip
+++ b/nesvor_amd/csrc/step.hip
@@ -11,6 +11,9 @@
   hipEvent_t ev_agg, ev_owner, ev_sg0, ev_sg1;
   void* wimg = nullptr;
   size_t wimg_stride = 0;
+  void* hg_order = nullptr;
+  void* hg_plan = nullptr;
+  int64_t handover_points = 0;
   bool pending_join = false;
   int bias_mean_ranks = 1;
   hipEvent_t bias_mean_event = nullptr;
@@ -131,6 +134,19 @@
   return bias_free_refused(d.density) || (d.has_lv && bias_free_refused(d.sigma)) || (d.has_b && bias_free_refused(d.bias_net));
 }
 
+void size_handover(StepCtx* c) {
+  const nesvor_step_t& d = c->d;
+  const int64_t N = (int64_t)d.B * d.S;
+  if (d.S < 128 || N <= 0 || N == c->handover_points) return;
+  if (c->hg_order != nullptr) (void)hipFree(c->hg_order);
+  if (c->hg_plan != nullptr) (void)hipFree(c->hg_plan);
+  c->hg_order = nullptr; c->hg_plan = nullptr; c->handover_points = 0;
+  const int64_t ob = nesvor_hashgrid_cloud_order_bytes(N), pb = nesvor_hashgrid_cloud_plan_bytes(&d.grid, N);
+  if (hipMalloc(&c->hg_order, (size_t)ob) != hipSuccess) { c->hg_order = nullptr; (void)hipGetLastError(); return; }
+  if (pb > 0 && hipMalloc(&c->hg_plan, (size_t)pb) != hipSuccess) { c->hg_plan = nullptr; (void)hipGetLastError(); }
+  c->handover_points = N;
+}
+
 }
 
 extern "C" void* nesvor_step_create(const nesvor_step_t* desc) {
@@ -151,6 +167,7 @@
     c->wimg_stride = ((size_t)need + 255) / 256 * 256;
     if (need > 0 && hipMalloc(&c->wimg, 3 * c->wimg_stride) != hipSuccess) { c->wimg = nullptr; (void)hipGetLastError(); }
   }
+  size_handover(c);
   if (desc->has_b) {
     if (hipMalloc(reinterpret_cast<void**>(&c->mean_ticket), sizeof(unsigned)) != hipSuccess) { c->mean_ticket = nullptr; (void)hipGetLastError(); }
     else if (hipMemset(c->mean_ticket, 0, sizeof(unsigned)) != hipSuccess) { (void)hipFree(c->mean_ticket); c->mean_ticket = nullptr; (void)hipGetLastError(); }
@@ -185,6 +202,7 @@
   if (handle == nullptr || desc == nullptr) return (int)hipErrorInvalidValue;
   if (bias_free_refused(*desc)) return (int)hipErrorInvalidValue;
   static_cast<StepCtx*>(handle)->d = *desc;
+  size_handover(static_cast<StepCtx*>(handle));
   return 0;
 }
 
@@ -204,6 +222,8 @@
   StepCtx* c = static_cast<StepCtx*>(handle);
   (void)hipEventDestroy(c->ev_agg); (void)hipEventDestroy(c->ev_owner); (void)hipEventDestroy(c->ev_sg0); (void)hipEventDestroy(c->ev_sg1);
   if (c->wimg != nullptr) (void)hipFree(c->wimg);
+  if (c->hg_order != nullptr) (void)hipFree(c->hg_order);
+  if (c->hg_plan != nullptr) (void)hipFree(c->hg_plan);
   if (c->mean_ticket != nullptr) (void)hipFree(c->mean_ticket);
   for (int k = 0; k < NESVOR_STEP_TIMED_SPANS; ++k) {
     if (c->t0[k] != nullptr) (void)hipEventDestroy(c->t0[k]);
@@ -249,6 +269,10 @@
   const bool split_d = scaled(net_d), split_s = d.has_lv && scaled(net_s), split_b = d.has_b && scaled(net_b);
   const int layout = NESVOR_LAYOUT_FEATURE_MAJOR;
   const bool overlap_owner = (d.overlap_owner & 1) != 0;
+  static const bool fwd_forced = getenv("NESVOR_HASHGRID_FWD") != nullptr;
+  const bool handover = S >= 128 && !fwd_forced && ctx->hg_order != nullptr && ctx->handover_points == N;
+  const void* hg_order = handover ? ctx->hg_order : nullptr;
+  const void* hg_plan = handover ? ctx->hg_plan : nullptr;
   const int64_t table_off = d.table - d.flat_param;
   const bool fuse_adamw = adam != nullptr && phase == 0 && (d.overlap_owner & 2) != 0 && d.table != nullptr && d.flat_param != nullptr &&
                           d.g_table == d.flat_grad + table_off && table_off >= 0 && table_off < d.flat_numel;
@@ -310,8 +334,12 @@
     }
     {
       Span t(ctx, NESVOR_STEP_SPAN_HASHGRID_FWD, main);
-      NESVOR_TRY(nesvor_hashgrid_forward_bounded(&d.grid, d.u, d.table, d.pe, N, layout | (S >= 128 ? NESVOR_LAYOUT_CLUSTERED : 0),
-                                                 split_d ? prep_d + NESVOR_MLP_PREP_XB : nullptr, main));
+      if (handover)
+        NESVOR_TRY(nesvor_hashgrid_forward_plan(&d.grid, d.u, d.table, d.pe, N, layout, split_d ? prep_d + NESVOR_MLP_PREP_XB : nullptr,
+                                                ctx->hg_order, phase == 0 ? ctx->hg_plan : nullptr, d.queue_scale, main));
+      else
+        NESVOR_TRY(nesvor_hashgrid_forward_bounded(&d.grid, d.u, d.table, d.pe, N, layout | (S >= 128 ? NESVOR_LAYOUT_CLUSTERED : 0),
+                                                   split_d ? prep_d + NESVOR_MLP_PREP_XB : nullptr, main));
     }
    }
     if (bias_stop) {
@@ -389,8 +417,8 @@
   if (phase == 0) {
     {
       Span t(ctx, NESVOR_STEP_SPAN_HASHGRID_BWD_AGGREGATE, main);
-      NESVOR_TRY(nesvor_hashgrid_backward_bounded(&d.grid, d.u, d.table, d.dpe, d.g_table, du, N, layout, d.hg_workspace, 1, 0, L,
-                                                  d.queue_scale, dpe_bound, main));
+      NESVOR_TRY(nesvor_hashgrid_backward_plan(&d.grid, d.u, d.table, d.dpe, d.g_table, du, N, layout, d.hg_workspace, 1, 0, L,
+                                               d.queue_scale, dpe_bound, hg_order, hg_plan, main));
     }
     hipStream_t owner_stream = main;
     if (overlap_owner) {
@@ -409,11 +437,11 @@
     }
     if (overlap_owner && hipEventRecord(ctx->ev_owner, side) != hipSuccess) return (int)hipGetLastError();
   } else if (phase == 1) {
-    return nesvor_hashgrid_backward_bounded(&d.grid, d.u, d.table, d.dpe, d.g_table, du, N, layout, d.hg_workspace, 3, split_level, L,
-                                            d.queue_scale, dpe_bound, main);
+    return nesvor_hashgrid_backward_plan(&d.grid, d.u, d.table, d.dpe, d.g_table, du, N, layout, d.hg_workspace, 3, split_level, L,
+                                         d.queue_scale, dpe_bound, hg_order, nullptr, main);
   } else {
-    NESVOR_TRY(nesvor_hashgrid_backward_bounded(&d.grid, d.u, d.table, d.dpe, d.g_table, du, N, layout, d.hg_workspace, 1 | 4 | 8, 0,
-                                                split_level, d.queue_scale, dpe_bound, main));
+    NESVOR_TRY(nesvor_hashgrid_backward_plan(&d.grid, d.u, d.table, d.dpe, d.g_table, du, N, layout, d.hg_workspace, 1 | 4 | 8, 0,
+                                             split_level, d.queue_scale, dpe_bound, hg_order, nullptr, main));
     hipStream_t owner_stream = main;
     if (overlap_owner) {
       if (hipEventRecord(ctx->ev_agg, main) != hipSuccess || hipStreamWaitEvent(side, ctx->ev_agg, 0) != hipSuccess) return (int)hipGetLastError();
diff --git a/nesvor_amd/encoding.py b/nesvor_amd/encoding.py
--- a/nesvor_amd/encoding.py
+++ b/nesvor_amd/encoding.py
@@ -12,8 +12,23 @@
 _FWD_MODE = __import__("os").environ.get("NESVOR_HASHGRID_FWD", "")
 
 
-def hashgrid_forward(spec: HashGridSpec, u: torch.Tensor, table: torch.Tensor, layout=_lib.LAYOUT_ROW_MAJOR, clustered=False):
+class CloudPlan:
+
+    def __init__(self, spec, u, order, records):
+        self.spec, self.u, self.version = spec, u, u._version
+        self.order, self.records = order, records
+
+    def fits(self, spec, u) -> bool:
+        return u is self.u and u._version == self.version and spec is self.spec
+
+
+def hashgrid_forward(spec: HashGridSpec, u: torch.Tensor, table: torch.Tensor, layout=_lib.LAYOUT_ROW_MAJOR, clustered=False,
+                     want_plan=False):
     _lib.require_device(u, table, dtype=torch.float32, name="hashgrid input/table")
+    if want_plan:
+        if not clustered or u.shape[0] == 0:
+            raise RuntimeError("a cloud plan exists for clustered, non-empty batches only")
+        return _hashgrid_forward_plan(spec, u, table, layout)
     N = u.shape[0]
     E = spec.n_output_dims
     shape = (N, E) if layout == _lib.LAYOUT_ROW_MAJOR else (E, N)
@@ -39,6 +54,23 @@
     return pe
 
 
+def _hashgrid_forward_plan(spec, u, table, layout, pe_absmax=None):
+    N = u.shape[0]
+    E = spec.n_output_dims
+    pe = torch.empty((N, E) if layout == _lib.LAYOUT_ROW_MAJOR else (E, N), dtype=torch.float32, device=u.device)
+    lib = _lib.load()
+    g = ctypes.byref(spec.c_struct)
+    order = torch.empty(lib.nesvor_hashgrid_cloud_order_bytes(N), dtype=torch.uint8, device=u.device)
+    nbytes = lib.nesvor_hashgrid_cloud_plan_bytes(g, N)
+    records = torch.empty(nbytes // 4, dtype=torch.int32, device=u.device) if nbytes > 0 else None
+    sizer = queue_sizer(spec, N, u.device)
+    with torch.cuda.device(u.device), _lib.kernel_timer.span("hashgrid_fwd"):
+        err = lib.nesvor_hashgrid_forward_plan(g, _lib.ptr(u), _lib.ptr(table), _lib.ptr(pe), N, layout, _lib.ptr(pe_absmax), _lib.ptr(order),
+                                               _lib.ptr(records), sizer.scale, _lib.stream_ptr())
+    _lib.check(err, "hashgrid forward (with cloud plan)")
+    return pe, CloudPlan(spec, u, order, records)
+
+
 def points_are_ordered(u: torch.Tensor, box_fraction: float = 1.0 / 16) -> bool:
     n = min(int(u.shape[0]), 4096)
     if n < 2:
@@ -142,7 +174,7 @@
 
 
 def hashgrid_backward(spec, u, table, dpe, grad_table=None, need_input_grad=True, layout=_lib.LAYOUT_ROW_MAJOR,
-                      method="owner", levels=None, grad_u=None, first=True, owner_stream=None, dy_bound=None, clustered=True):
+                      method="owner", levels=None, grad_u=None, first=True, owner_stream=None, dy_bound=None, clustered=True, plan=None):
     _lib.require_device(u, table, dpe, dtype=torch.float32, name="hashgrid backward input")
     if not clustered:
         layout = layout | _lib.LAYOUT_UNCLUSTERED | _lib.LAYOUT_DY_SCRATCH
@@ -166,8 +198,12 @@
                     _lib.ptr(grad_u), N, layout, _lib.ptr(ws))
             l0, l1 = (0, spec.n_levels) if levels is None else levels
             extra = 0 if first else (4 | 8)
-            call = lambda stage: lib.nesvor_hashgrid_backward_bounded(*args, stage | extra, l0, l1, sizer.scale, _lib.ptr(dy_bound),
-                                                                      _lib.stream_ptr())
+            if plan is not None and not (clustered and plan.fits(spec, u)):
+                plan = None
+            p_order = _lib.ptr(plan.order) if plan is not None else None
+            p_rec = _lib.ptr(plan.records) if plan is not None and (l0, l1) == (0, spec.n_levels) else None
+            call = lambda stage, st=None: lib.nesvor_hashgrid_backward_plan(*args, stage | extra, l0, l1, sizer.scale, _lib.ptr(dy_bound),
+                                                                            p_order, p_rec, st or _lib.stream_ptr())
             if _lib.kernel_timer.enabled:
                 with _lib.kernel_timer.span("hashgrid_bwd_aggregate"):
                     err = call(1)
@@ -178,8 +214,7 @@
                 err = call(1)
                 if err == 0:
                     owner_stream.wait_stream(torch.cuda.current_stream(u.device))
-                    err = lib.nesvor_hashgrid_backward_bounded(*args, 2 | extra, l0, l1, sizer.scale, _lib.ptr(dy_bound),
-                                                               ctypes.c_void_p(owner_stream.cuda_stream))
+                    err = call(2, ctypes.c_void_p(owner_stream.cuda_stream))
             else:
                 err = call(3)
         else:
```
